# gillet-thomas/NeuroViT

Measured on AMD Instinct MI355X. Metric: fMRI volumes/sec (fwd+bwd) ViT3D 128^3 p16 d768 L12 [timed step = fwd+bwd+AdamW update], higher is better.
Workload: dtype bf16; 1 GPU; ViT3D-base 128^3 patch 16, train step (fwd+bwd+AdamW), batch 4/GPU, dropout 0; global_batch=4, parallelism=dp1, grad_buckets=7, grad_allreduce=none (1 GPU)

## Files before the change

include/neurovit_hip.h:

```cpp
#ifndef NEUROVIT_HIP_H
#define NEUROVIT_HIP_H

#ifdef __cplusplus
extern "C" {
#endif

#define NV_OK 0
#define NV_ERR_ARG (-1)
#define NV_ERR_HIP (-2)
#define NV_ERR_ARCH (-3)

int nv_version(void);
int nv_arch_ok(void);
const char* nv_last_error(void);

#define NV_OPERAND_BF16 0
#define NV_OPERAND_FP16 1
int nv_set_operand_format(int fmt);
int nv_operand_format(void);

int nv_prof_enable(int on);
int nv_prof_summary(int kind, double* ms, double* work, long* count);
int nv_prof_summary_bytes(int kind, double* bytes);

int nv_gemm_bf16(int layout, int epi, int M, int N, int K, const void* A, long lda, const void* B, long ldb, void* C,
                 long ldc, const float* bias, const void* aux_in, long ld_aux_in, void* aux_out, long ld_aux_out,
                 int accumulate, float alpha, unsigned long drop_seed, float drop_p, void* stream);

int nv_gemm_tile_rows(int layout, int M, int N, int K, long lda, long ldb);

int nv_quant_rows_f8(const float* W, long ldw, int rows, int cols, void* out8, long ld8, float act_scale, float* colscale, void* stream);
int nv_ln_fwd_f8(const float* x, long ldx, int M, int d, const float* gamma, const float* beta, float eps, float out_scale, void* y8,
                 long ldy, void* stream);
int nv_gemm_f8(int epi, int M, int N, int K, const void* A8, long lda, const void* B8, long ldb, void* C, long ldc,
               const float* colscale, const float* bias, const void* aux_in, long ld_aux_in, float out_scale, void* stream);
int nv_ln_fwd_f8_train(const float* x, long ldx, int M, int d, const float* gamma, const float* beta, float eps, float out_scale, void* y8, long ldy8,
                       void* y16, long ldy16, float* mean, float* rstd, void* stream);
int nv_gemm_f8_gelu_train(int M, int N, int K, const void* A8, long lda, const void* B8, long ldb, const float* colscale, const float* bias,
                          float out_scale, void* h8, long ldh8, void* h16, long ldh16, void* u16, long ldu16, unsigned long drop_seed,
                          float drop_p, void* stream);
int nv_gemm_f8_resid_drop(int M, int N, int K, const void* A8, long lda, const void* B8, long ldb, void* C, long ldc, const float* colscale,
                          const float* bias, const void* aux_in, long ld_aux_in, unsigned long drop_seed, float drop_p, void* stream);

int nv_gemm_f32(int epi, int M, int N, int K, const float* A, long lda, const float* B, long ldb, float* C, long ldc,
                const float* bias, const float* resid, long ldr, void* stream);
int nv_gemm_f32_set_tile(int wm, int wn);
int nv_attn_fwd_f32(const float* qkv, long ld_qkv, int B, int n, int heads, int dim_head, float scale, float* out, long ld_out,
                    void* stream);
int nv_ln_fwd_f32(const float* x, long ldx, int M, int d, const float* gamma, const float* beta, float eps, float* y, long ldy,
                  float* mean, float* rstd, void* stream);

typedef struct nv_gemm_problem {
  int M, N, K;
  const void* A; long lda;
  const void* B; long ldb;
  void* C; long ldc;
  int accumulate;
  void* C16; long ldc16;
} nv_gemm_problem;
int nv_gemm_bf16_grouped(int layout, int epi, int count, const nv_gemm_problem* problems, void* stream);

typedef struct nv_adamw_arena {
  int struct_size;
  int step;
  double lr, beta1, beta2, eps, weight_decay;
  float grad_scale;
  int keep_grads;
  float* params; float* grads; float* adam_m; float* adam_v; void* params16;
} nv_adamw_arena;
int nv_gemm_bf16_grouped_adamw(int count, const nv_gemm_problem* problems, const nv_adamw_arena* opt, void* stream);
int nv_adamw_ranges(const nv_adamw_arena* opt, const long* begins, const long* lens, int count, void* stream);

int nv_gemm_set_tile(int bm, int bn);

int nv_gemm_lnfold_supported(int M, int N, int K);
long nv_ln_fold_stats_floats(int M, int d);
int nv_ln_fold_weight(const float* W, long ldw, int N, int K, const float* gamma, const float* beta, const float* bias, void* Wg16, long ldg,
                      float* colsum, float* fbias, void* stream);
int nv_gemm_resid_ln(int M, int N, int K, const void* A, long lda, const void* W, long ldw, const float* bias, const float* resid, long ldr, float* out,
                     long ldo, void* out16, long ldo16, float* stats, void* stream);
int nv_gemm_lnfold(int gelu, int M, int N, int K, const void* X16, long ldx, const void* Wg16, long ldw, const float* stats, const float* colsum,
                   const float* fbias, float eps, void* out16, long ldo, void* stream);

int nv_skinny_nt(int epi, int R, int N, int K, const void* A, long lda, const void* W, long ldw, const float* bias, const float* resid,
                 long ldr, void* out, long ldo, void* u_out, long ldu, unsigned long drop_seed, float drop_p, void* stream);
int nv_skinny_nn(int epi, int R, int N, int K, const void* A, long lda, const void* W, long ldw, const void* u, long ldu, void* out, long ldo,
                 float* dcol, int accumulate, unsigned long drop_seed, float drop_p, void* stream);
int nv_skinny_nn_sparse(int R, int N, int K, const void* A, long lda, const void* W, long ldw, void* out, long total_rows, int keep_every,
                        void* stream);

int nv_ln_fwd(const float* x, long ldx, int M, int d, const float* gamma, const float* beta, float eps, void* y, long ldy,
              float* mean, float* rstd, void* stream);
long nv_ln_bwd_workspace_bytes(int M, int d);
int nv_ln_bwd(const float* dy, long lddy, const float* x, long ldx, const float* mean, const float* rstd, const float* gamma,
              int M, int d, const float* g_in, float* g_out, long ldg, void* g16, long ldg16, float* dgamma, float* dbeta,
              float* dcolsum, int accumulate, void* workspace, long ws_bytes, unsigned long drop_seed, float drop_p,
              void* stream, void* reduce_stream);
#define NV_LN_NO_REDUCE ((void*)(-1L))
int nv_ln_bwd_reduce(const void* workspace, int M, int d, float* dgamma, float* dbeta, float* dcolsum, int accumulate, void* stream);

typedef struct nv_reduce_job {
  const float* partials;
  int rows, width, nseg;
  float* out[3];
  int accumulate;
} nv_reduce_job;
int nv_reduce_multi(const nv_reduce_job* jobs, int count, void* stream);
int nv_ln_bwd_partial_rows(int M);

long nv_zscore_crop_workspace_bytes(int B);
int nv_volume_sigma(const void* raw, int dtype, const long* strides5, int B, const int* crop8, float eps, float* sigma, float* mean,
                    void* workspace, long ws_bytes, void* stream);
int nv_zscore_crop(const void* raw, int dtype, const long* strides5, int B, const int* crop8, float eps, float* out,
                   float* stats, void* workspace, long ws_bytes, void* stream);

int nv_patch_ln_fwd(const float* video, const long* strides5, int B, int C, int F, int H, int W, int p1, int p2, int pf,
                    const float* gamma, const float* beta, float eps, void* out, long ldo, float* mean, float* rstd,
                    const float* vol_sigma, void* stream);
int nv_patch_set_mode(int mode);
int nv_patch_ln_fwd_4d(const float* x, int Bo, int H, int W, int D, int T, int p1, int p2, int pf, const float* gamma,
                       const float* beta, float eps, void* out, long ldo, float* mean, float* rstd, const float* vol_sigma,
                       void* stream);
int nv_patch_ln_fwd_f32(const float* video, const long* strides5, int B, int C, int F, int H, int W, int p1, int p2, int pf,
                        const float* gamma, const float* beta, float eps, float* out, long ldo, float* mean, float* rstd,
                        const float* vol_sigma, void* stream);
int nv_patch_ln_fwd_4d_f32(const float* x, int Bo, int H, int W, int D, int T, int p1, int p2, int pf, const float* gamma,
                           const float* beta, float eps, float* out, long ldo, float* mean, float* rstd, const float* vol_sigma,
                           void* stream);
long nv_patch_ln_bwd_workspace_bytes(int tokens, int P);
int nv_patch_ln_bwd(const float* video, const long* strides5, int B, int C, int F, int H, int W, int p1, int p2, int pf,
                    const float* dxp, long ldd, const float* mean, const float* rstd, float* dgamma, float* dbeta,
                    int accumulate, void* workspace, long ws_bytes, void* stream);
int nv_patch_ln_dx(const float* video, const long* strides5, int B, int C, int F, int H, int W, int p1, int p2, int pf,
                   const float* dxp, long ldd, const float* mean, const float* rstd, const float* gamma,
                   float* dvideo, const long* dstrides5, void* stream);

int nv_embed_finish_fwd(const float* t, long ldt, int B, int N, int d, const float* gamma, const float* beta, float eps,
                        const float* pos, const float* cls, float* x, long ldx, float* mean, float* rstd,
                        unsigned long drop_seed, float drop_p, void* stream);
long nv_embed_finish_bwd_workspace_bytes(int B, int N, int d);
int nv_embed_finish_bwd(const float* g, long ldg, const float* t, long ldt, const float* mean, const float* rstd,
                        const float* gamma, int B, int N, int d, float* dt, long lddt, void* dt16, long lddt16, float* dgamma,
                        float* dbeta, float* dbias_pe, float* dpos, float* dcls, int accumulate, void* workspace, long ws_bytes,
                        unsigned long drop_seed, float drop_p, void* stream);

int nv_attn_set_mode(int mode);
int nv_attn_fwd(const void* qkv, long ld_qkv, int B, int n, int heads, int dim_head, float scale, void* out, long ld_out,
                float* lse, unsigned long drop_seed, float drop_p, void* stream);
int nv_attn_fwd_o8(const void* qkv, long ld_qkv, int B, int n, int heads, int dim_head, float scale, void* out, long ld_out,
                   float out_scale, void* stream);
int nv_attn_bwd(const void* qkv, long ld_qkv, const void* out, const void* dout, long ld_out, const float* lse, int B, int n,
                int heads, int dim_head, float scale, float* delta, void* dqkv, long ld_dqkv, unsigned long drop_seed,
                float drop_p, void* stream);
#define NV_ATTN_PER_HEAD 0
#define NV_ATTN_FUSE_MEAN 1
#define NV_ATTN_FUSE_MAX 2
#define NV_ATTN_FUSE_MIN 3
#define NV_ATTN_ROWS_ALL 0
#define NV_ATTN_ROWS_CLS 1
int nv_attn_probs(int qkv_f32, const void* qkv, long ld_qkv, int B, int n, int heads, int dim_head, float scale, int fusion, int rows,
                  float* out, void* stream);
long nv_attn_rollout_workspace_bytes(int B, int n);
int nv_attn_rollout(const float* const* maps, int L, int B, int n, int start_mean, float* out, void* workspace, long ws_bytes, void* stream);
#define NV_ATTN_GRAD_PER_HEAD 0
#define NV_ATTN_GRAD_RELEVANCE 1
int nv_attn_grad(const void* qkv, long ld_qkv, const void* dout, long ld_dout, int B, int n, int heads, int dim_head, float scale, int form,
                 float* out, void* stream);
long nv_attn_relevance_workspace_bytes(int B, int n);
int nv_attn_relevance(const float* const* maps, int L, int B, int n, int start_mean, float* out, void* workspace, long ws_bytes, void* stream);
int nv_stream_sync(void* from, void* to);
int nv_spin_us(int microseconds, void* stream);

int nv_head_fwd(const float* x, long row_stride, int B, int d, const float* gamma, const float* beta, float eps,
                const float* W, const float* bias, int C, float* xh, float* stats, float* logits, void* stream);
long nv_head_bwd_workspace_bytes(int B, int d);
int nv_head_bwd(const float* dlogits, int B, int C, const float* W, const float* x, long row_stride, const float* stats,
                const float* xh, const float* gamma, int d, int n, float* g, long ldg, void* g16, long ldg16, float* dgamma,
                float* dbeta, float* dW, float* dbias, float* dcolsum, int accumulate, void* workspace, long ws_bytes,
                unsigned long drop_seed, float drop_p, int pool_mean, void* stream);
long nv_head_step_workspace_bytes(int B, int d);
int nv_head_step(const float* x, long row_stride, int B, int d, const float* gamma, const float* beta, float eps, const float* W,
                 const float* bias, int C, const long* labels, float grad_scale, float* xh, float* stats, float* logits, float* loss,
                 float* dlogits, int n, float* g, long ldg, void* g16, long ldg16, float* dgamma, float* dbeta, float* dW, float* dbias,
                 float* dcolsum, int accumulate, void* workspace, long ws_bytes, unsigned long drop_seed, float drop_p, void* stream);
int nv_token_mean(const float* x, int B, int n, int d, float* out, void* stream);

long nv_colsum_workspace_bytes(int M, int N);
int nv_colsum_bf16(const void* X, long ld, int M, int N, float* out, int accumulate, void* workspace, long ws_bytes,
                   void* stream);

int nv_ce_loss(const float* logits, const long* target, int B, int C, float grad_scale, float* loss, float* dlogits,
               void* stream);
int nv_adamw_step(float* p, const void* grad, int grad_bf16, float* m, float* v, void* p16, long count, int step, double lr,
                  double beta1, double beta2, double eps, double weight_decay, float grad_scale, int max_blocks, void* stream);
#define NV_LOSS_SCALE_FLOATS 16
int nv_loss_scale_init(float* state, float init_scale, float growth_factor, float backoff_factor, int growth_interval, int start_step, void* stream);
int nv_loss_scale_check(const float* grads, long count, float* state, void* stream);
int nv_loss_scale_update(float* state, double lr, double beta1, double beta2, void* stream);
int nv_ce_loss_scaled(const float* logits, const long* target, int B, int C, float grad_scale, const float* scale_state, float* loss,
                      float* dlogits, void* stream);
int nv_adamw_step_scaled(float* p, const void* grad, int grad_bf16, float* m, float* v, void* p16, long count, int step, double lr,
                         double beta1, double beta2, double eps, double weight_decay, float grad_scale, int max_blocks,
                         const float* scale_state, void* stream);
int nv_head_step_scaled(const float* x, long row_stride, int B, int d, const float* gamma, const float* beta, float eps, const float* W,
                        const float* bias, int C, const long* labels, float grad_scale, const float* scale_state, float* xh, float* stats,
                        float* logits, float* loss, float* dlogits, int n, float* g, long ldg, void* g16, long ldg16, float* dgamma,
                        float* dbeta, float* dW, float* dbias, float* dcolsum, int accumulate, void* workspace, long ws_bytes,
                        unsigned long drop_seed, float drop_p, void* stream);
#define NV_GRAD_CLIP_MAX_BLOCKS 2048
#define NV_GRAD_CLIP_BYTES (64 + 8 * NV_GRAD_CLIP_MAX_BLOCKS)
int nv_grad_sumsq(const void* grad, int grad_16bit, long count, float* clip_state, float* scale_state, int max_blocks, void* stream);
int nv_grad_clip_finish(float* clip_state, float max_norm, float grad_scale, const float* scale_state, void* stream);
int nv_adamw_step_clipped(float* p, const void* grad, int grad_bf16, float* m, float* v, void* p16, long count, int step, double lr,
                          double beta1, double beta2, double eps, double weight_decay, float grad_scale, int max_blocks,
                          const float* scale_state, const float* clip_state, void* stream);
#define NV_ADAMW_MAX_GROUPS 64
#define NV_ADAMW_MAX_SEGMENTS 1024
typedef struct nv_adamw_groups {
  int struct_size;
  int n_groups;
  const void* segments;
  double lr[NV_ADAMW_MAX_GROUPS];
  double weight_decay[NV_ADAMW_MAX_GROUPS];
} nv_adamw_groups;
long nv_adamw_segments_bytes(int segments);
int nv_adamw_segments_build(void* table, long table_bytes, const long* ends, const int* groups, int segments, int n_groups, long count, void* stream);
int nv_adamw_segments_release(void* table);
int nv_adamw_step_grouped(float* p, const void* grad, int grad_bf16, float* m, float* v, void* p16, long count, int step,
                          const nv_adamw_groups* groups, double beta1, double beta2, double eps, float grad_scale, int max_blocks,
                          const float* scale_state, const float* clip_state, void* stream);
int nv_ema_update(float* ema, const float* p, long count, float weight, int max_blocks, void* stream);
int nv_cast_bf16_2d(const float* src, long ld_src, int rows, int cols, void* dst, long ld_dst, void* stream);
int nv_dropout_apply(const float* x, long ldx, int M, int N, unsigned long drop_seed, float drop_p, void* out16, long ld16,
                     float* out32, long ld32, void* stream);
int nv_copy_2d_f32(const float* src, long ld_src, int rows, int cols, float* dst, long ld_dst, int accumulate, void* stream);

long nv_gradcam_workspace_bytes(int B, int n);
int nv_gradcam_reduce(const void* act, const float* grad, int B, int n, int d, float* cam, float* minmax, void* workspace,
                      long ws_bytes, void* stream);
long nv_gradcam_per_volume_workspace_bytes(int B, int n);
int nv_gradcam_reduce_per_volume(const void* act, const float* grad, int B, int n, int d, float* cam, float* minmax, void* workspace,
                                 long ws_bytes, void* stream);
long nv_token_map_to_volume_workspace_bytes(int B, const int* grid3);
int nv_token_map_to_volume(const float* maps, int B, const int* grid3, const int* out3, int normalize, double keep_percent, float* out,
                           void* workspace, long ws_bytes, void* stream);

#define NV_SCORE_PROB 0
#define NV_SCORE_LOGIT 1
int nv_token_ranks(const float* maps, int B, int N, int* ranks, void* stream);
int nv_mask_patches(const float* x, int B, const int* size3, const int* patch3, const int* labels, const int* jobs, int J, float value,
                    const float* base, long base_stride, float* out, void* stream);
int nv_mask_patches_set_group(int group);
int nv_class_scores(const float* logits, int J, int C, const int* jobs, const long* cls, int B, int kind, float* scores, void* stream);
int nv_curve_auc(const float* scores, int B, int K, long ld, float* auc, void* stream);
int nv_occlusion_gather(const float* ref, const float* scores, const int* labels, int B, int N, int NB, float* maps, void* stream);

int nv_path_points(const float* x, int B, long V, const int* jobs, int J, const float* alphas, int K, float value, const float* base,
                   long base_stride, float* out, void* stream);
int nv_class_score_grads(const float* logits, int J, int C, const int* jobs, const long* cls, int B, int kind, float* dlogits, void* stream);
int nv_path_accumulate(const float* g, const int* jobs, int J, const float* weights, int K, float* acc, int B, long V, void* stream);
int nv_path_finish(const float* acc, const float* x, int B, long V, float value, const float* base, long base_stride, float* attr, void* stream);
int nv_attr_token_sums(const float* attr, int B, const int* size3, const int* patch3, float* sums, void* stream);

#define NV_SERIES_SCOPE_SERIES 0
#define NV_SERIES_SCOPE_VOLUME 1
#define NV_SERIES_LAYOUT_SERIES 0
#define NV_SERIES_LAYOUT_FRAMES 1
long nv_gradcam_grouped_workspace_bytes(int V, int n, int group);
int nv_gradcam_reduce_grouped(const void* act, const float* grad, int V, int n, int d, int group, float* cam, float* minmax, void* workspace,
                              long ws_bytes, void* stream);
long nv_series_map_to_volumes_workspace_bytes(int B, int T, const int* grid3, int scope);
int nv_series_map_to_volumes(const float* maps, int B, int T, const int* grid3, const int* out3, int normalize, int scope, double keep_percent,
                             int layout, float* out, void* workspace, long ws_bytes, void* stream);
int nv_series_leave_one_out(const float* z, const float* z_base, int B, int T, float* out, void* stream);
int nv_temporal_grad_x_input(const float* dx, const float* z, int B, int T, float* out, void* stream);

long nv_temporal_head_param_count(int ff);
int nv_temporal_head_fwd(const float* x, int B, int T, int ff, const float* params, float eps, unsigned long drop_seed, float drop_p,
                         float* out, void* stream);
int nv_temporal_head_bwd(const float* x, int B, int T, int ff, const float* params, float eps, unsigned long drop_seed, float drop_p,
                         const float* dout, float* grads, int accumulate, float* dx, void* stream);

typedef struct nv_vit_config {
  int image_size, image_patch_size, frames, frame_patch_size;
  int channels, num_classes, dim, depth, heads, dim_head, mlp_dim;
  float ln_eps;
  int pool_mean;
  int image_width, patch_width;
  int no_proj_dropout;
} nv_vit_config;

long nv_vit_param_count(const nv_vit_config* cfg);
int nv_vit_param_table(const nv_vit_config* cfg, long* offsets, long* numels, int max_entries);
long nv_vit_workspace_bytes(const nv_vit_config* cfg, int B, int training);
long nv_vit_workspace_offset(const nv_vit_config* cfg, int B, int training, const char* name, int layer);
typedef struct nv_vit_attn_export {
  int struct_size;
  float** maps;
  int fusion;
  int rows;
} nv_vit_attn_export;
typedef struct nv_vit_input {
  const float* vol_sigma;
  int time_points;
  int rows_form;
  const nv_vit_attn_export* attn_export;
} nv_vit_input;
int nv_vit_forward_in(const nv_vit_config* cfg, int B, const float* video, const long* shape5, const long* strides5,
                      const nv_vit_input* in, const float* params, const void* params16, void* workspace, long ws_bytes,
                      int training, float drop_p, float emb_drop_p, unsigned long drop_seed, float* logits, void* stream);
int nv_vit_forward(const nv_vit_config* cfg, int B, const float* video, const long* shape5, const long* strides5,
                   const float* params, const void* params16, void* workspace, long ws_bytes, int training, float drop_p, float emb_drop_p,
                   unsigned long drop_seed, float* logits, void* stream);
long nv_vit_lnfold_floats(const nv_vit_config* cfg);
int nv_vit_lnfold_prepare(const nv_vit_config* cfg, const float* params, void* fold16, float* fold32, void* stream);
int nv_vit_forward_lnfold(const nv_vit_config* cfg, int B, const float* video, const long* shape5, const long* strides5, const nv_vit_input* in,
                          const float* params, const void* params16, const void* fold16, const float* fold32, void* workspace, long ws_bytes,
                          float* logits, void* stream);
int nv_vit_forward_f32(const nv_vit_config* cfg, int B, const float* video, const long* shape5, const long* strides5,
                       const nv_vit_input* in, const float* params, void* workspace, long ws_bytes, float* logits, void* stream);
long nv_vit_fp8_scale_count(const nv_vit_config* cfg);
int nv_vit_quantize_fp8(const nv_vit_config* cfg, const float* params, const float* act_scales, void* params8, float* colscales, void* stream);
int nv_vit_forward_fp8(const nv_vit_config* cfg, int B, const float* video, const long* shape5, const long* strides5,
                       const nv_vit_input* in, const float* params, const void* params16, const void* params8, const float* colscales,
                       const float* act_scales, void* workspace, long ws_bytes, float* logits, void* stream);
int nv_vit_forward_fp8_train(const nv_vit_config* cfg, int B, const float* video, const long* shape5, const long* strides5,
                             const nv_vit_input* in, const float* params, const void* params16, const void* params8, const float* colscales,
                             const float* act_scales, void* workspace, long ws_bytes, float drop_p, float emb_drop_p, unsigned long drop_seed,
                             float* logits, void* stream);
int nv_vit_backward(const nv_vit_config* cfg, int B, const float* video, const long* strides5, const float* params,
                    const void* params16, void* workspace, long ws_bytes, const float* dlogits, float* grads,
                    int accumulate, float drop_p, float emb_drop_p, unsigned long drop_seed, void* stream, void* aux_stream);

int nv_vit_backward_stages(const nv_vit_config* cfg, int B, const float* video, const long* strides5, const float* params,
                           const void* params16, void* workspace, long ws_bytes, const float* dlogits, float* grads,
                           int accumulate, int first_stage, int last_stage, float drop_p, float emb_drop_p,
                           unsigned long drop_seed, void* stream, void* aux_stream, int join_aux);
int nv_vit_backward_stages16(const nv_vit_config* cfg, int B, const float* video, const long* strides5, const float* params,
                             const void* params16, void* workspace, long ws_bytes, const float* dlogits, float* grads, void* grads16,
                             int accumulate, int first_stage, int last_stage, float drop_p, float emb_drop_p,
                             unsigned long drop_seed, void* stream, void* aux_stream, int join_aux, int rows_form);
typedef struct nv_vit_backward_opts {
  int struct_size;
  float* dvideo;
  const long* dvideo_strides5;
  int weight_grads;
} nv_vit_backward_opts;
int nv_vit_backward_ex(const nv_vit_config* cfg, int B, const float* video, const long* strides5, const float* params,
                       const void* params16, void* workspace, long ws_bytes, const float* dlogits, float* grads, void* grads16,
                       int accumulate, int first_stage, int last_stage, float drop_p, float emb_drop_p,
                       unsigned long drop_seed, void* stream, void* aux_stream, int join_aux, int rows_form, const nv_vit_backward_opts* opts);
typedef struct nv_vit_attn_grad_export {
  int struct_size;
  float** maps;
  int form;
} nv_vit_attn_grad_export;
int nv_vit_backward_attn(const nv_vit_config* cfg, int B, const float* video, const long* strides5, const float* params,
                         const void* params16, void* workspace, long ws_bytes, const float* dlogits, float* grads, void* grads16,
                         int accumulate, int first_stage, int last_stage, float drop_p, float emb_drop_p,
                         unsigned long drop_seed, void* stream, void* aux_stream, int join_aux, int rows_form, const nv_vit_backward_opts* opts,
                         const nv_vit_attn_grad_export* attn_grad);
int nv_vit_backward_tokens(const nv_vit_config* cfg, int B, const float* video, const long* strides5, const float* params,
                           const void* params16, void* workspace, long ws_bytes, const float* dtokens, float* grads, void* grads16,
                           int accumulate, int first_stage, int last_stage, float drop_p, float emb_drop_p,
                           unsigned long drop_seed, void* stream, void* aux_stream, int join_aux, int rows_form, const nv_vit_backward_opts* opts);
int nv_vit_stage_param_range(const nv_vit_config* cfg, int stage, long* begin, long* end);
int nv_vit_set_cls_tail(int on);
int nv_vit_set_head_step(int on);

typedef struct nv_dp_plan {
  int struct_size;
  int world;
  void* comm;
  void* comm_stream;
  int n_buckets;
  int update_per_bucket;
  void* grads16;
// ... 143 lines not shown
```

neurovit_amd/_cabi.py:

```python
from __future__ import annotations

import ctypes
import os
import re
from typing import Dict, List, Tuple

_HERE = os.path.dirname(os.path.abspath(__file__))
HEADER = os.path.join(os.path.dirname(_HERE), "include", "neurovit_hip.h")
LIB_PATH = os.environ.get("NEUROVIT_HIP_LIB") or os.path.join(_HERE, "lib", "libneurovit_hip.so")

_SCALARS = {"int": ctypes.c_int, "long": ctypes.c_long, "float": ctypes.c_float, "double": ctypes.c_double}


class VitConfig(ctypes.Structure):
    _fields_ = [("image_size", ctypes.c_int), ("image_patch_size", ctypes.c_int), ("frames", ctypes.c_int),
                ("frame_patch_size", ctypes.c_int), ("channels", ctypes.c_int), ("num_classes", ctypes.c_int),
                ("dim", ctypes.c_int), ("depth", ctypes.c_int), ("heads", ctypes.c_int), ("dim_head", ctypes.c_int),
                ("mlp_dim", ctypes.c_int), ("ln_eps", ctypes.c_float), ("pool_mean", ctypes.c_int),
                ("image_width", ctypes.c_int), ("patch_width", ctypes.c_int),
                ("no_proj_dropout", ctypes.c_int)]


class VitInput(ctypes.Structure):
    _fields_ = [("vol_sigma", ctypes.c_void_p), ("time_points", ctypes.c_int), ("rows_form", ctypes.c_int), ("attn_export", ctypes.c_void_p)]
# ... 28 lines not shown

class AdamwArena(ctypes.Structure):
    _fields_ = [("struct_size", ctypes.c_int), ("step", ctypes.c_int), ("lr", ctypes.c_double), ("beta1", ctypes.c_double),
                ("beta2", ctypes.c_double), ("eps", ctypes.c_double), ("weight_decay", ctypes.c_double), ("grad_scale", ctypes.c_float),
                ("keep_grads", ctypes.c_int), ("params", ctypes.c_void_p), ("grads", ctypes.c_void_p), ("adam_m", ctypes.c_void_p),
                ("adam_v", ctypes.c_void_p), ("params16", ctypes.c_void_p)]


class BackwardOpts(ctypes.Structure):
    _fields_ = [("struct_size", ctypes.c_int), ("dvideo", ctypes.c_void_p), ("dvideo_strides5", ctypes.c_void_p), ("weight_grads", ctypes.c_int)]


class LossOpts(ctypes.Structure):
    _fields_ = [("struct_size", ctypes.c_int), ("label_smoothing", ctypes.c_float), ("class_weight", ctypes.c_void_p), ("mix", ctypes.c_void_p)]


class DropPath(ctypes.Structure):
    _fields_ = [("struct_size", ctypes.c_int), ("factors", ctypes.c_void_p)]


DROP_PATH_SCHEDULES = {"linear": 0, "constant": 1}


ADAMW_MAX_GROUPS, ADAMW_MAX_SEGMENTS = 64, 1024


class AdamwGroups(ctypes.Structure):
    _fields_ = [("struct_size", ctypes.c_int), ("n_groups", ctypes.c_int), ("segments", ctypes.c_void_p),
                ("lr", ctypes.c_double * ADAMW_MAX_GROUPS), ("weight_decay", ctypes.c_double * ADAMW_MAX_GROUPS)]


MIX_COLS = 12


ABI_VERSION = 8


def parse_header(path: str = HEADER) -> Dict[str, Tuple[object, List[object]]]:
    src = open(path).read()
    src = re.sub(r"/\*.*?\*/", " ", src, flags=re.S)
    protos = {}
    for m in re.finditer(r"\b(int|long|const char\s*\*)\s+(nv_\w+)\s*\(([^;{]*?)\)\s*;", src, flags=re.S):
        ret, name, args = m.group(1), m.group(2), " ".join(m.group(3).split())
        restype = ctypes.c_char_p if "char" in ret else _SCALARS[ret]
        argtypes = []
        if args and args != "void":
            for a in args.split(","):
                a = a.strip()
                if "*" in a:
                    argtypes.append(ctypes.c_char_p if re.match(r"const char\s*\*", a) else ctypes.c_void_p)
                elif a.startswith("unsigned long"):
                    argtypes.append(ctypes.c_ulong)
                else:
                    argtypes.append(_SCALARS[a.split()[0]])
        protos[name] = (restype, argtypes)
    return protos


class _Lib:
    def __init__(self):
        self._dll = None
        self.protos = parse_header()

    def load(self):
        if self._dll is None:
            if not os.path.exists(LIB_PATH):
                raise RuntimeError(
                    f"neurovit_amd: {LIB_PATH} not found - build it with `python -c 'import __graft_entry__ as g; g.build()'` "
                    "(or `make -C neurovit_amd/csrc`). There is no CPU / PyTorch fallback for this path.")
            dll = ctypes.CDLL(LIB_PATH)
            for name, (restype, argtypes) in self.protos.items():
                fn = getattr(dll, name)
                fn.restype, fn.argtypes = restype, argtypes
            got = dll.nv_abi_version()
            if got != ABI_VERSION:
                raise RuntimeError(f"neurovit_amd: {LIB_PATH} has ABI revision {got}, this binding expects {ABI_VERSION} - rebuild the library "
                                   "(make -C neurovit_amd/csrc); see INTEGRATION.md 'ABI revisions'")
            if os.environ.get("NEUROVIT_ATTN_MODE"):
                dll.nv_attn_set_mode(int(os.environ["NEUROVIT_ATTN_MODE"]))
            if os.environ.get("NEUROVIT_ADAMW_WGS"):
                dll.nv_gemm_set_tile(12, int(os.environ["NEUROVIT_ADAMW_WGS"]))
            if os.environ.get("NEUROVIT_HEAD_STEP"):
                dll.nv_vit_set_head_step(int(os.environ["NEUROVIT_HEAD_STEP"]))
            if os.environ.get("NEUROVIT_WGRAD_WGS"):
                dll.nv_gemm_set_tile(14, int(os.environ["NEUROVIT_WGRAD_WGS"]))
            if os.environ.get("NEUROVIT_PATCH_MODE"):
                dll.nv_patch_set_mode(int(os.environ["NEUROVIT_PATCH_MODE"]))
            if os.environ.get("NEUROVIT_ADAMW_CAP"):
                dll.nv_gemm_set_tile(13, int(os.environ["NEUROVIT_ADAMW_CAP"]))
            self._dll = dll
        return self._dll

    def __getattr__(self, name):
        return getattr(self.load(), name)


lib = _Lib()


OPERAND_FORMATS = {"bf16": 0, "fp16": 1}
_operand_format = "bf16"


def set_operand_format(fmt: str) -> None:
    global _operand_format
    if fmt != _operand_format:
        if fmt not in OPERAND_FORMATS:
            raise ValueError(f"neurovit_amd: operand format must be 'bf16' or 'fp16', got {fmt!r}")
        check(lib.nv_set_operand_format(OPERAND_FORMATS[fmt]), "nv_set_operand_format")
        _operand_format = fmt


def operand_format() -> str:
    return _operand_format


def last_error() -> str:
    return (lib.nv_last_error() or b"").decode()


def check(rc: int, what: str = "") -> None:
    if rc != 0:
        raise RuntimeError(f"neurovit_amd C-ABI call failed ({what}, rc={rc}): {last_error()}")


def require_gpu() -> None:
    import torch
    if not torch.cuda.is_available():
        raise RuntimeError("neurovit_amd: no HIP device available - this path only runs on MI355X (gfx950); "
                           "there is no CPU fallback.")
    if lib.nv_arch_ok() != 1:
        raise RuntimeError(f"neurovit_amd: current device is not gfx950: {last_error()}")
```

neurovit_amd/csrc/attention.hip:

```cpp
#include "common.h"

bool attn_generic_supported(int dim_head);
int launch_attn_generic_fwd(const void* qkv, long ld, int B, int n, int heads, int dh, float scale, void* out, long ldo, float* lse, DropCfg drop,
                            hipStream_t s);
int launch_attn_generic_bwd(const void* qkv, long ld, const void* out, const void* dout, long ldo, const float* lse, int B, int n, int heads, int dh,
                            float scale, float* delta, void* dqkv, long ldd, DropCfg drop, hipStream_t s);

constexpr int DH = 64;
constexpr int TQ = 64;
constexpr int TK = 64;
constexpr int IMG = TK * DH * 2;

__device__ __forceinline__ void tile_gload(const r16* X, long ld, int row0, int nrows, int tid, uint4 (&reg)[2]) {
#pragma unroll
  for (int i = 0; i < 2; ++i) {
    const int c = tid + 256 * i, row = row0 + (c >> 3);
    const bool ok = row < nrows;
    const uint4 v = *reinterpret_cast<const uint4*>(X + (ok ? (long)row * ld + ((c & 7) << 3) : 0));
    reg[i] = ok ? v : make_uint4(0, 0, 0, 0);
  }
}
__device__ __forceinline__ void tile_swrite(char* img, int tid, const uint4 (&reg)[2]) {
#pragma unroll
  for (int i = 0; i < 2; ++i) {
// ... 742 lines not shown
  for (int qt = 0; qt < nqt; ++qt) {
    __syncthreads();
    tile_swrite(sQ, tid, rq);
    tile_swrite(sD, tid, rd);
    if (tid < TQ) { sL[tid] = rl; sDl[tid] = rdl; }
    __syncthreads();
    if (qt + 1 < nqt) {
      tile_gload(Q, ld, (qt + 1) * TQ, n, tid, rq);
      tile_gload(dO, ldo, (qt + 1) * TQ, n, tid, rd);
      stats_load(qt + 1);
    }
    dkv_tile<DROP, T>(sQ, sD, sL, sDl, qt, n, kf, vf, dk, dv, scale_log2e, drop, gb.by, key0 + r, r, g);
  }
  const int key = key0 + r;
  if (key < n) {
    r16* drow = dqkv + ((long)b * n + key) * ldd + h * DH;
#pragma unroll
    for (int t = 0; t < 4; ++t) {
      *reinterpret_cast<r16x4*>(drow + inner + 16 * t + 4 * g) = cvt4<T>(dk[t][0] * scale, dk[t][1] * scale, dk[t][2] * scale, dk[t][3] * scale);
      *reinterpret_cast<r16x4*>(drow + 2 * inner + 16 * t + 4 * g) = cvt4<T>(dv[t][0], dv[t][1], dv[t][2], dv[t][3]);
    }
  }
}

template <typename T>
__device__ __forceinline__ float row_delta(const r16* __restrict__ dout, const r16* __restrict__ out, long off, int g, r16x8 (&dof)[2]) {
  float dl = 0.f;
#pragma unroll
  for (int ks = 0; ks < 2; ++ks) {
    dof[ks] = *reinterpret_cast<const r16x8*>(dout + off + 32 * ks + 8 * g);
    const r16x8 of = *reinterpret_cast<const r16x8*>(out + off + 32 * ks + 8 * g);
#pragma unroll
    for (int j = 0; j < 8; ++j) dl += dec1<T>(dof[ks][j]) * dec1<T>(of[j]);
  }
  return group_sum(dl);
}

template <bool DROP, typename T>
__device__ __forceinline__ void attn_bwd_dq_res_body(char* rsmem, int by, int bx, int nblk, const r16* __restrict__ qkv, long ld,
                                                     const r16* __restrict__ out, const r16* __restrict__ dout, long ldo,
                                                     const float* __restrict__ lse, int n, int heads, float scale, float* __restrict__ delta,
                                                     r16* __restrict__ dqkv, long ldd, const DropCfg& drop) {
  const int tid = threadIdx.x, lane = tid & 63, r = lane & 15, g = lane >> 4;
  const int wid = __builtin_amdgcn_readfirstlane(tid >> 6);
  const int b = by / heads, h = by - b * heads, inner = heads * DH;
  const r16* Q = qkv + (long)b * n * ld + h * DH;
  const int nkt = (n + TK - 1) / TK;
  char* sK = rsmem;
  char* sV = rsmem + nkt * IMG;
  res_dma(Q + inner, ld, n, nkt, sK, wid, lane);
  res_dma(Q + 2 * inner, ld, n, nkt, sV, wid, lane);
  const int grp = res_group(n, wid, bx, nblk);
  const int q0 = (grp < 0 ? 0 : grp) * 16;
  const int qrow = min(q0 + r, n - 1);
  const float scale_log2e = scale * 1.44269504088896340736f;

  r16x8 qf[2], dof[2];
#pragma unroll
  for (int ks = 0; ks < 2; ++ks) qf[ks] = *reinterpret_cast<const r16x8*>(Q + (long)qrow * ld + 32 * ks + 8 * g);
  const float dl = row_delta<T>(dout, out, ((long)b * n + qrow) * ldo + h * DH, g, dof);
  const float lse2 = lse[((long)b * heads + h) * n + qrow] * 1.44269504088896340736f;
  __syncthreads();
  if (grp < 0) return;
  if (g == 0 && q0 + r < n) delta[((long)b * heads + h) * n + q0 + r] = dl;

  f32x4 dq[4];
#pragma unroll
  for (int t = 0; t < 4; ++t) dq[t] = f32x4{0.f, 0.f, 0.f, 0.f};
  for (int kt = 0; kt < nkt; ++kt)
    dq_tile<DROP, T>(sK + kt * IMG, sV + kt * IMG, kt, n, qf, dof, dq, dl, lse2, scale_log2e, drop, by, q0 + r, r, g);
  const int q = q0 + r;
  if (q < n) {
    r16* drow = dqkv + ((long)b * n + q) * ldd + h * DH;
#pragma unroll
    for (int t = 0; t < 4; ++t)
      *reinterpret_cast<r16x4*>(drow + 16 * t + 4 * g) = cvt4<T>(dq[t][0] * scale, dq[t][1] * scale, dq[t][2] * scale, dq[t][3] * scale);
  }
}

template <bool DROP, bool OWN_DELTA, typename T>
__device__ __forceinline__ void attn_bwd_dkv_res_body(char* rsmem, int by, int bx, int nblk, const r16* __restrict__ qkv, long ld,
                                                      const r16* __restrict__ out, const r16* __restrict__ dout, long ldo,
                                                      const float* __restrict__ lse, const float* __restrict__ delta, int n, int heads,
                                                      float scale, r16* __restrict__ dqkv, long ldd, const DropCfg& drop) {
  const int tid = threadIdx.x, lane = tid & 63, r = lane & 15, g = lane >> 4;
  const int wid = __builtin_amdgcn_readfirstlane(tid >> 6);
  const int b = by / heads, h = by - b * heads, inner = heads * DH;
  const r16* Q = qkv + (long)b * n * ld + h * DH;
  const r16* K = Q + inner;
  const r16* V = Q + 2 * inner;
  const r16* dO = dout + (long)b * n * ldo + h * DH;
  const float* L = lse + ((long)b * heads + h) * n;
  const int nqt = (n + TQ - 1) / TQ;
  char* sQ = rsmem;
  char* sD = rsmem + nqt * IMG;
  float* sL = reinterpret_cast<float*>(rsmem + 2 * nqt * IMG);
  float* sDl = sL + nqt * TQ;
  res_dma(Q, ld, n, nqt, sQ, wid, lane);
  res_dma(dO, ldo, n, nqt, sD, wid, lane);
  if constexpr (OWN_DELTA) {
    for (int q = tid; q < nqt * TQ; q += RES_THREADS) sL[q] = (q < n) ? L[q] * 1.44269504088896340736f : INFINITY;
    const r16* O = out + (long)b * n * ldo + h * DH;
    for (int q0 = 16 * wid; q0 < nqt * TQ; q0 += 16 * (RES_THREADS / 64)) {
      r16x8 scratch[2];
      const int q = q0 + r;
      const float dl = row_delta<T>(dO, O, (long)min(q, n - 1) * ldo, g, scratch);
      if (g == 0) sDl[q] = (q < n) ? dl : 0.f;
    }
  } else {
    const float* Dl = delta + ((long)b * heads + h) * n;
    for (int q = tid; q < nqt * TQ; q += RES_THREADS) {
      sL[q] = (q < n) ? L[q] * 1.44269504088896340736f : INFINITY;
      sDl[q] = (q < n) ? Dl[q] : 0.f;
    }
  }
  const int grp = res_group(n, wid, bx, nblk);
  const int key0 = (grp < 0 ? 0 : grp) * 16;
  const int krow = min(key0 + r, n - 1);
  const float scale_log2e = scale * 1.44269504088896340736f;
  r16x8 kf[2], vf[2];
#pragma unroll
  for (int ks = 0; ks < 2; ++ks) {
    kf[ks] = *reinterpret_cast<const r16x8*>(K + (long)krow * ld + 32 * ks + 8 * g);
    vf[ks] = *reinterpret_cast<const r16x8*>(V + (long)krow * ld + 32 * ks + 8 * g);
  }
  __syncthreads();
  if (grp < 0) return;

  f32x4 dk[4], dv[4];
#pragma unroll
  for (int t = 0; t < 4; ++t) dk[t] = dv[t] = f32x4{0.f, 0.f, 0.f, 0.f};
  for (int qt = 0; qt < nqt; ++qt)
    dkv_tile<DROP, T>(sQ + qt * IMG, sD + qt * IMG, sL + qt * TQ, sDl + qt * TQ, qt, n, kf, vf, dk, dv, scale_log2e, drop, by, key0 + r, r, g);
  const int key = key0 + r;
  if (key < n) {
    r16* drow = dqkv + ((long)b * n + key) * ldd + h * DH;
#pragma unroll
    for (int t = 0; t < 4; ++t) {
      *reinterpret_cast<r16x4*>(drow + inner + 16 * t + 4 * g) = cvt4<T>(dk[t][0] * scale, dk[t][1] * scale, dk[t][2] * scale, dk[t][3] * scale);
      *reinterpret_cast<r16x4*>(drow + 2 * inner + 16 * t + 4 * g) = cvt4<T>(dv[t][0], dv[t][1], dv[t][2], dv[t][3]);
    }
  }
}

template <bool DROP, typename T>
__global__ __launch_bounds__(RES_THREADS) void attn_bwd_dq_res_kernel(const r16* __restrict__ qkv, long ld, const r16* __restrict__ out,
                                                                      const r16* __restrict__ dout, long ldo, const float* __restrict__ lse,
                                                                      int n, int heads, float scale, float* __restrict__ delta,
                                                                      r16* __restrict__ dqkv, long ldd, DropCfg drop) {
  extern __shared__ __attribute__((aligned(16))) char rsmem[];
  const ResBlock rb = res_block(n);
  attn_bwd_dq_res_body<DROP, T>(rsmem, rb.by, rb.bx, rb.nblk, qkv, ld, out, dout, ldo, lse, n, heads, scale, delta, dqkv, ldd, drop);
}

template <bool DROP, typename T>
__global__ __launch_bounds__(RES_THREADS) void attn_bwd_dkv_res_kernel(const r16* __restrict__ qkv, long ld, const r16* __restrict__ dout,
                                                                       long ldo, const float* __restrict__ lse, const float* __restrict__ delta,
                                                                       int n, int heads, float scale, r16* __restrict__ dqkv, long ldd,
                                                                       DropCfg drop) {
  extern __shared__ __attribute__((aligned(16))) char rsmem[];
  const ResBlock rb = res_block(n);
  attn_bwd_dkv_res_body<DROP, false, T>(rsmem, rb.by, rb.bx, rb.nblk, qkv, ld, nullptr, dout, ldo, lse, delta, n, heads, scale, dqkv, ldd, drop);
}

template <bool DROP, typename T>
__global__ __launch_bounds__(RES_THREADS) void attn_bwd_res_kernel(const r16* __restrict__ qkv, long ld, const r16* __restrict__ out,
                                                                   const r16* __restrict__ dout, long ldo, const float* __restrict__ lse,
                                                                   int n, int heads, float scale, float* __restrict__ delta,
                                                                   r16* __restrict__ dqkv, long ldd, DropCfg drop) {
  extern __shared__ __attribute__((aligned(16))) char rsmem[];
  const int nblk = attn_res_blocks(n);
  const int lid = xcd_remap(blockIdx.x, gridDim.x);
  const int by = lid / (2 * nblk), rem = lid - by * 2 * nblk;
  if (rem < nblk) attn_bwd_dkv_res_body<DROP, true, T>(rsmem, by, rem, nblk, qkv, ld, out, dout, ldo, lse, nullptr, n, heads, scale, dqkv, ldd, drop);
  else attn_bwd_dq_res_body<DROP, T>(rsmem, by, rem - nblk, nblk, qkv, ld, out, dout, ldo, lse, n, heads, scale, delta, dqkv, ldd, drop);
}

template <bool DROP, typename T>
__global__ __launch_bounds__(256, 2) void attn_bwd_dq_wide_kernel(const r16* __restrict__ qkv, long ld, const r16* __restrict__ out,
                                                                  const r16* __restrict__ dout, long ldo, const float* __restrict__ lse, int n,
                                                                  int heads, float scale, float* __restrict__ delta, r16* __restrict__ dqkv,
                                                                  long ldd, DropCfg drop) {
  __shared__ __attribute__((aligned(16))) char wsmem[2 * 2 * IMG];
  const int tid = threadIdx.x, lane = tid & 63, r = lane & 15, g = lane >> 4;
  const int wid = __builtin_amdgcn_readfirstlane(tid >> 6);
  const Grid2 gb = grid2d_xcd((n + WIDE_ROWS - 1) / WIDE_ROWS);
  const int b = gb.by / heads, h = gb.by - b * heads, inner = heads * DH;
  const r16* Q = qkv + (long)b * n * ld + h * DH;
  const int q0 = gb.bx * WIDE_ROWS + 32 * wid;
  const float scale_log2e = scale * 1.44269504088896340736f;

  r16x8 qf[2][2], dof[2][2];
  float dl[2], lse2[2];
#pragma unroll
  for (int u = 0; u < 2; ++u) {
    const int qrow = min(q0 + 16 * u + r, n - 1);
    float d = 0.f;
#pragma unroll
    for (int ks = 0; ks < 2; ++ks) {
      qf[u][ks] = *reinterpret_cast<const r16x8*>(Q + (long)qrow * ld + 32 * ks + 8 * g);
      const long off = ((long)b * n + qrow) * ldo + h * DH + 32 * ks + 8 * g;
      dof[u][ks] = *reinterpret_cast<const r16x8*>(dout + off);
      const r16x8 of = *reinterpret_cast<const r16x8*>(out + off);
#pragma unroll
      for (int j = 0; j < 8; ++j) d += dec1<T>(dof[u][ks][j]) * dec1<T>(of[j]);
    }
    dl[u] = group_sum(d);
    lse2[u] = lse[((long)b * heads + h) * n + qrow] * 1.44269504088896340736f;
    if (g == 0 && q0 + 16 * u + r < n) delta[((long)b * heads + h) * n + q0 + 16 * u + r] = dl[u];
  }

  const unsigned bytes = (unsigned)((((long)n - 1) * ld + DH) * 2);
  const dma_desc rsK = uniform_rsrc((Q + inner), bytes);
  const dma_desc rsV = uniform_rsrc((Q + 2 * inner), bytes);
  int voff[2];
#pragma unroll
  for (int i = 0; i < 2; ++i) {
    const int row = (wid + 4 * i) * 8 + (lane >> 3);
    voff[i] = (int)(((long)row * ld + (((lane & 7) ^ (row & 7)) << 3)) * 2);
  }
  const int step = (int)(64 * ld * 2);
  auto issue = [&](int t, char* stage) {
#pragma unroll
    for (int i = 0; i < 2; ++i) {
      lds_dma<16>(rsK, stage + (wid + 4 * i) * 1024, voff[i], t * step);
      lds_dma<16>(rsV, stage + IMG + (wid + 4 * i) * 1024, voff[i], t * step);
    }
  };

  f32x4 dq[2][4];
#pragma unroll
  for (int u = 0; u < 2; ++u)
#pragma unroll
    for (int t = 0; t < 4; ++t) dq[u][t] = f32x4{0.f, 0.f, 0.f, 0.f};
  const int nkt = (n + TK - 1) / TK;
  issue(0, wsmem);
  for (int kt = 0; kt < nkt; ++kt) {
    const char* cur = wsmem + (kt & 1) * 2 * IMG;
    asm volatile("s_waitcnt vmcnt(0)" ::: "memory");
    __builtin_amdgcn_s_barrier();
    if (kt + 1 < nkt) issue(kt + 1, wsmem + ((kt + 1) & 1) * 2 * IMG);
    RowFrags F;
    f32x4 sc[2][4], dp[2][4], ds[2][4];
    load_row_frags(cur, r, g, F);
    mfma_rows<T>(F, qf[0], sc[0], true);
// ... 92 lines not shown
      lds_dma<4>(rsL, stage + 2 * IMG, ln * 4, t * TQ * 4);
      lds_dma<4>(rsDl, stage + 2 * IMG + TQ * 4, ln * 4, t * TQ * 4);
    }
  };

  f32x4 dk[2][4], dv[2][4];
#pragma unroll
  for (int u = 0; u < 2; ++u)
#pragma unroll
    for (int t = 0; t < 4; ++t) dk[u][t] = dv[u][t] = f32x4{0.f, 0.f, 0.f, 0.f};
  const int nqt = (n + TQ - 1) / TQ;
  issue(0, wsmem);
  for (int qt = 0; qt < nqt; ++qt) {
    const char* cur = wsmem + (qt & 1) * STG;
    asm volatile("s_waitcnt vmcnt(0)" ::: "memory");
    __builtin_amdgcn_s_barrier();
    if (qt + 1 < nqt) issue(qt + 1, wsmem + ((qt + 1) & 1) * STG);
    const float* sL = reinterpret_cast<const float*>(cur + 2 * IMG);
    const float* sDl = sL + TQ;
    RowFrags F;
    if constexpr (DROP) {
#pragma unroll
      for (int u = 0; u < 2; ++u) {
        f32x4 sc1[4], dp1[4];
        load_row_frags(cur, r, g, F);
        mfma_rows<T>(F, kf[u], sc1, true);
        __builtin_amdgcn_sched_barrier(0);
        load_row_frags(cur + IMG, r, g, F);
        mfma_rows<T>(F, vf[u], dp1, true);
        __builtin_amdgcn_sched_barrier(0);
        dkv_softmax_grad_inplace<DROP>(sc1, dp1, sL, sDl, qt, n, scale_log2e, drop, gb.by, key0 + 16 * u + r, g);
        r16x8 pf1[2], dsf1[2];
        pf1[0] = cvt8<T>(sc1[0], sc1[1]); pf1[1] = cvt8<T>(sc1[2], sc1[3]);
        dsf1[0] = cvt8<T>(dp1[0], dp1[1]); dsf1[1] = cvt8<T>(dp1[2], dp1[3]);
        __builtin_amdgcn_sched_barrier(0);
        load_tr_frags(cur + IMG, r, g, F);
        mfma_rows<T>(F, pf1, dv[u], false);
        __builtin_amdgcn_sched_barrier(0);
        load_tr_frags(cur, r, g, F);
        mfma_rows<T>(F, dsf1, dk[u], false);
        __builtin_amdgcn_sched_barrier(0);
      }
      continue;
    }
    f32x4 sc[2][4], dp[2][4];
    load_row_frags(cur, r, g, F);
    mfma_rows<T>(F, kf[0], sc[0], true);
    mfma_rows<T>(F, kf[1], sc[1], true);
    __builtin_amdgcn_sched_barrier(0);
    load_row_frags(cur + IMG, r, g, F);
    mfma_rows<T>(F, vf[0], dp[0], true);
    mfma_rows<T>(F, vf[1], dp[1], true);
    __builtin_amdgcn_sched_barrier(0);
    r16x8 pf[2][2], dsf[2][2];
    dkv_softmax_grad_inplace<DROP>(sc[0], dp[0], sL, sDl, qt, n, scale_log2e, drop, gb.by, key0 + r, g);
    pf[0][0] = cvt8<T>(sc[0][0], sc[0][1]); pf[0][1] = cvt8<T>(sc[0][2], sc[0][3]);
    dsf[0][0] = cvt8<T>(dp[0][0], dp[0][1]); dsf[0][1] = cvt8<T>(dp[0][2], dp[0][3]);
    dkv_softmax_grad_inplace<DROP>(sc[1], dp[1], sL, sDl, qt, n, scale_log2e, drop, gb.by, key0 + 16 + r, g);
    pf[1][0] = cvt8<T>(sc[1][0], sc[1][1]); pf[1][1] = cvt8<T>(sc[1][2], sc[1][3]);
    dsf[1][0] = cvt8<T>(dp[1][0], dp[1][1]); dsf[1][1] = cvt8<T>(dp[1][2], dp[1][3]);
    __builtin_amdgcn_sched_barrier(0);
    load_tr_frags(cur + IMG, r, g, F);
    mfma_rows<T>(F, pf[0], dv[0], false);
    mfma_rows<T>(F, pf[1], dv[1], false);
    __builtin_amdgcn_sched_barrier(0);
    load_tr_frags(cur, r, g, F);
    mfma_rows<T>(F, dsf[0], dk[0], false);
    mfma_rows<T>(F, dsf[1], dk[1], false);
  }
#pragma unroll
  for (int u = 0; u < 2; ++u) {
    const int key = key0 + 16 * u + r;
    if (key < n) {
      r16* drow = dqkv + ((long)b * n + key) * ldd + h * DH;
#pragma unroll
      for (int t = 0; t < 4; ++t) {
        *reinterpret_cast<r16x4*>(drow + inner + 16 * t + 4 * g) = cvt4<T>(dk[u][t][0] * scale, dk[u][t][1] * scale, dk[u][t][2] * scale, dk[u][t][3] * scale);
        *reinterpret_cast<r16x4*>(drow + 2 * inner + 16 * t + 4 * g) = cvt4<T>(dv[u][t][0], dv[u][t][1], dv[u][t][2], dv[u][t][3]);
      }
    }
  }
}

extern "C" int nv_attn_bwd(const void* qkv, long ld_qkv, const void* out, const void* dout, long ld_out, const float* lse, int B, int n,
                           int heads, int dim_head, float scale, float* delta, void* dqkv, long ld_dqkv, unsigned long drop_seed, float drop_p,
                           void* stream) {
  NV_CHECK_ARG(attn_generic_supported(dim_head), "nv_attn_bwd: dim_head=%d unsupported (multiples of 8 up to 128)", dim_head);
  NV_CHECK_ARG(B > 0 && n > 0 && heads > 0 && ld_qkv >= 3 * heads * dim_head && ld_dqkv >= 3 * heads * dim_head && ld_out >= heads * dim_head &&
                   (ld_qkv % 8) == 0 && (ld_out % 8) == 0 && (ld_dqkv % 4) == 0,
               "nv_attn_bwd: bad dims");
  NV_CHECK_ARG(nv_aligned16(qkv) && nv_aligned16(out) && nv_aligned16(dout) && nv_aligned16(dqkv), "nv_attn_bwd: alignment");
  hipStream_t s = (hipStream_t)stream;
  const DropCfg drop = make_drop(drop_seed, drop_p);
  if (dim_head != DH)
    return launch_attn_generic_bwd(qkv, ld_qkv, out, dout, ld_out, lse, B, n, heads, dim_head, scale, delta, dqkv, ld_dqkv, drop, s);
  const dim3 grid(((n + TQ - 1) / TQ) * B * heads);
  const bool dropping = drop.thresh != 0, fp16 = nv_operand_format() == NV_OPERAND_FP16;
  const r16* q16 = (const r16*)qkv; const r16* o16 = (const r16*)out; const r16* do16 = (const r16*)dout; r16* dq16 = (r16*)dqkv;
  const int slot = nv_prof_begin(4, 10.0 * B * heads * (double)n * n * DH, stream);
  if (attn_resident(n) && g_attn_mode != 3) {
    NV_CHECK_ARG((long)n * ld_qkv < (1L << 30) && (long)n * ld_out < (1L << 30), "nv_attn_bwd: operand too large for 32-bit buffer offsets");
    const int nt = (n + TK - 1) / TK;
    static bool attr = false;
    if (!attr) {
      ATTN_ATTR(K_DQ_RES, 2 * RES_MAX_TILES * IMG);
      ATTN_ATTR(K_DKV_RES, 2 * RES_MAX_TILES * IMG + 2 * RES_MAX_TILES * TQ * 4);
      ATTN_ATTR(K_BWD_RES, 2 * RES_MAX_TILES * IMG + 2 * RES_MAX_TILES * TQ * 4);
      attr = true;
    }
    const dim3 rgrid(attn_res_blocks(n) * B * heads);
    if (g_attn_bwd_merged) {
      ATTN_LAUNCH(K_BWD_RES, dim3(2 * rgrid.x), dim3(RES_THREADS), 2 * nt * IMG + 2 * nt * TQ * 4, s, q16, ld_qkv, o16, do16, ld_out, lse, n, heads, scale, delta, dq16, ld_dqkv, drop);
      nv_prof_end(slot, stream);
      NV_CHECK_LAUNCH("nv_attn_bwd(resident, one launch)");
      return NV_OK;
    }
    ATTN_LAUNCH(K_DQ_RES, rgrid, dim3(RES_THREADS), 2 * nt * IMG, s, q16, ld_qkv, o16, do16, ld_out, lse, n, heads, scale, delta, dq16, ld_dqkv, drop);
    NV_CHECK_LAUNCH("nv_attn_bwd/dq(resident)");
    ATTN_LAUNCH(K_DKV_RES, rgrid, dim3(RES_THREADS), 2 * nt * IMG + 2 * nt * TQ * 4, s, q16, ld_qkv, do16, ld_out, lse, delta, n, heads, scale, dq16, ld_dqkv, drop);
    nv_prof_end(slot, stream);
    NV_CHECK_LAUNCH("nv_attn_bwd/dkv(resident)");
    return NV_OK;
  }
  const bool wide = g_attn_mode != 1 && (long)n * ld_qkv < (1L << 30) && (long)n * ld_out < (1L << 30) &&
                    (g_attn_mode >= 3 || (long)B * heads * ((n + WIDE_ROWS - 1) / WIDE_ROWS) >= 512);
  const dim3 wgrid(((n + WIDE_ROWS - 1) / WIDE_ROWS) * B * heads);
  if (wide) ATTN_LAUNCH(K_DQ_WIDE, wgrid, dim3(256), 0, s, q16, ld_qkv, o16, do16, ld_out, lse, n, heads, scale, delta, dq16, ld_dqkv, drop);
  else ATTN_LAUNCH(K_DQ, grid, dim3(256), 0, s, q16, ld_qkv, o16, do16, ld_out, lse, n, heads, scale, delta, dq16, ld_dqkv, drop);
  NV_CHECK_LAUNCH("nv_attn_bwd/dq");
  if (wide) ATTN_LAUNCH(K_DKV_WIDE, wgrid, dim3(256), 0, s, q16, ld_qkv, do16, ld_out, lse, delta, n, heads, scale, dq16, ld_dqkv, drop);
  else ATTN_LAUNCH(K_DKV, grid, dim3(256), 0, s, q16, ld_qkv, do16, ld_out, lse, delta, n, heads, scale, dq16, ld_dqkv, drop);
  nv_prof_end(slot, stream);
  NV_CHECK_LAUNCH("nv_attn_bwd/dkv");
  return NV_OK;
}
```

neurovit_amd/csrc/engine.hip:

```cpp
#include <stdlib.h>
#include <string.h>

#include <unordered_map>
#include <utility>
#include <vector>

#include "../../include/neurovit_hip.h"

#include "common.h"

namespace {

inline long align_up(long v, long a) { return (v + a - 1) / a * a; }

struct Dims {
  int B, N, n, P, Ppad, d, inner, m, L, C, heads, dh, M, T;
  int gf, gh, gw;
  int pool_mean;
};

static int g_cls_tail = 1;
extern "C" int nv_vit_set_cls_tail(int on) { g_cls_tail = on ? 1 : 0; return 0; }
static int g_head_step = 1;
extern "C" int nv_vit_set_head_step(int on) { g_head_step = on ? 1 : 0; return 0; }
static bool cls_tail_wanted(const Dims& D, int training, float drop_p, int rows_form) {
  const bool want = rows_form == 1 ? false : (rows_form == 2 ? true : g_cls_tail != 0);
  (void)drop_p;
  return want && !D.pool_mean && (!training || D.B <= 4);
}

static inline float proj_drop_p(const nv_vit_config* c, float drop_p) { return c->no_proj_dropout ? 0.f : drop_p; }

static inline int img_w(const nv_vit_config* c) { return c->image_width > 0 ? c->image_width : c->image_size; }
static inline int pat_w(const nv_vit_config* c) { return c->patch_width > 0 ? c->patch_width : c->image_patch_size; }

int make_dims(const nv_vit_config* c, int B, Dims& D) {
  NV_CHECK_ARG(c && B > 0, "nv_vit: null config or B <= 0");
  NV_CHECK_ARG(c->image_size > 0 && c->image_patch_size > 0 && c->frames > 0 && c->frame_patch_size > 0 &&
                   c->image_size % c->image_patch_size == 0 && c->image_width >= 0 && c->patch_width >= 0 && img_w(c) % pat_w(c) == 0,
               "Image dimensions must be divisible by the patch size.");
  NV_CHECK_ARG(c->frames % c->frame_patch_size == 0, "Frames must be divisible by frame patch size");
  NV_CHECK_ARG(c->dim_head >= 8 && c->dim_head <= 128 && c->dim_head % 8 == 0,
               "nv_vit: dim_head=%d unsupported (multiples of 8 up to 128; 64 runs the MFMA attention kernels, the others scalar ones)", c->dim_head);
  NV_CHECK_ARG(c->dim % 8 == 0 && c->dim <= 2048 && c->mlp_dim % 8 == 0, "nv_vit: dim must be a multiple of 8 and <= 2048, mlp_dim a multiple of 8");
  NV_CHECK_ARG(c->depth >= 1 && c->num_classes >= 1 && c->channels >= 1, "nv_vit: bad depth/classes/channels");
  D.B = B;
  D.gf = c->frames / c->frame_patch_size;
  D.gh = c->image_size / c->image_patch_size;
  D.gw = img_w(c) / pat_w(c);
  D.N = D.gf * D.gh * D.gw;
  D.n = D.N + 1;
  D.P = c->channels * c->image_patch_size * pat_w(c) * c->frame_patch_size;
  D.Ppad = (int)align_up(D.P, 8);
  D.d = c->dim; D.heads = c->heads; D.dh = c->dim_head; D.inner = c->heads * c->dim_head; D.m = c->mlp_dim;
  D.L = c->depth; D.C = c->num_classes;
  D.M = B * D.n; D.T = B * D.N;
  D.pool_mean = c->pool_mean != 0;
  return NV_OK;
}

struct LayerP { long n1g, n1b, wqkv, wo, bo, n2g, n2b, w1, b1, w2, b2; };
struct ParamTab {
  long pos, cls, pe_g, pe_b, pe_w, pe_bias, pe_g2, pe_b2, hg, hb, hw, hbias, total;
  std::vector<LayerP> layer;
  std::vector<long> offsets, numels;
};

void make_params(const Dims& D, ParamTab& T) {
  long cur = 0;
  auto add = [&](long numel) { const long o = cur; T.offsets.push_back(o); T.numels.push_back(numel); cur = align_up(cur + numel, 8); return o; };
  T.pos = add((long)D.n * D.d); T.cls = add(D.d);
  T.pe_g = add(D.P); T.pe_b = add(D.P); T.pe_w = add((long)D.d * D.P); T.pe_bias = add(D.d); T.pe_g2 = add(D.d); T.pe_b2 = add(D.d);
  T.layer.resize(D.L);
  for (int l = 0; l < D.L; ++l) {
    LayerP& p = T.layer[l];
    p.n1g = add(D.d); p.n1b = add(D.d); p.wqkv = add(3L * D.inner * D.d); p.wo = add((long)D.d * D.inner); p.bo = add(D.d);
    p.n2g = add(D.d); p.n2b = add(D.d); p.w1 = add((long)D.m * D.d); p.b1 = add(D.m); p.w2 = add((long)D.d * D.m); p.b2 = add(D.d);
  }
  T.hg = add(D.d); T.hb = add(D.d); T.hw = add((long)D.C * D.d); T.hbias = add(D.C);
  T.total = cur;
}

struct LayerW { long xn1, st1, qkv, lse, ao, x1, xn2, st2, u, h, x2; };
struct LayerScratch { long g16, g16b, du, dqkv, red, red2, red3, cs1; };
struct WS {
  long xp, pst, t, est, x0, xh, hst, wpe16, xm;
  long fst1, fst2;
  long f8x, f8h;
  std::vector<LayerW> layer;
  long g, dxn, hookg, dao, delta, dt, dt16, dxp, dwpe;
  LayerScratch sc[2];
  const LayerScratch& scratch(int l) const { return sc[l & 1]; }
  long red_bytes, red2_bytes, total;
};

void make_ws(const Dims& D, int training, WS& W) {
  long cur = 0;
  auto add = [&](long bytes) { const long o = cur; cur = align_up(cur + bytes, 256); return o; };
  const long M = D.M, T = D.T, d = D.d;
  W.xp = add(T * D.Ppad * 2); W.pst = add(T * 2 * 4); W.t = add(T * d * 4); W.est = add(T * 2 * 4); W.x0 = add(M * d * 4);
  W.xh = add((long)D.B * d * 4); W.hst = add((long)D.B * 2 * 4);
  W.xm = D.pool_mean ? add((long)D.B * d * 4) : -1;
  W.wpe16 = (D.P != D.Ppad) ? add(d * D.Ppad * 2) : -1;
  W.fst1 = add(nv_ln_fold_stats_floats((int)M, (int)d) * 4); W.fst2 = add(nv_ln_fold_stats_floats((int)M, (int)d) * 4);
  const int nl = training ? D.L : 1;
  W.layer.resize(D.L);
  for (int l = 0; l < nl; ++l) {
    LayerW& w = W.layer[l];
    w.xn1 = add(M * d * 2); w.st1 = add(M * 2 * 4); w.qkv = add(M * 3 * D.inner * 2); w.lse = add((long)D.B * D.heads * D.n * 4);
    w.ao = add(M * D.inner * 2); w.x1 = add(M * d * 4); w.xn2 = add(M * d * 2); w.st2 = add(M * 2 * 4);
    w.u = add(M * D.m * 2); w.h = add(M * D.m * 2); w.x2 = add(M * d * 4);
  }
  for (int l = nl; l < D.L; ++l) W.layer[l] = W.layer[0];
  W.f8x = W.f8h = -1;
  if (training) {
    LayerScratch& e = W.sc[0]; LayerScratch& o = W.sc[1];
    W.g = add(M * d * 4); e.g16 = add(M * d * 2); W.dxn = add(M * d * 4); W.hookg = add(M * d * 4); e.du = add(M * D.m * 2);
    W.dao = add(M * D.inner * 2); e.dqkv = add(M * 3 * D.inner * 2); W.delta = add((long)D.B * D.heads * D.n * 4);
    W.dt = add(T * d * 4); W.dt16 = add(T * d * 2); W.dxp = add(T * D.Ppad * 4);
    W.dwpe = (D.P != D.Ppad) ? add(d * D.Ppad * 4) : -1;
    long r = nv_ln_bwd_workspace_bytes(D.M, D.d);
    const long r2 = nv_patch_ln_bwd_workspace_bytes(D.T, D.P), r3 = nv_head_step_workspace_bytes(D.B, D.d),
               r4 = nv_colsum_workspace_bytes(D.M, D.m);
    r = r > r2 ? r : r2; r = r > r3 ? r : r3; r = r > r4 ? r : r4;
    W.red_bytes = r; e.red = add(r);
    e.g16b = add(M * d * 2);
    W.red2_bytes = r4 > r2 ? r4 : r2; e.red2 = add(W.red2_bytes);
    e.red3 = add(nv_ln_bwd_workspace_bytes(D.M, D.d));
    o.g16 = add(M * d * 2); o.g16b = add(M * d * 2); o.du = add(M * D.m * 2); o.dqkv = add(M * 3 * D.inner * 2);
    o.red = add(W.red_bytes); o.red2 = add(W.red2_bytes); o.red3 = add(nv_ln_bwd_workspace_bytes(D.M, D.d));
    const long cs1_bytes = (long)((M + 63) / 64) * D.m * 4;
    e.cs1 = add(cs1_bytes); o.cs1 = add(cs1_bytes);
    W.f8x = add(M * d); W.f8h = add(M * (long)D.m);
  } else {
    W.g = W.dxn = W.hookg = W.dao = W.delta = W.dt = W.dt16 = W.dxp = W.dwpe = -1;
    W.sc[0] = W.sc[1] = {-1, -1, -1, -1, -1, -1, -1, -1};
    W.red_bytes = W.red2_bytes = 0;
  }
  W.total = cur;
}

struct WSF { long xp, pst, t, est, x0, xh, hst, xm, xn1, qkv, ao, x1, xn2, h, x2, total; };
void make_wsf(const Dims& D, WSF& W) {
  long cur = 0;
  auto add = [&](long bytes) { const long o = cur; cur = align_up(cur + bytes, 256); return o; };
  const long M = D.M, T = D.T, d = D.d;
  W.xp = add(T * D.P * 4); W.pst = add(T * 2 * 4); W.t = add(T * d * 4); W.est = add(T * 2 * 4); W.x0 = add(M * d * 4);
  W.xh = add((long)D.B * d * 4); W.hst = add((long)D.B * 2 * 4);
  W.xm = D.pool_mean ? add((long)D.B * d * 4) : -1;
  W.xn1 = add(M * d * 4); W.qkv = add(M * 3 * D.inner * 4); W.ao = add(M * D.inner * 4); W.x1 = add(M * d * 4);
  W.xn2 = add(M * d * 4); W.h = add(M * D.m * 4); W.x2 = add(M * d * 4);
  W.total = cur;
}

inline unsigned long site_seed(unsigned long seed, int site) { return seed ^ (0x9E3779B97F4A7C15ul * (unsigned long)(site + 1)); }

inline const float* path_of(const float* sd, int l, int c, int B) { return sd ? sd + ((long)l * 2 + c) * B : nullptr; }
int check_drop_path(const nv_vit_drop_path* sd, const char* who) {
  if (!sd) return NV_OK;
  NV_CHECK_ARG(sd->struct_size == (int)sizeof(nv_vit_drop_path), "%s: nv_vit_drop_path.struct_size=%d, expected %d (ABI revision %d)", who, sd->struct_size,
               (int)sizeof(nv_vit_drop_path), NV_ABI_VERSION);
  NV_CHECK_ARG(sd->factors && nv_aligned(sd->factors, 4), "%s: nv_vit_drop_path.factors is NULL or not 4-byte aligned", who);
  return NV_OK;
}

inline int stream_sync(hipStream_t from, hipStream_t to) { return nv_stream_sync((void*)from, (void*)to); }
inline int event_failed(const char* what) { nv_set_error("nv_vit_backward: event %s failed", what); return NV_ERR_HIP; }
inline int wait_event(hipStream_t s, hipEvent_t e) { return hipStreamWaitEvent(s, e, 0) == hipSuccess ? NV_OK : event_failed("wait"); }
inline int record_event(hipEvent_t e, hipStream_t s) { return (e && hipEventRecord(e, s) == hipSuccess) ? NV_OK : event_failed("record"); }
inline hipEvent_t deferred_event() {
  static std::vector<hipEvent_t> pool;
  static size_t next = 0;
  if (pool.size() < 32) {
    hipEvent_t e;
    if (hipEventCreateWithFlags(&e, nv_sync_event_flags()) != hipSuccess) return nullptr;
    pool.push_back(e);
    return e;
  }
  return pool[next++ % pool.size()];
}

struct Carry { hipEvent_t ev = nullptr; bool pending = false; };
std::unordered_map<void*, Carry>& carry_map() { static std::unordered_map<void*, Carry> m; return m; }
hipEvent_t carry_take(void* workspace) {
  auto it = carry_map().find(workspace);
  if (it == carry_map().end() || !it->second.pending) return nullptr;
  it->second.pending = false;
  return it->second.ev;
}
int carry_record(void* workspace, hipStream_t on) {
  Carry& c = carry_map()[workspace];
  if (!c.ev && hipEventCreateWithFlags(&c.ev, nv_sync_event_flags()) != hipSuccess) return event_failed("create");
  if (const int rc = record_event(c.ev, on)) return rc;
  c.pending = true;
  return NV_OK;
}

#define RUN(call)            \
  do {                       \
    const int rc__ = (call); \
    if (rc__) return rc__;   \
  } while (0)

struct LinearW { long off[4], numel[4]; };
inline LinearW linear_weights(const Dims& D, const LayerP& q) {
  return {{q.wqkv, q.wo, q.w1, q.w2}, {3L * D.inner * D.d, (long)D.d * D.inner, (long)D.m * D.d, (long)D.d * D.m}};
}

struct Layout { Dims D; ParamTab T; WS W; };
int make_layout(const nv_vit_config* c, int B, int training, Layout& Y) {
  RUN(make_dims(c, B, Y.D));
  make_params(Y.D, Y.T);
  make_ws(Y.D, training, Y.W);
  return NV_OK;
}

}

extern "C" long nv_vit_param_count(const nv_vit_config* cfg) {
  Dims D; if (make_dims(cfg, 1, D)) return -1;
// ... 4 lines not shown
extern "C" int nv_vit_param_table(const nv_vit_config* cfg, long* offsets, long* numels, int max_entries) {
  Dims D; if (make_dims(cfg, 1, D)) return NV_ERR_ARG;
  ParamTab T; make_params(D, T);
  const int cnt = (int)T.offsets.size();
  for (int i = 0; i < cnt && i < max_entries; ++i) { offsets[i] = T.offsets[i]; numels[i] = T.numels[i]; }
  return cnt;
}

extern "C" long nv_vit_workspace_bytes(const nv_vit_config* cfg, int B, int training) {
  Dims D; if (make_dims(cfg, B, D)) return -1;
  if (training == 2) { WSF F; make_wsf(D, F); return F.total; }
  WS W; make_ws(D, training, W);
  return W.total;
}

extern "C" long nv_vit_workspace_offset(const nv_vit_config* cfg, int B, int training, const char* name, int layer) {
  Dims D; if (make_dims(cfg, B, D)) return -1;
  if (training == 2) {
    WSF F; make_wsf(D, F);
    if (layer >= D.L) return -1;
    if (!strcmp(name, "xn1")) return F.xn1; if (!strcmp(name, "qkv")) return F.qkv; if (!strcmp(name, "ao")) return F.ao;
    if (!strcmp(name, "x1")) return F.x1; if (!strcmp(name, "xn2")) return F.xn2; if (!strcmp(name, "h")) return F.h;
    if (!strcmp(name, "x2")) return (layer >= 0 && (layer & 1)) ? F.x0 : F.x2;
    if (!strcmp(name, "xp")) return F.xp; if (!strcmp(name, "t")) return F.t; if (!strcmp(name, "x0")) return F.x0; if (!strcmp(name, "xh")) return F.xh;
    return -1;
  }
  WS W; make_ws(D, training, W);
  if (layer >= 0) {
    if (layer >= D.L) return -1;
    const LayerW& w = W.layer[layer];
    if (!strcmp(name, "xn1")) return w.xn1; if (!strcmp(name, "st1")) return w.st1; if (!strcmp(name, "qkv")) return w.qkv;
    if (!strcmp(name, "lse")) return w.lse; if (!strcmp(name, "ao")) return w.ao; if (!strcmp(name, "x1")) return w.x1;
    if (!strcmp(name, "xn2")) return w.xn2; if (!strcmp(name, "st2")) return w.st2; if (!strcmp(name, "u")) return w.u;
    if (!strcmp(name, "h")) return w.h; if (!strcmp(name, "x2")) return w.x2;
    return -1;
  }
  if (!strcmp(name, "xp")) return W.xp; if (!strcmp(name, "pst")) return W.pst; if (!strcmp(name, "t")) return W.t;
  if (!strcmp(name, "est")) return W.est; if (!strcmp(name, "x0")) return W.x0; if (!strcmp(name, "xh")) return W.xh;
  if (!strcmp(name, "g")) return W.g; if (!strcmp(name, "hookg")) return W.hookg; if (!strcmp(name, "dqkv")) return W.sc[0].dqkv;
  if (!strcmp(name, "dt")) return W.dt; if (!strcmp(name, "dxp")) return W.dxp;
  return -1;
}

static int check_video(const char* who, const nv_vit_config* cfg, int B, const long* shape5, const nv_vit_input* in, bool allow_4d) {
  if (in && in->time_points > 0) {
    NV_CHECK_ARG(allow_4d, "%s: the fused 4D input form is forward-only", who);
    NV_CHECK_ARG(shape5[0] * shape5[4] == B && shape5[4] == in->time_points && shape5[1] == cfg->image_size && shape5[2] == img_w(cfg) && shape5[3] == cfg->frames &&
                     B % in->time_points == 0 && cfg->channels == 1,
                 "%s: 4D input is [%ld,%ld,%ld,%ld,%ld], expected [B/T, %d, %d, %d, T=%d] with B = %d", who, shape5[0], shape5[1], shape5[2], shape5[3],
                 shape5[4], cfg->image_size, img_w(cfg), cfg->frames, in->time_points, B);
    return NV_OK;
  }
  NV_CHECK_ARG(shape5[0] == B && shape5[1] == cfg->channels && shape5[2] == cfg->frames && shape5[3] == cfg->image_size && shape5[4] == img_w(cfg),
               "%s: video is [%ld,%ld,%ld,%ld,%ld], the model was built for [%d,%d,%d,%d,%d] (B, channels, frames, height, width)", who,
               shape5[0], shape5[1], shape5[2], shape5[3], shape5[4], B, cfg->channels, cfg->frames, cfg->image_size, img_w(cfg));
  return NV_OK;
}

static int embed_front16(const nv_vit_config* cfg, const Layout& Y, int B, const float* video, const long* strides5, const nv_vit_input* in, const float* p,
                         const r16* p16, char* ws, unsigned long emb_seed, float emb_drop_p, void* stream) {
  const Dims& D = Y.D; const ParamTab& T = Y.T; const WS& W = Y.W;
  const float eps = cfg->ln_eps;
  const int d = D.d;
  float* pst = (float*)(ws + W.pst);
  const float* sigma = in ? in->vol_sigma : nullptr;
  if (in && in->time_points > 0)
    RUN(nv_patch_ln_fwd_4d(video, B / in->time_points, cfg->image_size, img_w(cfg), cfg->frames, in->time_points, cfg->image_patch_size,
                           pat_w(cfg), cfg->frame_patch_size, p + T.pe_g, p + T.pe_b, eps, ws + W.xp, D.Ppad, pst, pst + D.T, sigma, stream));
  else
    RUN(nv_patch_ln_fwd(video, strides5, B, cfg->channels, cfg->frames, cfg->image_size, img_w(cfg), cfg->image_patch_size,
                        pat_w(cfg), cfg->frame_patch_size, p + T.pe_g, p + T.pe_b, eps, ws + W.xp, D.Ppad, pst, pst + D.T, sigma, stream));
  const void* wpe = p16 + T.pe_w;
  if (D.P != D.Ppad) {
    RUN(nv_cast_bf16_2d(p + T.pe_w, D.P, d, D.P, ws + W.wpe16, D.Ppad, stream));
    wpe = ws + W.wpe16;
  }
  RUN(nv_gemm_bf16(0, 2, D.T, d, D.Ppad, ws + W.xp, D.Ppad, wpe, D.Ppad, ws + W.t, d, p + T.pe_bias, nullptr, 0, nullptr, 0, 0, 1.f, 0, 0.f, stream));
  float* est = (float*)(ws + W.est);
  return nv_embed_finish_fwd((float*)(ws + W.t), d, B, D.N, d, p + T.pe_g2, p + T.pe_b2, eps, p + T.pos, p + T.cls, (float*)(ws + W.x0), d, est,
                             est + D.T, emb_seed, emb_drop_p, stream);
}

static int cls_rows_block16(const Dims& D, const LayerP& q, const LayerW& w, int l, const float* p, const r16* p16, char* ws, float eps, const float* xin,
                            float* x1, float* x2, float* st2, void* u, unsigned long drop_seed, float drop_p, float proj_p, void* stream, const float* sd = nullptr) {
  const int B = D.B, d = D.d;
  const long rs = D.n;
  RUN(nv_skinny_nt_path(0, B, d, D.inner, ws + w.ao, D.inner * rs, p16 + q.wo, D.inner, p + q.bo, xin, d * rs, x1, d * rs, nullptr, 0, site_seed(drop_seed, 4 * l + 1), proj_p, stream,
                        path_of(sd, l, 0, B), D.n));
  RUN(nv_ln_fwd(x1, d * rs, B, d, p + q.n2g, p + q.n2b, eps, ws + w.xn2, d * rs, st2, st2 + D.M, stream));
  RUN(nv_skinny_nt(1, B, D.m, d, ws + w.xn2, d * rs, p16 + q.w1, d, p + q.b1, nullptr, 0, ws + w.h, D.m * rs, u, D.m * rs, site_seed(drop_seed, 4 * l + 2), drop_p, stream));
  return nv_skinny_nt_path(0, B, d, D.m, ws + w.h, D.m * rs, p16 + q.w2, D.m, p + q.b2, x1, d * rs, x2, d * rs, nullptr, 0, site_seed(drop_seed, 4 * l + 3), drop_p, stream,
                           path_of(sd, l, 1, B), D.n);
}

static int pool_head(const Dims& D, const ParamTab& T, const float* p, float eps, const float* xin, char* ws, long xm, long xh, long hst, float* logits,
                     void* stream) {
  const float* pooled = xin;
  long pooled_stride = (long)D.n * D.d;
  if (D.pool_mean) {
    RUN(nv_token_mean(xin, D.B, D.n, D.d, (float*)(ws + xm), stream));
    pooled = (float*)(ws + xm); pooled_stride = D.d;
  }
  return nv_head_fwd(pooled, pooled_stride, D.B, D.d, p + T.hg, p + T.hb, eps, p + T.hw, p + T.hbias, D.C, (float*)(ws + xh), (float*)(ws + hst), logits, stream);
}

extern "C" int nv_vit_forward(const nv_vit_config* cfg, int B, const float* video, const long* shape5, const long* strides5,
                              const float* params, const void* params16, void* workspace, long ws_bytes, int training, float drop_p, float emb_drop_p,
                              unsigned long drop_seed, float* logits, void* stream) {
  return nv_vit_forward_in(cfg, B, video, shape5, strides5, nullptr, params, params16, workspace, ws_bytes, training, drop_p, emb_drop_p, drop_seed, logits, stream);
}

static const nv_vit_attn_export* attn_export_of(const nv_vit_input* in) { return in ? in->attn_export : nullptr; }
static int check_attn_export(const nv_vit_input* in, const char* who) {
  const nv_vit_attn_export* ex = attn_export_of(in);
  if (!ex) return NV_OK;
  NV_CHECK_ARG(ex->struct_size == (int)sizeof(nv_vit_attn_export), "%s: nv_vit_attn_export.struct_size=%d, expected %d (ABI revision %d)", who,
               ex->struct_size, (int)sizeof(nv_vit_attn_export), NV_ABI_VERSION);
  NV_CHECK_ARG(ex->maps, "%s: nv_vit_attn_export.maps is NULL", who);
  NV_CHECK_ARG(ex->fusion >= NV_ATTN_PER_HEAD && ex->fusion <= NV_ATTN_FUSE_MIN && (ex->rows == NV_ATTN_ROWS_ALL || ex->rows == NV_ATTN_ROWS_CLS),
               "%s: nv_vit_attn_export fusion=%d / rows=%d out of range", who, ex->fusion, ex->rows);
  return NV_OK;
}
static int export_layer(const nv_vit_input* in, int l, int qkv_f32, const void* qkv, const Dims& D, int B, float scale, void* stream) {
  const nv_vit_attn_export* ex = attn_export_of(in);
  if (!ex || !ex->maps[l]) return NV_OK;
  return nv_attn_probs(qkv_f32, qkv, 3L * D.inner, B, D.n, D.heads, D.dh, scale, ex->fusion, ex->rows, ex->maps[l], stream);
}

static int forward_in_impl(const Layout& Y, const nv_vit_config* cfg, int B, const float* video, const long* shape5, const long* strides5, const nv_vit_input* in,
                           const float* params, const void* params16, void* workspace, long ws_bytes, int training, float drop_p, float emb_drop_p,
                           unsigned long drop_seed, float* logits, void* stream, bool skip_head, const void* fold16 = nullptr, const float* fold32 = nullptr,
                           const float* sd = nullptr);

extern "C" long nv_vit_lnfold_floats(const nv_vit_config* cfg) {
  Dims D; if (make_dims(cfg, 1, D)) return -1;
  return (long)D.L * (6L * D.inner + 2L * D.m);
}
extern "C" int nv_vit_lnfold_prepare(const nv_vit_config* cfg, const float* params, void* fold16, float* fold32, void* stream) {
  Dims D; RUN(make_dims(cfg, 1, D));
  ParamTab T; make_params(D, T);
  NV_CHECK_ARG(params && fold16 && fold32 && nv_aligned16(params) && nv_aligned16(fold16) && nv_aligned16(fold32), "nv_vit_lnfold_prepare: null / unaligned arena");
  r16* f16 = (r16*)fold16;
  const long per = 6L * D.inner + 2L * D.m;
  for (int l = 0; l < D.L; ++l) {
    const LayerP& q = T.layer[l];
    float* f = fold32 + l * per;
    RUN(nv_ln_fold_weight(params + q.wqkv, D.d, 3 * D.inner, D.d, params + q.n1g, params + q.n1b, nullptr, f16 + q.wqkv, D.d, f, f + 3L * D.inner, stream));
    RUN(nv_ln_fold_weight(params + q.w1, D.d, D.m, D.d, params + q.n2g, params + q.n2b, params + q.b1, f16 + q.w1, D.d, f + 6L * D.inner, f + 6L * D.inner + D.m, stream));
  }
  return NV_OK;
}
extern "C" int nv_vit_forward_lnfold(const nv_vit_config* cfg, int B, const float* video, const long* shape5, const long* strides5, const nv_vit_input* in,
                                     const float* params, const void* params16, const void* fold16, const float* fold32, void* workspace, long ws_bytes,
                                     float* logits, void* stream) {
  NV_CHECK_ARG(fold16 && fold32 && nv_aligned16(fold16) && nv_aligned16(fold32), "nv_vit_forward_lnfold: null / unaligned fold arenas (nv_vit_lnfold_prepare)");
  Layout Y; RUN(make_layout(cfg, B, 0, Y));
  return forward_in_impl(Y, cfg, B, video, shape5, strides5, in, params, params16, workspace, ws_bytes, 0, 0.f, 0.f, 0, logits, stream, false, fold16, fold32);
}

extern "C" int nv_vit_forward_in(const nv_vit_config* cfg, int B, const float* video, const long* shape5, const long* strides5, const nv_vit_input* in,
                                 const float* params, const void* params16, void* workspace, long ws_bytes, int training, float drop_p, float emb_drop_p,
                                 unsigned long drop_seed, float* logits, void* stream) {
  Layout Y; RUN(make_layout(cfg, B, training, Y));
  return forward_in_impl(Y, cfg, B, video, shape5, strides5, in, params, params16, workspace, ws_bytes, training, drop_p, emb_drop_p, drop_seed, logits, stream, false);
}

extern "C" int nv_vit_forward_sd(const nv_vit_config* cfg, int B, const float* video, const long* shape5, const long* strides5, const nv_vit_input* in,
                                 const float* params, const void* params16, void* workspace, long ws_bytes, int training, float drop_p, float emb_drop_p,
                                 unsigned long drop_seed, float* logits, void* stream, const nv_vit_drop_path* sd) {
  if (!sd) return nv_vit_forward_in(cfg, B, video, shape5, strides5, in, params, params16, workspace, ws_bytes, training, drop_p, emb_drop_p, drop_seed, logits, stream);
  RUN(check_drop_path(sd, "nv_vit_forward_sd"));
  NV_CHECK_ARG(training == 1, "nv_vit_forward_sd: stochastic depth belongs to training forwards (training = %d)", training);
  NV_CHECK_ARG(!(in && in->time_points > 0), "nv_vit_forward_sd: not with the fused 4D input form (time_points > 0)");
  Layout Y; RUN(make_layout(cfg, B, 1, Y));
  return forward_in_impl(Y, cfg, B, video, shape5, strides5, in, params, params16, workspace, ws_bytes, 1, drop_p, emb_drop_p, drop_seed, logits, stream, false, nullptr, nullptr,
                         sd->factors);
}

static int forward_in_impl(const Layout& Y, const nv_vit_config* cfg, int B, const float* video, const long* shape5, const long* strides5, const nv_vit_input* in,
                           const float* params, const void* params16, void* workspace, long ws_bytes, int training, float drop_p, float emb_drop_p,
                           unsigned long drop_seed, float* logits, void* stream, bool skip_head, const void* fold16, const float* fold32, const float* sd) {
  const Dims& D = Y.D; const ParamTab& T = Y.T; const WS& W = Y.W;
  NV_CHECK_ARG(video && shape5 && strides5 && params && params16 && workspace && logits, "nv_vit_forward: null pointer");
  RUN(check_video("nv_vit_forward", cfg, B, shape5, in, true));
  NV_CHECK_ARG(ws_bytes >= W.total, "nv_vit_forward: workspace too small (%ld < %ld)", ws_bytes, W.total);
  NV_CHECK_ARG(((uintptr_t)workspace & 255) == 0 && nv_aligned16(params) && nv_aligned16(params16), "nv_vit_forward: alignment");
  RUN(check_attn_export(in, "nv_vit_forward"));
  char* ws = (char*)workspace;
  const float* p = params;
  const r16* p16 = (const r16*)params16;
  const float eps = cfg->ln_eps;
  const int M = D.M, d = D.d;

  RUN(embed_front16(cfg, Y, B, video, strides5, in, p, p16, ws, site_seed(drop_seed, 4 * D.L), emb_drop_p, stream));
  const float scale = 1.0f / sqrtf((float)D.dh);
  const float* xin = (float*)(ws + W.x0);
  const bool tail = cls_tail_wanted(D, training, drop_p, in ? in->rows_form : 0);
  const bool fold = fold16 && fold32 && !training && drop_p == 0.f && M <= 12288 && nv_gemm_lnfold_supported(M, 3 * D.inner, d) && nv_gemm_lnfold_supported(M, D.m, d) &&
                    nv_gemm_lnfold_supported(M, d, D.inner) && nv_gemm_lnfold_supported(M, d, D.m);
  const r16* f16 = (const r16*)fold16;
  const long fper = 6L * D.inner + 2L * D.m;
  float* fst1 = (float*)(ws + W.fst1);
  float* fst2 = (float*)(ws + W.fst2);
  bool have_in16 = false;
  for (int l = 0; l < D.L; ++l) {
    const LayerP& q = T.layer[l];
    const LayerW& w = W.layer[l];
    const float* ff = fold ? fold32 + l * fper : nullptr;
    float* x1 = (float*)(ws + w.x1);
    float* x2 = (float*)(ws + ((!training && (l & 1)) ? W.x0 : w.x2));
    float* st1 = (float*)(ws + w.st1);
    float* st2 = (float*)(ws + w.st2);
    if (have_in16) {
      RUN(nv_gemm_lnfold(0, M, 3 * D.inner, d, ws + w.xn1, d, f16 + q.wqkv, d, fst1, ff, ff + 3L * D.inner, eps, ws + w.qkv, 3 * D.inner, stream));
    } else {
      RUN(nv_ln_fwd(xin, d, M, d, p + q.n1g, p + q.n1b, eps, ws + w.xn1, d, st1, st1 + M, stream));
      RUN(nv_gemm_bf16(0, 0, M, 3 * D.inner, d, ws + w.xn1, d, p16 + q.wqkv, d, ws + w.qkv, 3 * D.inner, nullptr, nullptr, 0, nullptr, 0, 0, 1.f, 0, 0.f, stream));
    }
    have_in16 = false;
    RUN(nv_attn_fwd(ws + w.qkv, 3 * D.inner, B, D.n, D.heads, D.dh, scale, ws + w.ao, D.inner, (float*)(ws + w.lse), site_seed(drop_seed, 4 * l + 0), drop_p, stream));
    RUN(export_layer(in, l, 0, ws + w.qkv, D, B, scale, stream));
    if (tail && l == D.L - 1) {
      RUN(cls_rows_block16(D, q, w, l, p, p16, ws, eps, xin, x1, x2, st2, training ? ws + w.u : nullptr, drop_seed, drop_p, proj_drop_p(cfg, drop_p), stream, sd));
      xin = x2;
      continue;
    }
    if (fold) {
      RUN(nv_gemm_resid_ln(M, d, D.inner, ws + w.ao, D.inner, p16 + q.wo, D.inner, p + q.bo, xin, d, x1, d, ws + w.xn2, d, fst2, stream));
      RUN(nv_gemm_lnfold(1, M, D.m, d, ws + w.xn2, d, f16 + q.w1, d, fst2, ff + 6L * D.inner, ff + 6L * D.inner + D.m, eps, ws + w.h, D.m, stream));
      const bool next_folds = l + 1 <= D.L - 2;
      if (next_folds) {
        RUN(nv_gemm_resid_ln(M, d, D.m, ws + w.h, D.m, p16 + q.w2, D.m, p + q.b2, x1, d, x2, d, ws + W.layer[l + 1].xn1, d, fst1, stream));
        have_in16 = true;
      } else {
        RUN(nv_gemm_bf16(0, 4, M, d, D.m, ws + w.h, D.m, p16 + q.w2, D.m, x2, d, p + q.b2, x1, d, nullptr, 0, 0, 1.f, 0, 0.f, stream));
      }
      xin = x2;
      continue;
    }
    RUN(nv_gemm_bf16_path(0, 4, M, d, D.inner, ws + w.ao, D.inner, p16 + q.wo, D.inner, x1, d, p + q.bo, xin, d, nullptr, 0, 0, 1.f, site_seed(drop_seed, 4 * l + 1), proj_drop_p(cfg, drop_p), stream,
                          path_of(sd, l, 0, B), D.n));
    RUN(nv_ln_fwd(x1, d, M, d, p + q.n2g, p + q.n2b, eps, ws + w.xn2, d, st2, st2 + M, stream));
    RUN(nv_gemm_bf16(0, 3, M, D.m, d, ws + w.xn2, d, p16 + q.w1, d, ws + w.h, D.m, p + q.b1, nullptr, 0, training ? ws + w.u : nullptr, D.m, 0, 1.f, site_seed(drop_seed, 4 * l + 2), drop_p, stream));
    RUN(nv_gemm_bf16_path(0, 4, M, d, D.m, ws + w.h, D.m, p16 + q.w2, D.m, x2, d, p + q.b2, x1, d, nullptr, 0, 0, 1.f, site_seed(drop_seed, 4 * l + 3), drop_p, stream,
                          path_of(sd, l, 1, B), D.n));
    xin = x2;
  }
  if (skip_head) return NV_OK;
  return pool_head(D, T, p, eps, xin, ws, W.xm, W.xh, W.hst, logits, stream);
}

extern "C" int nv_vit_forward_f32(const nv_vit_config* cfg, int B, const float* video, const long* shape5, const long* strides5, const nv_vit_input* in,
                                  const float* params, void* workspace, long ws_bytes, float* logits, void* stream) {
  Dims D; RUN(make_dims(cfg, B, D));
  ParamTab T; make_params(D, T);
  WSF W; make_wsf(D, W);
  NV_CHECK_ARG(video && shape5 && strides5 && params && workspace && logits, "nv_vit_forward_f32: null pointer");
  RUN(check_video("nv_vit_forward_f32", cfg, B, shape5, in, true));
  NV_CHECK_ARG(ws_bytes >= W.total, "nv_vit_forward_f32: workspace too small (%ld < %ld)", ws_bytes, W.total);
  NV_CHECK_ARG(((uintptr_t)workspace & 255) == 0 && nv_aligned16(params), "nv_vit_forward_f32: alignment");
  RUN(check_attn_export(in, "nv_vit_forward_f32"));
  char* ws = (char*)workspace;
  const float* p = params;
  const float eps = cfg->ln_eps;
  const int M = D.M, d = D.d;
  auto F32 = [&](long off) -> float* { return (float*)(ws + off); };

  float* pst = F32(W.pst);
  const float* sigma = in ? in->vol_sigma : nullptr;
  if (in && in->time_points > 0)
    RUN(nv_patch_ln_fwd_4d_f32(video, B / in->time_points, cfg->image_size, img_w(cfg), cfg->frames, in->time_points, cfg->image_patch_size,
                               pat_w(cfg), cfg->frame_patch_size, p + T.pe_g, p + T.pe_b, eps, F32(W.xp), D.P, pst, pst + D.T, sigma, stream));
  else
    RUN(nv_patch_ln_fwd_f32(video, strides5, B, cfg->channels, cfg->frames, cfg->image_size, img_w(cfg), cfg->image_patch_size,
                            pat_w(cfg), cfg->frame_patch_size, p + T.pe_g, p + T.pe_b, eps, F32(W.xp), D.P, pst, pst + D.T, sigma, stream));
  RUN(nv_gemm_f32(2, D.T, d, D.P, F32(W.xp), D.P, p + T.pe_w, D.P, F32(W.t), d, p + T.pe_bias, nullptr, 0, stream));
  float* est = F32(W.est);
  RUN(nv_embed_finish_fwd(F32(W.t), d, B, D.N, d, p + T.pe_g2, p + T.pe_b2, eps, p + T.pos, p + T.cls, F32(W.x0), d, est, est + D.T, 0, 0.f, stream));
  const float scale = 1.0f / sqrtf((float)D.dh);
  const float* xin = F32(W.x0);
  const bool tail = cls_tail_wanted(D, 0, 0.f, in ? in->rows_form : 0);
  for (int l = 0; l < D.L; ++l) {
    const LayerP& q = T.layer[l];
    float* x1 = F32(W.x1);
    float* x2 = F32((l & 1) ? W.x0 : W.x2);
    RUN(nv_ln_fwd_f32(xin, d, M, d, p + q.n1g, p + q.n1b, eps, F32(W.xn1), d, nullptr, nullptr, stream));
    RUN(nv_gemm_f32(0, M, 3 * D.inner, d, F32(W.xn1), d, p + q.wqkv, d, F32(W.qkv), 3 * D.inner, nullptr, nullptr, 0, stream));
    RUN(nv_attn_fwd_f32(F32(W.qkv), 3 * D.inner, B, D.n, D.heads, D.dh, scale, F32(W.ao), D.inner, stream));
    RUN(export_layer(in, l, 1, F32(W.qkv), D, B, scale, stream));
    const bool cls_rows = tail && l == D.L - 1;
    const int Mr = cls_rows ? B : M;
    const long rs = cls_rows ? (long)D.n : 1;
    RUN(nv_gemm_f32(4, Mr, d, D.inner, F32(W.ao), D.inner * rs, p + q.wo, D.inner, x1, d * rs, p + q.bo, xin, d * rs, stream));
    RUN(nv_ln_fwd_f32(x1, d * rs, Mr, d, p + q.n2g, p + q.n2b, eps, F32(W.xn2), d * rs, nullptr, nullptr, stream));
    RUN(nv_gemm_f32(3, Mr, D.m, d, F32(W.xn2), d * rs, p + q.w1, d, F32(W.h), D.m * rs, p + q.b1, nullptr, 0, stream));
    RUN(nv_gemm_f32(4, Mr, d, D.m, F32(W.h), D.m * rs, p + q.w2, D.m, x2, d * rs, p + q.b2, x1, d * rs, stream));
    xin = x2;
  }
  return pool_head(D, T, p, eps, xin, ws, W.xm, W.xh, W.hst, logits, stream);
}

extern "C" long nv_vit_fp8_scale_count(const nv_vit_config* cfg) {
  Dims D; if (make_dims(cfg, 1, D)) return -1;
  return (long)D.L * (3L * D.inner + D.m + 2L * D.d);
}

// ... 30 lines not shown
  NV_CHECK_ARG(ws_bytes >= W.total, "nv_vit_forward_fp8: workspace too small (%ld < %ld)", ws_bytes, W.total);
  NV_CHECK_ARG(D.d % 128 == 0 && D.m % 128 == 0, "nv_vit_forward_fp8: dim and mlp_dim must be multiples of 128");
  NV_CHECK_ARG(((uintptr_t)workspace & 255) == 0 && nv_aligned16(params) && nv_aligned16(params16) && nv_aligned16(params8), "nv_vit_forward_fp8: alignment");
  NV_CHECK_ARG(!attn_export_of(in), "nv_vit_forward_fp8: no attention-probability export on the fp8 path");
  char* ws = (char*)workspace;
  const float* p = params;
  const r16* p16 = (const r16*)params16;
  const char* p8 = (const char*)params8;
  const float eps = cfg->ln_eps;
  const int M = D.M, d = D.d;
  const long per = 3L * D.inner + D.m + 2L * D.d;

  RUN(embed_front16(cfg, Y, B, video, strides5, in, p, p16, ws, 0, 0.f, stream));
  const float scale = 1.0f / sqrtf((float)D.dh);
  const float* xin = (float*)(ws + W.x0);
  const bool tail8 = cls_tail_wanted(D, 0, 0.f, in ? in->rows_form : 0);
  for (int l = 0; l < D.L; ++l) {
    const LayerP& q = T.layer[l];
    const LayerW& w = W.layer[l];
    const float* cs = colscales + l * per;
    const float s_xn1 = act_scales[4 * l], s_xn2 = act_scales[4 * l + 1], s_h = act_scales[4 * l + 2], s_ao = act_scales[4 * l + 3];
    const bool tail_here = tail8 && l == D.L - 1;
    const bool ao8 = !tail_here && D.dh == 64 && s_ao > 0.f && D.inner % 128 == 0;
    float* x1 = (float*)(ws + w.x1);
    float* x2 = (float*)(ws + ((l & 1) ? W.x0 : w.x2));
    RUN(nv_ln_fwd_f8(xin, d, M, d, p + q.n1g, p + q.n1b, eps, s_xn1, ws + w.xn1, d, stream));
    RUN(nv_gemm_f8(0, M, 3 * D.inner, d, ws + w.xn1, d, p8 + q.wqkv, d, ws + w.qkv, 3 * D.inner, cs, nullptr, nullptr, 0, 1.f, stream));
    if (ao8) RUN(nv_attn_fwd_o8(ws + w.qkv, 3 * D.inner, B, D.n, D.heads, D.dh, scale, ws + w.ao, D.inner, s_ao, stream));
    else RUN(nv_attn_fwd(ws + w.qkv, 3 * D.inner, B, D.n, D.heads, D.dh, scale, ws + w.ao, D.inner, (float*)(ws + w.lse), 0, 0.f, stream));
    if (tail_here) {
      RUN(cls_rows_block16(D, q, w, l, p, p16, ws, eps, xin, x1, x2, (float*)(ws + w.st2), nullptr, 0, 0.f, 0.f, stream));
      xin = x2;
      continue;
    }
    if (ao8) RUN(nv_gemm_f8(4, M, d, D.inner, ws + w.ao, D.inner, p8 + q.wo, D.inner, x1, d, cs + 3L * D.inner + D.m + D.d, p + q.bo, xin, d, 1.f, stream));
    else RUN(nv_gemm_bf16(0, 4, M, d, D.inner, ws + w.ao, D.inner, p16 + q.wo, D.inner, x1, d, p + q.bo, xin, d, nullptr, 0, 0, 1.f, 0, 0.f, stream));
    RUN(nv_ln_fwd_f8(x1, d, M, d, p + q.n2g, p + q.n2b, eps, s_xn2, ws + w.xn2, d, stream));
    RUN(nv_gemm_f8(7, M, D.m, d, ws + w.xn2, d, p8 + q.w1, d, ws + w.h, D.m, cs + 3L * D.inner, p + q.b1, nullptr, 0, s_h, stream));
    RUN(nv_gemm_f8(4, M, d, D.m, ws + w.h, D.m, p8 + q.w2, D.m, x2, d, cs + 3L * D.inner + D.m, p + q.b2, x1, d, 1.f, stream));
    xin = x2;
  }
  return pool_head(D, T, p, eps, xin, ws, W.xm, W.xh, W.hst, logits, stream);
}

extern "C" int nv_vit_forward_fp8_train(const nv_vit_config* cfg, int B, const float* video, const long* shape5, const long* strides5, const nv_vit_input* in,
                                        const float* params, const void* params16, const void* params8, const float* colscales, const float* act_scales,
                                        void* workspace, long ws_bytes, float drop_p, float emb_drop_p, unsigned long drop_seed, float* logits, void* stream) {
  Layout Y; RUN(make_layout(cfg, B, 1, Y));
  const Dims& D = Y.D; const ParamTab& T = Y.T; const WS& W = Y.W;
  NV_CHECK_ARG(video && shape5 && strides5 && params && params16 && params8 && colscales && act_scales && workspace && logits, "nv_vit_forward_fp8_train: null pointer");
  RUN(check_video("nv_vit_forward_fp8_train", cfg, B, shape5, in, false));
  NV_CHECK_ARG(ws_bytes >= W.total, "nv_vit_forward_fp8_train: workspace too small (%ld < %ld): the training layout is needed", ws_bytes, W.total);
  NV_CHECK_ARG(D.d % 128 == 0 && D.m % 128 == 0, "nv_vit_forward_fp8_train: dim and mlp_dim must be multiples of 128 (got %d, %d)", D.d, D.m);
  NV_CHECK_ARG(((uintptr_t)workspace & 255) == 0 && nv_aligned16(params) && nv_aligned16(params16) && nv_aligned16(params8), "nv_vit_forward_fp8_train: alignment");
  NV_CHECK_ARG(!attn_export_of(in), "nv_vit_forward_fp8_train: no attention-probability export on the fp8 path");
  char* ws = (char*)workspace;
  const float* p = params;
  const r16* p16 = (const r16*)params16;
  const char* p8 = (const char*)params8;
  const float eps = cfg->ln_eps;
  const int M = D.M, d = D.d;
  const long per = 3L * D.inner + D.m + 2L * D.d;

  RUN(embed_front16(cfg, Y, B, video, strides5, in, p, p16, ws, site_seed(drop_seed, 4 * D.L), emb_drop_p, stream));
  const float scale = 1.0f / sqrtf((float)D.dh);
  const float* xin = (float*)(ws + W.x0);
  const bool tail = cls_tail_wanted(D, 1, drop_p, in ? in->rows_form : 0);
  void* x8 = ws + W.f8x;
  void* h8 = ws + W.f8h;
  for (int l = 0; l < D.L; ++l) {
    const LayerP& q = T.layer[l];
    const LayerW& w = W.layer[l];
    const float* cs = colscales + l * per;
    const float s_xn1 = act_scales[4 * l], s_xn2 = act_scales[4 * l + 1], s_h = act_scales[4 * l + 2];
    NV_CHECK_ARG(s_xn1 > 0.f && s_xn2 > 0.f && s_h > 0.f, "nv_vit_forward_fp8_train: activation scales of layer %d must be positive", l);
    float* x1 = (float*)(ws + w.x1);
    float* x2 = (float*)(ws + w.x2);
    float* st1 = (float*)(ws + w.st1);
    float* st2 = (float*)(ws + w.st2);
    RUN(nv_ln_fwd_f8_train(xin, d, M, d, p + q.n1g, p + q.n1b, eps, s_xn1, x8, d, ws + w.xn1, d, st1, st1 + M, stream));
    RUN(nv_gemm_f8(0, M, 3 * D.inner, d, x8, d, p8 + q.wqkv, d, ws + w.qkv, 3 * D.inner, cs, nullptr, nullptr, 0, 1.f, stream));
    RUN(nv_attn_fwd(ws + w.qkv, 3 * D.inner, B, D.n, D.heads, D.dh, scale, ws + w.ao, D.inner, (float*)(ws + w.lse), site_seed(drop_seed, 4 * l + 0), drop_p, stream));
    if (tail && l == D.L - 1) {
      RUN(cls_rows_block16(D, q, w, l, p, p16, ws, eps, xin, x1, x2, st2, ws + w.u, drop_seed, drop_p, proj_drop_p(cfg, drop_p), stream));
      xin = x2;
      continue;
    }
    RUN(nv_gemm_bf16(0, 4, M, d, D.inner, ws + w.ao, D.inner, p16 + q.wo, D.inner, x1, d, p + q.bo, xin, d, nullptr, 0, 0, 1.f, site_seed(drop_seed, 4 * l + 1), proj_drop_p(cfg, drop_p), stream));
    RUN(nv_ln_fwd_f8_train(x1, d, M, d, p + q.n2g, p + q.n2b, eps, s_xn2, x8, d, ws + w.xn2, d, st2, st2 + M, stream));
    RUN(nv_gemm_f8_gelu_train(M, D.m, d, x8, d, p8 + q.w1, d, cs + 3L * D.inner, p + q.b1, s_h, h8, D.m, ws + w.h, D.m, ws + w.u, D.m,
                              site_seed(drop_seed, 4 * l + 2), drop_p, stream));
    RUN(nv_gemm_f8_resid_drop(M, d, D.m, h8, D.m, p8 + q.w2, D.m, x2, d, cs + 3L * D.inner + D.m, p + q.b2, x1, d, site_seed(drop_seed, 4 * l + 3), drop_p, stream));
    xin = x2;
  }
  return pool_head(D, T, p, eps, xin, ws, W.xm, W.xh, W.hst, logits, stream);
}

namespace {

struct BwdCall {
  const float* video; const long* strides5; const float* params; const void* params16; void* workspace; long ws_bytes; const float* dlogits;
  float* grads; void* grads16;
  int accumulate, first_stage, last_stage; float drop_p, emb_drop_p; unsigned long drop_seed; void* stream; void* aux_stream; int join_aux, rows_form;
  const nv_adamw_arena* fuse; int fuse_mode;
  const nv_vit_backward_opts* opts;
  const nv_vit_attn_grad_export* attn_grad;
  const float* dtokens;
  const float* sd;
};

struct BwdLayer { int l; bool tail; int Mr; long rs; };

struct Bwd {
  const nv_vit_config* cfg; const BwdCall& c; const Dims& D; const ParamTab& T; const WS& W;
  char* ws; const float* p; const r16* p16; float* g;
  bool wg, tail_fwd;
  int M, d, acc, du_tile_rows;
  float scale;
  hipStream_t S, A;
  float* GR(long off) const { return c.grads ? c.grads + off : nullptr; }
  void* M16(long off) const { return c.grads16 ? (void*)((r16*)c.grads16 + off) : nullptr; }
  float* dxn1(int l) const { return (float*)(ws + (l == D.L - 1 ? W.hookg : W.dxn)); }

  int bwd_head() const {
    const float* xlast = (float*)(ws + W.layer[D.L - 1].x2);
    return nv_head_bwd_path(c.dlogits, D.B, D.C, p + T.hw, D.pool_mean ? (const float*)(ws + W.xm) : xlast, D.pool_mean ? (long)d : (long)D.n * d,
                       (float*)(ws + W.hst), (float*)(ws + W.xh), p + T.hg, d, D.n, g, d, ws + W.scratch(D.L - 1).g16, d,
                       GR(T.hg), GR(T.hb), GR(T.hw), GR(T.hbias), GR(T.layer[D.L - 1].b2), acc, ws + W.sc[0].red, W.red_bytes,
                       site_seed(c.drop_seed, 4 * (D.L - 1) + 3), c.drop_p, D.pool_mean, S, path_of(c.sd, D.L - 1, 1, D.B), D.n);
  }

  int bwd_ffn(const BwdLayer& R) const {
    const int l = R.l; const long rs = R.rs;
    const LayerP& q = T.layer[l]; const LayerW& w = W.layer[l]; const LayerScratch& sc = W.scratch(l);
    float* dxn = (float*)(ws + W.dxn); float* st2 = (float*)(ws + w.st2);
    void* g16 = ws + sc.g16; void* du = ws + sc.du;
    if (R.tail) {
      RUN(nv_skinny_nn(0, D.B, D.m, d, g16, d * rs, p16 + q.w2, D.m, ws + w.u, D.m * rs, du, D.m * rs, GR(q.b1), acc, site_seed(c.drop_seed, 4 * l + 2), c.drop_p, S));
      RUN(nv_skinny_nn(1, D.B, d, D.m, du, D.m * rs, p16 + q.w1, d, nullptr, 0, dxn, d * rs, nullptr, 0, 0, 0.f, S));
    } else {
      RUN(nv_gemm_bf16(1, du_tile_rows ? 6 : 5, M, D.m, d, g16, d, p16 + q.w2, D.m, du, D.m, nullptr, ws + w.u, D.m, du_tile_rows ? (float*)(ws + sc.cs1) : nullptr, D.m, 0, 1.f,
                       site_seed(c.drop_seed, 4 * l + 2), c.drop_p, S));
      RUN(nv_gemm_bf16(1, 1, M, d, D.m, du, D.m, p16 + q.w1, d, dxn, d, nullptr, nullptr, 0, nullptr, 0, 0, 1.f, 0, 0.f, S));
    }
    return nv_ln_bwd_path(dxn, d * rs, (float*)(ws + w.x1), d * rs, st2, st2 + M, p + q.n2g, R.Mr, d, g, g, d * rs, ws + sc.g16b, d * rs, GR(q.n2g), GR(q.n2b), GR(q.bo), acc, ws + sc.red,
                          W.red_bytes, site_seed(c.drop_seed, 4 * l + 1), proj_drop_p(cfg, c.drop_p), S, NV_LN_NO_REDUCE, path_of(c.sd, l, 0, D.B), D.n);
  }

  int bwd_attn(const BwdLayer& R) const {
    const int l = R.l;
    const LayerP& q = T.layer[l]; const LayerW& w = W.layer[l]; const LayerScratch& sc = W.scratch(l);
    if (R.tail)
      RUN(nv_skinny_nn_sparse(D.B, D.inner, d, ws + sc.g16b, d * R.rs, p16 + q.wo, D.inner, ws + W.dao, M, D.n, S));
    else
      RUN(nv_gemm_bf16(1, 0, M, D.inner, d, ws + sc.g16b, d, p16 + q.wo, D.inner, ws + W.dao, D.inner, nullptr, nullptr, 0, nullptr, 0, 0, 1.f, 0, 0.f, S));
    RUN(nv_attn_bwd(ws + w.qkv, 3 * D.inner, ws + w.ao, ws + W.dao, D.inner, (float*)(ws + w.lse), D.B, D.n, D.heads, D.dh, scale,
                    (float*)(ws + W.delta), ws + sc.dqkv, 3 * D.inner, site_seed(c.drop_seed, 4 * l + 0), c.drop_p, S));
    if (c.attn_grad && c.attn_grad->maps[l])
      RUN(nv_attn_grad(ws + w.qkv, 3 * D.inner, ws + W.dao, D.inner, D.B, D.n, D.heads, D.dh, scale, c.attn_grad->form, c.attn_grad->maps[l], S));
    return NV_OK;
  }

  int bwd_dxn1(int l) const {
    return nv_gemm_bf16(1, 1, M, d, 3 * D.inner, ws + W.scratch(l).dqkv, 3 * D.inner, p16 + T.layer[l].wqkv, d, dxn1(l), d, nullptr, nullptr, 0, nullptr, 0, 0, 1.f, 0, 0.f, S);
  }

  int bwd_ln1(int l) const {
    const LayerP& q = T.layer[l];
    const float* xin = (l == 0) ? (float*)(ws + W.x0) : (float*)(ws + W.layer[l - 1].x2);
    float* st1 = (float*)(ws + W.layer[l].st1);
    return nv_ln_bwd_path(dxn1(l), d, xin, d, st1, st1 + M, p + q.n1g, M, d, g, g, d, ws + W.scratch(l - 1).g16, d, GR(q.n1g), GR(q.n1b), (l > 0) ? GR(T.layer[l - 1].b2) : nullptr,
                          acc, ws + W.scratch(l).red3, nv_ln_bwd_workspace_bytes(M, d), site_seed(c.drop_seed, 4 * (l - 1) + 3), (l > 0) ? c.drop_p : 0.f, S, NV_LN_NO_REDUCE,
                          (l > 0) ? path_of(c.sd, l - 1, 1, D.B) : nullptr, D.n);
  }

  int bwd_reduce_ln1(int lp) const {
    const LayerP& qp = T.layer[lp];
    return nv_ln_bwd_reduce(ws + W.scratch(lp).red3, M, d, GR(qp.n1g), GR(qp.n1b), (lp > 0) ? GR(T.layer[lp - 1].b2) : nullptr, acc, A);
  }

  int bwd_layer_update(int lu) const {
    const LinearW lw = linear_weights(D, T.layer[lu]);
    const long b[3] = {lw.off[0], lw.off[2], lw.off[3]};
    const long n[3] = {align_up(lw.numel[0], 8) + lw.numel[1], lw.numel[2], lw.numel[3]};
    return nv_adamw_ranges(c.fuse, b, n, 3, A);
  }

  int bwd_layer_params(const BwdLayer& R, int ln1_of) const {
    const int l = R.l, Mr = R.Mr; const long rs = R.rs;
    const LayerP& q = T.layer[l]; const LayerW& w = W.layer[l]; const LayerScratch& sc = W.scratch(l);
    void* g16 = ws + sc.g16; void* g16b = ws + sc.g16b; void* du = ws + sc.du; void* dqkv = ws + sc.dqkv;
    nv_reduce_job jobs[3];
    int nj = 0;
    if (R.tail) {}
    else if (du_tile_rows) jobs[nj++] = {(float*)(ws + sc.cs1), (M + du_tile_rows - 1) / du_tile_rows, D.m, 1, {GR(q.b1), nullptr, nullptr}, acc};
    else RUN(nv_colsum_bf16(du, D.m, M, D.m, GR(q.b1), acc, ws + sc.red2, W.red2_bytes, A));
    jobs[nj++] = {(const float*)(ws + sc.red), nv_ln_bwd_partial_rows(Mr), d, 3, {GR(q.n2g), GR(q.n2b), GR(q.bo)}, acc};
    if (ln1_of >= 0) {
      const LayerP& qp = T.layer[ln1_of];
      jobs[nj++] = {(const float*)(ws + W.scratch(ln1_of).red3), nv_ln_bwd_partial_rows(M), d, 3, {GR(qp.n1g), GR(qp.n1b), (ln1_of > 0) ? GR(T.layer[ln1_of - 1].b2) : nullptr}, acc};
    }
    RUN(nv_reduce_multi(jobs, nj, A));
    nv_gemm_problem pr[4];
    pr[0] = {d, D.m, Mr, g16, d * rs, ws + w.h, D.m * rs, GR(q.w2), D.m, acc, M16(q.w2), D.m};
    pr[1] = {D.m, d, Mr, du, D.m * rs, ws + w.xn2, d * rs, GR(q.w1), d, acc, M16(q.w1), d};
    pr[2] = {d, D.inner, Mr, g16b, d * rs, ws + w.ao, D.inner * rs, GR(q.wo), D.inner, acc, M16(q.wo), D.inner};
    pr[3] = {3 * D.inner, d, M, dqkv, 3 * D.inner, ws + w.xn1, d, GR(q.wqkv), d, acc, M16(q.wqkv), d};
    if (c.fuse && c.fuse_mode != 3) return nv_gemm_bf16_grouped_adamw(4, pr, c.fuse, A);
    return nv_gemm_bf16_grouped(2, 1, 4, pr, A);
  }

  int bwd_embed_tokens() const {
    float* est = (float*)(ws + W.est);
    return nv_embed_finish_bwd(g, d, (float*)(ws + W.t), d, est, est + D.T, p + T.pe_g2, D.B, D.N, d, (float*)(ws + W.dt), d, ws + W.dt16, d, GR(T.pe_g2),
                               GR(T.pe_b2), GR(T.pe_bias), GR(T.pos), GR(T.cls), acc, ws + W.sc[1].red, W.red_bytes, site_seed(c.drop_seed, 4 * D.L), c.emb_drop_p, S);
  }

  int bwd_embed() const {
    float* pst = (float*)(ws + W.pst);
    float* const dvideo = c.opts ? c.opts->dvideo : nullptr;
    const void* wpe = (D.P != D.Ppad) ? (const void*)(ws + W.wpe16) : (const void*)(p16 + T.pe_w);
    void* redA = ws + (A != S ? W.sc[0].red2 : W.sc[0].red);
    const long redA_bytes = A != S ? W.red2_bytes : W.red_bytes;
    RUN(nv_gemm_bf16(1, 1, D.T, D.Ppad, d, ws + W.dt16, d, wpe, D.Ppad, ws + W.dxp, D.Ppad, nullptr, nullptr, 0, nullptr, 0, 0, 1.f, 0, 0.f, A));
    if (dvideo)
      RUN(nv_patch_ln_dx(c.video, c.strides5, D.B, cfg->channels, cfg->frames, cfg->image_size, img_w(cfg), cfg->image_patch_size, pat_w(cfg), cfg->frame_patch_size,
                         (const float*)(ws + W.dxp), D.Ppad, pst, pst + D.T, p + T.pe_g, dvideo, c.opts->dvideo_strides5, A));
    if (!wg) return NV_OK;
    RUN(nv_patch_ln_bwd(c.video, c.strides5, D.B, cfg->channels, cfg->frames, cfg->image_size, img_w(cfg), cfg->image_patch_size,
                        pat_w(cfg), cfg->frame_patch_size, (float*)(ws + W.dxp), D.Ppad, pst, pst + D.T, GR(T.pe_g), GR(T.pe_b), acc, redA, redA_bytes, A));
    if (D.P != D.Ppad) {
      RUN(nv_gemm_bf16(2, 1, d, D.Ppad, D.T, ws + W.dt16, d, ws + W.xp, D.Ppad, ws + W.dwpe, D.Ppad, nullptr, nullptr, 0, nullptr, 0, 0, 1.f, 0, 0.f, S));
      return nv_copy_2d_f32((float*)(ws + W.dwpe), D.Ppad, d, D.P, GR(T.pe_w), D.P, acc, S);
    }
    return nv_gemm_bf16(2, 1, d, D.P, D.T, ws + W.dt16, d, ws + W.xp, D.Ppad, GR(T.pe_w), D.P, nullptr, nullptr, 0, M16(T.pe_w), D.P, acc, 1.f, 0, 0.f, S);
  }
};


int seed_tokens(const Bwd& X) {
// ... 367 lines not shown
```

neurovit_amd/csrc/norm.hip:

```cpp
#include "common.h"

#define WAVES_PER_BLOCK 4

#include <type_traits>
template <typename OT>
__device__ __forceinline__ void store4(OT* p, const f32x4& o) {
  if constexpr (std::is_same<OT, float>::value) *reinterpret_cast<f32x4*>(p) = o;
  else *reinterpret_cast<r16x4*>(p) = cvt4<OT>(o[0], o[1], o[2], o[3]);
}
__device__ __forceinline__ r16 cvt1_rt(float v, int fp16) { return fp16 ? cvt1<fp16_t>(v) : cvt1<bf16_t>(v); }

template <int NV>
__device__ __forceinline__ void row_load(const float* row, int d, int lane, f32x4 (&x)[NV]) {
#pragma unroll
  for (int v = 0; v < NV; ++v) {
    const int c = (lane + 64 * v) * 4;
    x[v] = (c < d) ? *reinterpret_cast<const f32x4*>(row + c) : f32x4{0.f, 0.f, 0.f, 0.f};
  }
}
template <int NV>
__device__ __forceinline__ void row_stats(const f32x4 (&x)[NV], int d, int lane, float eps, float& mean, float& rstd) {
  float s = 0.f;
#pragma unroll
  for (int v = 0; v < NV; ++v) s += (x[v][0] + x[v][1]) + (x[v][2] + x[v][3]);
  mean = wave_sum(s) / (float)d;
  float q = 0.f;
#pragma unroll
  for (int v = 0; v < NV; ++v) {
    const int c = (lane + 64 * v) * 4;
    if (c < d) {
      const f32x4 t = x[v] - mean;
      q += (t[0] * t[0] + t[1] * t[1]) + (t[2] * t[2] + t[3] * t[3]);
    }
  }
  rstd = 1.0f / sqrtf(wave_sum(q) / (float)d + eps);
}

template <int NV, typename OT>
__global__ __launch_bounds__(256) void ln_fwd_kernel(const float* __restrict__ x, long ldx, int M, int d, const float* __restrict__ gamma,
                                                     const float* __restrict__ beta, float eps, OT* __restrict__ y, long ldy,
                                                     float* __restrict__ mean_out, float* __restrict__ rstd_out) {
  const int lane = threadIdx.x & 63, row = blockIdx.x * WAVES_PER_BLOCK + (threadIdx.x >> 6);
  if (row >= M) return;
  f32x4 xv[NV];
  row_load<NV>(x + (long)row * ldx, d, lane, xv);
  float mean, rstd;
  row_stats<NV>(xv, d, lane, eps, mean, rstd);
#pragma unroll
  for (int v = 0; v < NV; ++v) {
    const int c = (lane + 64 * v) * 4;
    if (c < d) {
      const f32x4 gm = *reinterpret_cast<const f32x4*>(gamma + c), bt = *reinterpret_cast<const f32x4*>(beta + c);
      const f32x4 o = (xv[v] - mean) * rstd * gm + bt;
      store4<OT>(y + (long)row * ldy + c, o);
    }
  }
  if (lane == 0 && mean_out) {
    mean_out[row] = mean;
    rstd_out[row] = rstd;
  }
}

extern "C" int nv_ln_fwd(const float* x, long ldx, int M, int d, const float* gamma, const float* beta, float eps, void* y,
                         long ldy, float* mean, float* rstd, void* stream) {
  NV_CHECK_ARG(M > 0 && d > 0 && (d % 4) == 0 && d <= 2048, "nv_ln_fwd: d=%d must be a multiple of 4 and <= 2048", d);
  NV_CHECK_ARG((ldx % 4) == 0 && (ldy % 4) == 0 && nv_aligned16(x) && nv_aligned16(y) && nv_aligned16(gamma) && nv_aligned16(beta),
               "nv_ln_fwd: alignment");
  const dim3 grid((M + WAVES_PER_BLOCK - 1) / WAVES_PER_BLOCK), block(256);
  hipStream_t s = (hipStream_t)stream;
  NV_DISPATCH_OPERAND(T,
    if (d <= 1024) hipLaunchKernelGGL((ln_fwd_kernel<4, T>), grid, block, 0, s, x, ldx, M, d, gamma, beta, eps, (T*)y, ldy, mean, rstd);
    else hipLaunchKernelGGL((ln_fwd_kernel<8, T>), grid, block, 0, s, x, ldx, M, d, gamma, beta, eps, (T*)y, ldy, mean, rstd));
  NV_CHECK_LAUNCH("nv_ln_fwd");
  return NV_OK;
}

extern "C" int nv_ln_fwd_f32(const float* x, long ldx, int M, int d, const float* gamma, const float* beta, float eps, float* y,
                             long ldy, float* mean, float* rstd, void* stream) {
  NV_CHECK_ARG(M > 0 && d > 0 && (d % 4) == 0 && d <= 2048, "nv_ln_fwd_f32: d=%d must be a multiple of 4 and <= 2048", d);
  NV_CHECK_ARG((ldx % 4) == 0 && (ldy % 4) == 0 && nv_aligned16(x) && nv_aligned16(y) && nv_aligned16(gamma) && nv_aligned16(beta) && (!mean == !rstd),
               "nv_ln_fwd_f32: alignment");
  const dim3 grid((M + WAVES_PER_BLOCK - 1) / WAVES_PER_BLOCK), block(256);
  hipStream_t s = (hipStream_t)stream;
  if (d <= 1024) hipLaunchKernelGGL((ln_fwd_kernel<4, float>), grid, block, 0, s, x, ldx, M, d, gamma, beta, eps, y, ldy, mean, rstd);
  else hipLaunchKernelGGL((ln_fwd_kernel<8, float>), grid, block, 0, s, x, ldx, M, d, gamma, beta, eps, y, ldy, mean, rstd);
  NV_CHECK_LAUNCH("nv_ln_fwd_f32");
  return NV_OK;
}

template <bool PATH> using HeadPath = std::conditional_t<PATH, const float*, NoPath>;
template <int NV, int ROWS, typename T, bool PATH>
__global__ __launch_bounds__(256) void ln_bwd_kernel(const float* __restrict__ dy, long lddy, const float* __restrict__ x, long ldx,
                                                     const float* __restrict__ mean_in, const float* __restrict__ rstd_in,
                                                     const float* __restrict__ gamma, int M, int d, const float* g_in, float* g_out,
                                                     long ldg, r16* __restrict__ g16, long ldg16, float* __restrict__ partials,
                                                     DropCfg drop, int seg_rows, int seg_skip, PathArg<PATH> path) {
  extern __shared__ __attribute__((aligned(16))) float red[];
  const int lane = threadIdx.x & 63, wid = threadIdx.x >> 6;
  const int nw = gridDim.x * WAVES_PER_BLOCK;
  f32x4 gm[NV], a_g[NV], a_b[NV], a_c[NV];
#pragma unroll
  for (int v = 0; v < NV; ++v) {
    const int c = (lane + 64 * v) * 4;
    gm[v] = (c < d) ? *reinterpret_cast<const f32x4*>(gamma + c) : f32x4{0.f, 0.f, 0.f, 0.f};
    a_g[v] = a_b[v] = a_c[v] = f32x4{0.f, 0.f, 0.f, 0.f};
  }
  for (int base = blockIdx.x * WAVES_PER_BLOCK + wid; base < M; base += ROWS * nw) {
    f32x4 xv[ROWS][NV], dv[ROWS][NV], gi[ROWS][NV];
    float mean[ROWS], rstd[ROWS];
#pragma unroll
    for (int r = 0; r < ROWS; ++r) {
      const int row = base + r * nw;
      const int rr = row < M ? row : base;
      row_load<NV>(x + (long)rr * ldx, d, lane, xv[r]);
      const long dyr = seg_rows ? (long)rr + (long)(rr / seg_rows) * seg_skip : (long)rr;
      row_load<NV>(dy + dyr * lddy, d, lane, dv[r]);
      if (g_in) row_load<NV>(g_in + (long)rr * ldg, d, lane, gi[r]);
      mean[r] = mean_in[rr]; rstd[r] = rstd_in[rr];
    }
#pragma unroll
    for (int r = 0; r < ROWS; ++r) {
      const int row = base + r * nw;
      if (row < M) {
        [[maybe_unused]] float pf = 1.f;
        if constexpr (PATH) pf = path_factor(path, row);
        float s1 = 0.f, s2 = 0.f;
#pragma unroll
        for (int v = 0; v < NV; ++v) {
          xv[r][v] = (xv[r][v] - mean[r]) * rstd[r];
          const f32x4 dyh = dv[r][v] * gm[v];
          s1 += (dyh[0] + dyh[1]) + (dyh[2] + dyh[3]);
          const f32x4 t = dyh * xv[r][v];
          s2 += (t[0] + t[1]) + (t[2] + t[3]);
          a_g[v] += dv[r][v] * xv[r][v];
          a_b[v] += dv[r][v];
        }
        const float c1 = wave_sum(s1) / (float)d, c2 = wave_sum(s2) / (float)d;
#pragma unroll
        for (int v = 0; v < NV; ++v) {
// ... 1282 lines not shown
```

neurovit_amd/csrc/skinny.hip:

```cpp
#include "common.h"

namespace {

constexpr int SK_R = 4;

enum { SK_NT_RESID = 0, SK_NT_GELU = 1 };
enum { SK_NN_DGELU = 0, SK_NN_F32 = 1, SK_NN_BF16 = 2 };

template <int EPI, typename T, bool PATH>
__global__ __launch_bounds__(256) void skinny_nt_kernel(const r16* __restrict__ A, long lda, int R, const r16* __restrict__ W, long ldw, int N, int K,
                                                        const float* __restrict__ bias, const float* __restrict__ resid, long ldr,
                                                        void* __restrict__ out, long ldo, r16* __restrict__ u_out, long ldu, DropCfg drop, PathArg<PATH> path) {
  const int lane = threadIdx.x & 63, n = blockIdx.x * 4 + (threadIdx.x >> 6);
  const int r0 = blockIdx.y * SK_R, rows = (R - r0 < SK_R) ? R - r0 : SK_R;
  if (n >= N) return;
  float acc[SK_R];
#pragma unroll
  for (int r = 0; r < SK_R; ++r) acc[r] = 0.f;
  const r16* w = W + (long)n * ldw;
  for (int k = lane * 8; k < K; k += 4 * 512) {
    r16x8 wq[4], aq[4][SK_R];
#pragma unroll
    for (int q = 0; q < 4; ++q) {
      const int kq = k + 512 * q;
      if (kq < K) {
        wq[q] = *reinterpret_cast<const r16x8*>(w + kq);
#pragma unroll
        for (int r = 0; r < SK_R; ++r)
          if (r < rows) aq[q][r] = *reinterpret_cast<const r16x8*>(A + (long)(r0 + r) * lda + kq);
      }
    }
#pragma unroll
    for (int q = 0; q < 4; ++q) {
      if (k + 512 * q < K) {
#pragma unroll
        for (int r = 0; r < SK_R; ++r) {
          if (r < rows) {
#pragma unroll
            for (int e = 0; e < 8; ++e) acc[r] = __builtin_fmaf(dec1<T>(aq[q][r][e]), dec1<T>(wq[q][e]), acc[r]);
          }
        }
      }
    }
  }
  float mine = 0.f;
#pragma unroll
  for (int r = 0; r < SK_R; ++r) {
    if (r < rows) {
      const float t = wave_sum(acc[r]);
      if (lane == r) mine = t;
    }
  }
  if (lane < rows) {
    const long row = r0 + lane;
    const float v = mine + bias[n];
    float keep = drop.thresh ? drop_factor(drop, (unsigned long long)(row * ldo + n)) : 1.f;
    if constexpr (PATH) keep *= path_factor(path, (int)row);
    if constexpr (EPI == SK_NT_RESID) {
      ((float*)out)[row * ldo + n] = v * keep + resid[row * ldr + n];
    } else {
      if (u_out) u_out[row * ldu + n] = cvt1<T>(v);
      ((r16*)out)[row * ldo + n] = cvt1<T>(gelu_f(v) * keep);
    }
  }
}

constexpr int NN_COLS = 16;
constexpr int NN_KK = 64 / (NN_COLS / 8);

template <int EPI, typename T>
__global__ __launch_bounds__(1024) void skinny_nn_kernel(const r16* __restrict__ A, long lda, int R, const r16* __restrict__ W, long ldw, int N, int K,
                                                         const r16* __restrict__ u, long ldu, void* __restrict__ out, long ldo,
                                                         float* __restrict__ dcol, int accumulate, long fill_rows, int keep_every, DropCfg drop) {
  extern __shared__ __attribute__((aligned(16))) float sk_lds[];
  if (blockIdx.z == 1) {
    zero_rows_except(reinterpret_cast<char*>(out), fill_rows, (long)N * 2, keep_every, blockIdx.y * gridDim.x + blockIdx.x, gridDim.x * gridDim.y);
    return;
  }
  float (*part)[NN_KK][SK_R][NN_COLS] = reinterpret_cast<float (*)[NN_KK][SK_R][NN_COLS]>(sk_lds);
  float (*red)[SK_R][NN_COLS] = reinterpret_cast<float (*)[SK_R][NN_COLS]>(sk_lds + 16 * NN_KK * SK_R * NN_COLS);
  const int tid = threadIdx.x, lane = tid & 63, wv = tid >> 6, ng = lane & (NN_COLS / 8 - 1), kk = lane / (NN_COLS / 8);
  const int n0 = blockIdx.x * NN_COLS, nc = n0 + ng * 8;
  const int r0 = blockIdx.y * SK_R, rows = (R - r0 < SK_R) ? R - r0 : SK_R;
  float acc[SK_R][8];
#pragma unroll
  for (int r = 0; r < SK_R; ++r)
#pragma unroll
    for (int e = 0; e < 8; ++e) acc[r][e] = 0.f;
  if (nc < N) {
    constexpr int STEP = 16 * NN_KK;
    for (int k = wv * NN_KK + kk; k < K; k += 4 * STEP) {
      r16x8 wq[4];
      float aq[4][SK_R];
#pragma unroll
      for (int q = 0; q < 4; ++q) {
        const int kq = k + STEP * q;
        if (kq < K) {
          wq[q] = *reinterpret_cast<const r16x8*>(W + (long)kq * ldw + nc);
#pragma unroll
          for (int r = 0; r < SK_R; ++r)
            if (r < rows) aq[q][r] = dec1<T>(A[(long)(r0 + r) * lda + kq]);
        }
      }
#pragma unroll
      for (int q = 0; q < 4; ++q) {
        if (k + STEP * q < K) {
#pragma unroll
          for (int r = 0; r < SK_R; ++r) {
            if (r < rows) {
#pragma unroll
              for (int e = 0; e < 8; ++e) acc[r][e] = __builtin_fmaf(aq[q][r], dec1<T>(wq[q][e]), acc[r][e]);
            }
          }
        }
      }
    }
  }
#pragma unroll
  for (int r = 0; r < SK_R; ++r) {
    *reinterpret_cast<f32x4*>(&part[wv][kk][r][ng * 8]) = f32x4{acc[r][0], acc[r][1], acc[r][2], acc[r][3]};
    *reinterpret_cast<f32x4*>(&part[wv][kk][r][ng * 8 + 4]) = f32x4{acc[r][4], acc[r][5], acc[r][6], acc[r][7]};
  }
  __syncthreads();
  {
    const int w = tid / (SK_R * NN_COLS), rc = tid % (SK_R * NN_COLS);
    float v = 0.f;
#pragma unroll
    for (int q = 0; q < NN_KK; ++q) v += part[w][q][rc / NN_COLS][rc % NN_COLS];
    red[w][rc / NN_COLS][rc % NN_COLS] = v;
  }
  __syncthreads();
  const int c = tid % NN_COLS, r = tid / NN_COLS;
  float stored = 0.f;
  const bool live = r < rows && n0 + c < N;
  if (live) {
    float v = 0.f;
#pragma unroll
    for (int w = 0; w < 16; ++w) v += red[w][r][c];
    const long row = r0 + r;
    const int n = n0 + c;
    if constexpr (EPI == SK_NN_DGELU) {
      const float keep = drop.thresh ? drop_factor(drop, (unsigned long long)(row * ldo + n)) : 1.f;
      const r16 o = cvt1<T>(v * keep * gelu_grad_f(dec1<T>(u[row * ldu + n])));
      ((r16*)out)[row * ldo + n] = o;
      stored = dec1<T>(o);
    } else if constexpr (EPI == SK_NN_F32) {
      ((float*)out)[row * ldo + n] = v;
    } else {
      ((r16*)out)[row * ldo + n] = cvt1<T>(v);
    }
  }
  if constexpr (EPI == SK_NN_DGELU) {
    if (dcol) {
      __syncthreads();
      if (r < SK_R) red[0][r][c] = live ? stored : 0.f;
      __syncthreads();
      if (r == 0 && n0 + c < N) {
        float s = 0.f;
#pragma unroll
        for (int q = 0; q < SK_R; ++q) s += red[0][q][c];
        dcol[n0 + c] = (accumulate ? dcol[n0 + c] : 0.f) + s;
      }
    }
  }
}

constexpr int NN_LDS = (16 * NN_KK * SK_R * NN_COLS + 16 * SK_R * NN_COLS) * (int)sizeof(float);
template <typename T>
void nn_attrs_fmt() {
  (void)hipFuncSetAttribute(reinterpret_cast<const void*>(skinny_nn_kernel<SK_NN_DGELU, T>), hipFuncAttributeMaxDynamicSharedMemorySize, NN_LDS);
  (void)hipFuncSetAttribute(reinterpret_cast<const void*>(skinny_nn_kernel<SK_NN_F32, T>), hipFuncAttributeMaxDynamicSharedMemorySize, NN_LDS);
  (void)hipFuncSetAttribute(reinterpret_cast<const void*>(skinny_nn_kernel<SK_NN_BF16, T>), hipFuncAttributeMaxDynamicSharedMemorySize, NN_LDS);
}
void nn_attrs() {
  static bool attr = false;
  if (attr) return;
  nn_attrs_fmt<bf16_t>(); nn_attrs_fmt<fp16_t>();
  attr = true;
}

}

extern "C" int nv_skinny_nt(int epi, int R, int N, int K, const void* A, long lda, const void* W, long ldw, const float* bias, const float* resid,
                            long ldr, void* out, long ldo, void* u_out, long ldu, unsigned long drop_seed, float drop_p, void* stream) {
  NV_CHECK_ARG(drop_p == 0.f || (ldo % N) == 0, "nv_skinny_nt: with dropout `out` must be a row-strided view of a dense [M, N] tensor (ldo a multiple of N)");
  const DropCfg drop = make_drop(drop_seed, drop_p);
  NV_CHECK_ARG(R > 0 && N > 0 && K > 0 && (K % 8) == 0 && (lda % 8) == 0 && (ldw % 8) == 0 && A && W && bias && out && nv_aligned16(A) && nv_aligned16(W),
               "nv_skinny_nt: K, lda, ldw must be multiples of 8, operands 16-byte aligned");
  NV_CHECK_ARG(epi == SK_NT_GELU || (epi == SK_NT_RESID && resid), "nv_skinny_nt: epilogue 0 needs resid; epilogues are 0 (bias + residual, f32) and 1 (bias + GELU, bf16)");
  const dim3 grid((N + 3) / 4, (R + SK_R - 1) / SK_R), block(256);
  hipStream_t s = (hipStream_t)stream;
  NV_DISPATCH_OPERAND(T,
    if (epi == SK_NT_RESID)
      hipLaunchKernelGGL((skinny_nt_kernel<SK_NT_RESID, T, false>), grid, block, 0, s, (const r16*)A, lda, R, (const r16*)W, ldw, N, K, bias, resid, ldr, out, ldo, (r16*)nullptr, 0L, drop, NoPath{});
    else
      hipLaunchKernelGGL((skinny_nt_kernel<SK_NT_GELU, T, false>), grid, block, 0, s, (const r16*)A, lda, R, (const r16*)W, ldw, N, K, bias, resid, ldr, out, ldo, (r16*)u_out, ldu, drop, NoPath{}));
  NV_CHECK_LAUNCH("nv_skinny_nt");
  return NV_OK;
}

extern "C" int nv_skinny_nt_path(int epi, int R, int N, int K, const void* A, long lda, const void* W, long ldw, const float* bias, const float* resid,
                                 long ldr, void* out, long ldo, void* u_out, long ldu, unsigned long drop_seed, float drop_p, void* stream, const float* path,
                                 int path_rows) {
  if (!path) return nv_skinny_nt(epi, R, N, K, A, lda, W, ldw, bias, resid, ldr, out, ldo, u_out, ldu, drop_seed, drop_p, stream);
  NV_CHECK_ARG(epi == SK_NT_RESID && resid, "nv_skinny_nt_path: a factor table goes with epilogue 0 (bias + residual) only, got %d", epi);
  NV_CHECK_ARG(R > 0 && N > 0 && K > 0 && (K % 8) == 0 && (lda % 8) == 0 && (ldw % 8) == 0 && A && W && bias && out && nv_aligned16(A) && nv_aligned16(W),
               "nv_skinny_nt_path: K, lda, ldw must be multiples of 8, operands 16-byte aligned");
  NV_CHECK_ARG(path_rows > 0 && nv_aligned(path, 4) && ldo >= N && (ldo % N) == 0 && (long)R * (ldo / N) < (1L << 31),
               "nv_skinny_nt_path: path_rows = %d must be positive and `out` a row-strided view of a dense [M, N] tensor (ldo a multiple of N)", path_rows);
  const DropCfg drop = make_drop(drop_seed, drop_p);
  const PathCfg pc{path, path_rows, (int)(ldo / N)};
  const dim3 grid((N + 3) / 4, (R + SK_R - 1) / SK_R), block(256);
  NV_DISPATCH_OPERAND(T, hipLaunchKernelGGL((skinny_nt_kernel<SK_NT_RESID, T, true>), grid, block, 0, (hipStream_t)stream, (const r16*)A, lda, R, (const r16*)W, ldw, N, K, bias,
                                            resid, ldr, out, ldo, (r16*)nullptr, 0L, drop, pc));
  NV_CHECK_LAUNCH("nv_skinny_nt_path");
  return NV_OK;
}

extern "C" int nv_skinny_nn(int epi, int R, int N, int K, const void* A, long lda, const void* W, long ldw, const void* u, long ldu, void* out, long ldo,
                            float* dcol, int accumulate, unsigned long drop_seed, float drop_p, void* stream) {
  NV_CHECK_ARG(drop_p == 0.f || (epi == SK_NN_DGELU && (ldo % N) == 0), "nv_skinny_nn: dropout only with epilogue 0, `out` a row-strided view of a dense [M, N] tensor");
  const DropCfg drop = make_drop(drop_seed, drop_p);
  NV_CHECK_ARG(R > 0 && N > 0 && K > 0 && (N % 8) == 0 && (ldw % 8) == 0 && A && W && out && nv_aligned16(W), "nv_skinny_nn: N, ldw must be multiples of 8, W 16-byte aligned");
  NV_CHECK_ARG(epi >= 0 && epi <= 2 && (epi != SK_NN_DGELU || u) && (!dcol || (epi == SK_NN_DGELU && R <= SK_R)), "nv_skinny_nn: epilogue 0 needs u; column sums only with epilogue 0 and R <= 4");
  const dim3 grid((N + NN_COLS - 1) / NN_COLS, (R + SK_R - 1) / SK_R), block(1024);
  hipStream_t s = (hipStream_t)stream;
  nn_attrs();
#define SK_NN(E) hipLaunchKernelGGL((skinny_nn_kernel<E, T>), grid, block, NN_LDS, s, (const r16*)A, lda, R, (const r16*)W, ldw, N, K, (const r16*)u, ldu, out, ldo, dcol, accumulate, 0L, 0, drop)
  NV_DISPATCH_OPERAND(T, if (epi == SK_NN_DGELU) SK_NN(SK_NN_DGELU); else if (epi == SK_NN_F32) SK_NN(SK_NN_F32); else SK_NN(SK_NN_BF16));
#undef SK_NN
  NV_CHECK_LAUNCH("nv_skinny_nn");
  return NV_OK;
}

extern "C" int nv_skinny_nn_sparse(int R, int N, int K, const void* A, long lda, const void* W, long ldw, void* out, long total_rows, int keep_every,
                                   void* stream) {
  NV_CHECK_ARG(R > 0 && N > 0 && K > 0 && (N % 8) == 0 && (ldw % 8) == 0 && A && W && out && nv_aligned16(W) && nv_aligned16(out) && keep_every >= 1 &&
                   (long)(R - 1) * keep_every < total_rows && (long)R * keep_every >= total_rows,
               "nv_skinny_nn_sparse: N, ldw multiples of 8; W, out 16-byte aligned; R = ceil(total_rows / keep_every) (every kept row is computed: the fill skips them all)");
  const dim3 grid((N + NN_COLS - 1) / NN_COLS, (R + SK_R - 1) / SK_R, 2), block(1024);
  nn_attrs();
  NV_DISPATCH_OPERAND(T, hipLaunchKernelGGL((skinny_nn_kernel<SK_NN_BF16, T>), grid, block, NN_LDS, (hipStream_t)stream, (const r16*)A, lda, R, (const r16*)W, ldw, N, K,
                                            (const r16*)nullptr, 0L, out, (long)N * keep_every, (float*)nullptr, 0, total_rows, keep_every, make_drop(0, 0.f)));
  NV_CHECK_LAUNCH("nv_skinny_nn_sparse");
  return NV_OK;
}
```

neurovit_amd/ops.py:

```python
from __future__ import annotations

import ctypes
from typing import Optional, Tuple

import torch

from . import _cabi
from ._cabi import check, lib


def op16() -> torch.dtype:
    return torch.float16 if _cabi.operand_format() == "fp16" else torch.bfloat16


NT, NN, TN = 0, 1, 2
EPI_STORE_BF16, EPI_STORE_F32, EPI_BIAS_F32, EPI_BIAS_GELU, EPI_BIAS_RESID, EPI_DGELU, EPI_DGELU_COLSUM = 0, 1, 2, 3, 4, 5, 6


def _stream() -> int:
    return torch.cuda.current_stream().cuda_stream


def _p(t: Optional[torch.Tensor]):
    return None if t is None else t.data_ptr()


def _need_cuda(*ts):
    for t in ts:
        if t is not None and not t.is_cuda:
            raise RuntimeError("neurovit_amd ops run on MI355X only (got a CPU tensor); there is no CPU fallback")


def shape5(video: torch.Tensor):
    assert video.dim() == 5
    return (ctypes.c_long * 5)(*video.shape)


def cast_ranges_bf16(src: torch.Tensor, dst: torch.Tensor, ranges) -> None:
    _need_cuda(src, dst)
    assert src.dtype == torch.float32 and dst.dtype == op16() and src.dim() == 1 and dst.numel() >= src.numel()
    ranges = [(int(b), int(e)) for b, e in ranges if e > b]
    if not ranges:
        return
    begins = (ctypes.c_long * len(ranges))(*[b for b, _ in ranges])
    lens = (ctypes.c_long * len(ranges))(*[e - b for b, e in ranges])
    check(lib.nv_cast_ranges_bf16(_p(src), _p(dst), begins, lens, len(ranges), _stream()), "nv_cast_ranges_bf16")


NO_PATH = object()


def _path_call(name: str, path, path_rows: int):
    if path is NO_PATH:
        return getattr(lib, name), ()
    return getattr(lib, name + "_path"), (_p(path), int(path_rows))


def skinny_nt(epi: int, A: torch.Tensor, W: torch.Tensor, bias: torch.Tensor, out: torch.Tensor, resid: Optional[torch.Tensor] = None,
              u_out: Optional[torch.Tensor] = None, drop_seed: int = 0, drop_p: float = 0.0, path=NO_PATH, path_rows: int = 0) -> torch.Tensor:
    _need_cuda(A, W)
    R, K = A.shape
    N = W.shape[0]
    fn, tail = _path_call("nv_skinny_nt", path, path_rows)
    check(fn(epi, R, N, K, _p(A), A.stride(0), _p(W), W.stride(0), _p(bias), _p(resid), 0 if resid is None else resid.stride(0),
             _p(out), out.stride(0), _p(u_out), 0 if u_out is None else u_out.stride(0), int(drop_seed), float(drop_p), _stream(), *tail), "nv_skinny_nt")
    return out


def skinny_nn(epi: int, A: torch.Tensor, W: torch.Tensor, out: torch.Tensor, u: Optional[torch.Tensor] = None,
              dcol: Optional[torch.Tensor] = None, accumulate: bool = False, drop_seed: int = 0, drop_p: float = 0.0) -> torch.Tensor:
    _need_cuda(A, W)
    R, K = A.shape
    N = W.shape[1]
    check(lib.nv_skinny_nn(epi, R, N, K, _p(A), A.stride(0), _p(W), W.stride(0), _p(u), 0 if u is None else u.stride(0), _p(out), out.stride(0),
                           _p(dcol), int(accumulate), int(drop_seed), float(drop_p), _stream()), "nv_skinny_nn")
    return out


def strides5(video: torch.Tensor):
    assert video.dim() == 5
    return (ctypes.c_long * 5)(*video.stride())


def gemm(layout: int, epi: int, A: torch.Tensor, B: torch.Tensor, *, out: Optional[torch.Tensor] = None, bias=None,
         aux_in=None, aux_out=None, accumulate: bool = False, alpha: float = 1.0, drop_seed: int = 0, drop_p: float = 0.0,
         path=NO_PATH, path_rows: int = 0) -> torch.Tensor:
    _need_cuda(A, B)
    assert A.dtype == op16() and B.dtype == op16() and A.stride(1) == 1 and B.stride(1) == 1
    if layout == NT:
        M, K = A.shape; N = B.shape[0]; assert B.shape[1] == K
    elif layout == NN:
        M, K = A.shape; N = B.shape[1]; assert B.shape[0] == K
    else:
        K, M = A.shape; N = B.shape[1]; assert B.shape[0] == K
    odt = op16() if epi in (EPI_STORE_BF16, EPI_BIAS_GELU, EPI_DGELU, EPI_DGELU_COLSUM) else torch.float32
    if out is None:
        out = torch.empty((M, N), dtype=odt, device=A.device)
    assert out.dtype == odt and out.shape == (M, N) and out.stride(1) == 1
    fn, tail = _path_call("nv_gemm_bf16", path, path_rows)
    check(fn(layout, epi, M, N, K, _p(A), A.stride(0), _p(B), B.stride(0), _p(out), out.stride(0), _p(bias),
             _p(aux_in), 0 if aux_in is None else aux_in.stride(0), _p(aux_out),
             0 if aux_out is None else aux_out.stride(0), int(accumulate), float(alpha), drop_seed, drop_p, _stream(), *tail), "nv_gemm_bf16")
    return out


EPI_F32_STORE, EPI_F32_BIAS, EPI_F32_BIAS_GELU, EPI_F32_BIAS_RESID = 0, 2, 3, 4


def gemm_f32(epi: int, A: torch.Tensor, W: torch.Tensor, *, bias=None, resid=None, out: Optional[torch.Tensor] = None) -> torch.Tensor:
    _need_cuda(A, W)
    assert A.dtype == torch.float32 and W.dtype == torch.float32 and A.stride(1) == 1 and W.stride(1) == 1
    M, K = A.shape
    N = W.shape[0]
    assert W.shape[1] == K
    if out is None:
        out = torch.empty((M, N), dtype=torch.float32, device=A.device)
    assert out.dtype == torch.float32 and out.shape == (M, N) and out.stride(1) == 1
    check(lib.nv_gemm_f32(epi, M, N, K, _p(A), A.stride(0), _p(W), W.stride(0), _p(out), out.stride(0), _p(bias), _p(resid),
                          0 if resid is None else resid.stride(0), _stream()), "nv_gemm_f32")
    return out


def attn_fwd_f32(qkv: torch.Tensor, B: int, n: int, heads: int, dim_head: int = 64) -> torch.Tensor:
    _need_cuda(qkv)
    assert qkv.dtype == torch.float32 and qkv.stride(1) == 1
    inner = heads * dim_head
    out = torch.empty((B * n, inner), dtype=torch.float32, device=qkv.device)
    check(lib.nv_attn_fwd_f32(_p(qkv), qkv.stride(0), B, n, heads, dim_head, dim_head ** -0.5, _p(out), inner, _stream()), "nv_attn_fwd_f32")
    return out


def ln_fwd_f32(x: torch.Tensor, gamma, beta, eps: float = 1e-5) -> torch.Tensor:
    _need_cuda(x)
    M, d = x.shape
    y = torch.empty((M, d), dtype=torch.float32, device=x.device)
    check(lib.nv_ln_fwd_f32(_p(x), x.stride(0), M, d, _p(gamma), _p(beta), eps, _p(y), d, None, None, _stream()), "nv_ln_fwd_f32")
    return y


def patch_ln_fwd_f32(video: torch.Tensor, p1: int, p2: int, pf: int, gamma, beta, eps: float = 1e-5, vol_sigma=None):
    _need_cuda(video)
    B, C, F, H, W = video.shape
    P = C * p1 * p2 * pf
    N = (F // pf) * (H // p1) * (W // p2)
    out = torch.empty((B * N, P), dtype=torch.float32, device=video.device)
    st = torch.empty((2, B * N), dtype=torch.float32, device=video.device)
    check(lib.nv_patch_ln_fwd_f32(_p(video), strides5(video), B, C, F, H, W, p1, p2, pf, _p(gamma), _p(beta), eps, _p(out), P, _p(st[0]),
                                  _p(st[1]), _p(vol_sigma), _stream()), "nv_patch_ln_fwd_f32")
    return out, st


class GemmProblem(ctypes.Structure):
    _fields_ = [("M", ctypes.c_int), ("N", ctypes.c_int), ("K", ctypes.c_int), ("A", ctypes.c_void_p), ("lda", ctypes.c_long),
                ("B", ctypes.c_void_p), ("ldb", ctypes.c_long), ("C", ctypes.c_void_p), ("ldc", ctypes.c_long), ("accumulate", ctypes.c_int),
                ("C16", ctypes.c_void_p), ("ldc16", ctypes.c_long)]


def gemm_tn_grouped(problems) -> None:
# ... 106 lines not shown
    dgamma, dbeta, dbias = (torch.empty(d, device=dev) for _ in range(3))
    dpos = torch.empty((N + 1, d), device=dev); dcls = torch.empty(d, device=dev)
    nb = lib.nv_embed_finish_bwd_workspace_bytes(B, N, d)
    ws = torch.empty(nb, dtype=torch.uint8, device=dev)
    g2 = g.reshape(B * (N + 1), d)
    check(lib.nv_embed_finish_bwd(_p(g2), d, _p(t), t.stride(0), _p(st[0]), _p(st[1]), _p(gamma), B, N, d, _p(dt), d, _p(dt16), d, _p(dgamma),
                                  _p(dbeta), _p(dbias), _p(dpos), _p(dcls), 0, _p(ws), nb, drop_seed, drop_p, _stream()), "nv_embed_finish_bwd")
    return dt, dt16, dgamma, dbeta, dbias, dpos, dcls


def attn_fwd(qkv: torch.Tensor, B: int, n: int, heads: int, dim_head: int = 64, drop_seed=0, drop_p=0.0):
    _need_cuda(qkv)
    inner = heads * dim_head
    out = torch.empty((B * n, inner), dtype=op16(), device=qkv.device)
    lse = torch.empty((B, heads, n), dtype=torch.float32, device=qkv.device)
    check(lib.nv_attn_fwd(_p(qkv), qkv.stride(0), B, n, heads, dim_head, dim_head ** -0.5, _p(out), inner, _p(lse), drop_seed, drop_p, _stream()), "nv_attn_fwd")
    return out, lse


def attn_fwd_o8(qkv: torch.Tensor, B: int, n: int, heads: int, out_scale: float, dim_head: int = 64) -> torch.Tensor:
    _need_cuda(qkv)
    inner = heads * dim_head
    out = torch.empty((B * n, inner), dtype=torch.uint8, device=qkv.device)
    check(lib.nv_attn_fwd_o8(_p(qkv), qkv.stride(0), B, n, heads, dim_head, dim_head ** -0.5, _p(out), inner, float(out_scale), _stream()), "nv_attn_fwd_o8")
    return out


def attn_probs(qkv: torch.Tensor, B: int, n: int, heads: int, dim_head: int = 64, head_fusion: Optional[str] = None, rows: str = "all",
               out: Optional[torch.Tensor] = None) -> torch.Tensor:
    _need_cuda(qkv)
    assert qkv.stride(1) == 1 and qkv.dtype in (torch.float32, op16())
    fusion, form = _cabi.ATTN_FUSIONS[head_fusion], _cabi.ATTN_ROWS[rows]
    R = 1 if rows == "cls" else n
    shape = (B, heads, R, n) if head_fusion is None else (B, R, n)
    if out is None:
        out = torch.empty(shape, dtype=torch.float32, device=qkv.device)
    assert out.shape == shape and out.dtype == torch.float32 and out.is_contiguous()
    check(lib.nv_attn_probs(int(qkv.dtype == torch.float32), _p(qkv), qkv.stride(0), B, n, heads, dim_head, dim_head ** -0.5, fusion, form,
                            _p(out), _stream()), "nv_attn_probs")
    return out


def attn_rollout(maps, start_mean: bool = False) -> torch.Tensor:
    _need_cuda(*maps)
    B, n, _ = maps[0].shape
    for m in maps:
        assert m.shape == (B, n, n) and m.dtype == torch.float32 and m.is_contiguous()
    ptrs = (ctypes.c_void_p * len(maps))(*[m.data_ptr() for m in maps])
    nb = lib.nv_attn_rollout_workspace_bytes(B, n)
    ws = torch.empty(nb // 4, dtype=torch.float32, device=maps[0].device)
    out = torch.empty((B, n - 1), dtype=torch.float32, device=maps[0].device)
    check(lib.nv_attn_rollout(ctypes.cast(ptrs, ctypes.c_void_p), len(maps), B, n, int(bool(start_mean)), _p(out), _p(ws), nb, _stream()),
          "nv_attn_rollout")
    return out


def attn_grad(qkv: torch.Tensor, dout: torch.Tensor, B: int, n: int, heads: int, dim_head: int = 64, form: str = "per_head",
              out: Optional[torch.Tensor] = None) -> torch.Tensor:
    _need_cuda(qkv, dout)
    assert qkv.stride(1) == 1 and dout.stride(1) == 1 and qkv.dtype == op16() and dout.dtype == op16()
    shape = (B, heads, n, n) if form == "per_head" else (B, n, n)
    if out is None:
        out = torch.empty(shape, dtype=torch.float32, device=qkv.device)
    assert out.shape == shape and out.dtype == torch.float32 and out.is_contiguous()
    check(lib.nv_attn_grad(_p(qkv), qkv.stride(0), _p(dout), dout.stride(0), B, n, heads, dim_head, dim_head ** -0.5,
                           _cabi.ATTN_GRAD_FORMS[form], _p(out), _stream()), "nv_attn_grad")
    return out


def attn_relevance(maps, start_mean: bool = False) -> torch.Tensor:
    _need_cuda(*maps)
    B, n, _ = maps[0].shape
    for m in maps:
        assert m.shape == (B, n, n) and m.dtype == torch.float32 and m.is_contiguous()
    ptrs = (ctypes.c_void_p * len(maps))(*[m.data_ptr() for m in maps])
    nb = lib.nv_attn_relevance_workspace_bytes(B, n)
    ws = torch.empty(nb // 4, dtype=torch.float32, device=maps[0].device)
    out = torch.empty((B, n - 1), dtype=torch.float32, device=maps[0].device)
    check(lib.nv_attn_relevance(ctypes.cast(ptrs, ctypes.c_void_p), len(maps), B, n, int(bool(start_mean)), _p(out), _p(ws), nb, _stream()),
          "nv_attn_relevance")
    return out


def attn_bwd(qkv, out, dout, lse, B, n, heads, dim_head=64, drop_seed=0, drop_p=0.0):
    inner = heads * dim_head
    dqkv = torch.empty((B * n, 3 * inner), dtype=op16(), device=qkv.device)
    delta = torch.empty((B, heads, n), dtype=torch.float32, device=qkv.device)
    check(lib.nv_attn_bwd(_p(qkv), qkv.stride(0), _p(out), _p(dout), inner, _p(lse), B, n, heads, dim_head, dim_head ** -0.5, _p(delta),
                          _p(dqkv), 3 * inner, drop_seed, drop_p, _stream()), "nv_attn_bwd")
    return dqkv, delta


def head_fwd(x: torch.Tensor, gamma, beta, W, bias, eps=1e-5):
    B, n, d = x.shape
    C = W.shape[0]
    xh = torch.empty((B, d), device=x.device); st = torch.empty((B, 2), device=x.device)
    logits = torch.empty((B, C), device=x.device)
    check(lib.nv_head_fwd(_p(x), n * d, B, d, _p(gamma), _p(beta), eps, _p(W), _p(bias), C, _p(xh), _p(st), _p(logits), _stream()), "nv_head_fwd")
    return logits, xh, st


def head_bwd(dlogits, W, x, st, xh, gamma, drop_seed=0, drop_p=0.0, path=NO_PATH, path_rows: int = 0):
    B, n, d = x.shape
    C = W.shape[0]
    dev = x.device
    g = torch.empty((B, n, d), device=dev); g16 = torch.empty((B, n, d), dtype=op16(), device=dev)
    dgamma, dbeta, dcol = (torch.empty(d, device=dev) for _ in range(3))
    dW = torch.empty((C, d), device=dev); db = torch.empty(C, device=dev)
    nb = lib.nv_head_bwd_workspace_bytes(B, d)
    ws = torch.empty(nb, dtype=torch.uint8, device=dev)
    fn, tail = _path_call("nv_head_bwd", path, path_rows)
    check(fn(_p(dlogits), B, C, _p(W), _p(x), n * d, _p(st), _p(xh), _p(gamma), d, n, _p(g), d, _p(g16), d, _p(dgamma), _p(dbeta),
             _p(dW), _p(db), _p(dcol), 0, _p(ws), nb, drop_seed, drop_p, 0, _stream(), *tail), "nv_head_bwd")
    return g, g16, dgamma, dbeta, dW, db, dcol


def _head_step_outputs(B, n, d, C, dev):
    logits, xh, st = torch.empty((B, C), device=dev), torch.empty((B, d), device=dev), torch.empty((B, 2), device=dev)
    loss, dl = torch.empty(1, device=dev), torch.empty((B, C), device=dev)
    g = torch.full((B, n, d), float("nan"), device=dev)
    g16 = torch.full((B, n, d), float("nan"), dtype=op16(), device=dev)
    dgamma, dbeta, dcol = (torch.empty(d, device=dev) for _ in range(3))
    dW, db = torch.empty((C, d), device=dev), torch.empty(C, device=dev)
    ws = torch.empty(lib.nv_head_step_workspace_bytes(B, d), dtype=torch.uint8, device=dev)
    return (logits, xh, st, loss, dl, g, g16, dgamma, dbeta, dW, db, dcol), ws


def head_step(x, gamma, beta, W, bias, labels, eps=1e-5, drop_seed=0, drop_p=0.0, path=NO_PATH, path_rows: int = 0, scale_state=None, opts=None):
    B, n, d = x.shape
    C = W.shape[0]
    outs, ws = _head_step_outputs(B, n, d, C, x.device)
    logits, xh, st, loss, dl, g, g16, dgamma, dbeta, dW, db, dcol = outs
    if path is not NO_PATH:
        check(lib.nv_head_step_path(_p(x), n * d, B, d, _p(gamma), _p(beta), eps, _p(W), _p(bias), C, _p(labels), 1.0, _p(scale_state),
                                    None if opts is None else ctypes.byref(opts), _p(xh), _p(st), _p(logits), _p(loss), _p(dl), n, _p(g), d, _p(g16), d,
                                    _p(dgamma), _p(dbeta), _p(dW), _p(db), _p(dcol), 0, _p(ws), ws.numel(), drop_seed, drop_p, _stream(), _p(path), int(path_rows)),
              "nv_head_step_path")
        return outs
    check(lib.nv_head_step(_p(x), n * d, B, d, _p(gamma), _p(beta), eps, _p(W), _p(bias), C, _p(labels), 1.0, _p(xh), _p(st), _p(logits), _p(loss), _p(dl),
                           n, _p(g), d, _p(g16), d, _p(dgamma), _p(dbeta), _p(dW), _p(db), _p(dcol), 0, _p(ws), ws.numel(), drop_seed, drop_p, _stream()),
          "nv_head_step")
    return outs


def colsum_bf16(X: torch.Tensor, accumulate=False, out=None):
    M, N = X.shape
    out = torch.empty(N, device=X.device) if out is None else out
    nb = lib.nv_colsum_workspace_bytes(M, N)
    ws = torch.empty(nb, dtype=torch.uint8, device=X.device)
    check(lib.nv_colsum_bf16(_p(X), X.stride(0), M, N, _p(out), int(accumulate), _p(ws), nb, _stream()), "nv_colsum_bf16")
    return out


def ce_loss(logits: torch.Tensor, target: torch.Tensor, grad_scale: float = 1.0, want_grad=True, scale_state=None):
    B, C = logits.shape
    loss = torch.empty(1, device=logits.device)
    dl = torch.empty_like(logits) if want_grad else None
    check(lib.nv_ce_loss_scaled(_p(logits), _p(target), B, C, grad_scale, _p(scale_state), _p(loss), _p(dl), _stream()), "nv_ce_loss")
    return loss, dl


def loss_opts(label_smoothing: float = 0.0, class_weight: Optional[torch.Tensor] = None, mix: Optional[torch.Tensor] = None, B: Optional[int] = None,
              C: Optional[int] = None, device=None):
    from ._cabi import LossOpts, MIX_COLS
    if isinstance(label_smoothing, bool) or not isinstance(label_smoothing, (int, float)):
        raise TypeError(f"label_smoothing must be a number, got {label_smoothing!r}")
    if not (0.0 <= float(label_smoothing) < 1.0):
        raise ValueError(f"label_smoothing {label_smoothing} outside [0, 1)")
    if class_weight is not None:
        if not (torch.is_tensor(class_weight) and class_weight.dtype == torch.float32 and class_weight.dim() == 1 and class_weight.is_contiguous()):
            raise ValueError("class_weight must be a dense float32 vector [C]")
        if C is not None and class_weight.numel() != C:
# ... 679 lines not shown
```

Measured before the change: 1165 volumes/s.

## Specialize last-layer CLS tail: fused LN+skinny GEMM, split skinny NN, live-tile attention bwd

For the last layer, when only CLS rows matter (the tail path), the forward fuses LayerNorm with the skinny NT matmul into one kernel. The backward uses a split-K style skinny NN kernel that takes a workspace. The attention dK/dV backward now iterates only over the first query tile, since the gradient on the other query rows is zero in the tail. A new default-on flag (NEUROVIT_CLS_TURN) gates all of this. The aim is to cut launches and wasted work in the final block, at the cost of extra workspace and correctness that depends on the assumption that only CLS rows carry gradient.

```diff
diff --git a/include/neurovit_hip.h b/include/neurovit_hip.h
--- a/include/neurovit_hip.h
+++ b/include/neurovit_hip.h
@@ -88,6 +88,14 @@
                  float* dcol, int accumulate, unsigned long drop_seed, float drop_p, void* stream);
 int nv_skinny_nn_sparse(int R, int N, int K, const void* A, long lda, const void* W, long ldw, void* out, long total_rows, int keep_every,
                         void* stream);
+int nv_skinny_nn_ws(int epi, int R, int N, int K, const void* A, long lda, const void* W, long ldw, const void* u, long ldu, void* out, long ldo,
+                    float* dcol, int accumulate, unsigned long drop_seed, float drop_p, void* stream, void* ws, long ws_bytes);
+int nv_skinny_nt_ln(int R, int N, int K, const float* x, long ldx, const float* gamma, const float* beta, float eps, void* xn, long ldxn, float* mean,
+                    float* rstd, const void* W, long ldw, const float* bias, void* out, long ldo, void* u_out, long ldu, unsigned long drop_seed,
+                    float drop_p, void* stream, void* nn_ws);
+long nv_skinny_nn_workspace_bytes(int N);
+int nv_skinny_nt_ws(int epi, int R, int N, int K, const void* A, long lda, const void* W, long ldw, const float* bias, const float* resid,
+                    long ldr, void* out, long ldo, void* u_out, long ldu, unsigned long drop_seed, float drop_p, void* stream, void* nn_ws);
 
 int nv_ln_fwd(const float* x, long ldx, int M, int d, const float* gamma, const float* beta, float eps, void* y, long ldy,
               float* mean, float* rstd, void* stream);
@@ -152,6 +160,9 @@
 int nv_attn_bwd(const void* qkv, long ld_qkv, const void* out, const void* dout, long ld_out, const float* lse, int B, int n,
                 int heads, int dim_head, float scale, float* delta, void* dqkv, long ld_dqkv, unsigned long drop_seed,
                 float drop_p, void* stream);
+int nv_attn_bwd_live(const void* qkv, long ld_qkv, const void* out, const void* dout, long ld_out, const float* lse, int B, int n,
+                     int heads, int dim_head, float scale, float* delta, void* dqkv, long ld_dqkv, unsigned long drop_seed,
+                     float drop_p, void* stream, int live_q_tiles);
 #define NV_ATTN_PER_HEAD 0
 #define NV_ATTN_FUSE_MEAN 1
 #define NV_ATTN_FUSE_MAX 2
@@ -293,6 +304,7 @@
 long nv_vit_param_count(const nv_vit_config* cfg);
 int nv_vit_param_table(const nv_vit_config* cfg, long* offsets, long* numels, int max_entries);
 long nv_vit_workspace_bytes(const nv_vit_config* cfg, int B, int training);
+int nv_vit_set_cls_turn(int on);
 long nv_vit_workspace_offset(const nv_vit_config* cfg, int B, int training, const char* name, int layer);
 typedef struct nv_vit_attn_export {
   int struct_size;
diff --git a/neurovit_amd/_cabi.py b/neurovit_amd/_cabi.py
--- a/neurovit_amd/_cabi.py
+++ b/neurovit_amd/_cabi.py
@@ -134,6 +134,8 @@
                 dll.nv_gemm_set_tile(12, int(os.environ["NEUROVIT_ADAMW_WGS"]))
             if os.environ.get("NEUROVIT_HEAD_STEP"):
                 dll.nv_vit_set_head_step(int(os.environ["NEUROVIT_HEAD_STEP"]))
+            if os.environ.get("NEUROVIT_CLS_TURN"):
+                dll.nv_vit_set_cls_turn(int(os.environ["NEUROVIT_CLS_TURN"]))
             if os.environ.get("NEUROVIT_WGRAD_WGS"):
                 dll.nv_gemm_set_tile(14, int(os.environ["NEUROVIT_WGRAD_WGS"]))
             if os.environ.get("NEUROVIT_PATCH_MODE"):
diff --git a/neurovit_amd/csrc/attention.hip b/neurovit_amd/csrc/attention.hip
--- a/neurovit_amd/csrc/attention.hip
+++ b/neurovit_amd/csrc/attention.hip
@@ -848,7 +848,7 @@
 __device__ __forceinline__ void attn_bwd_dkv_res_body(char* rsmem, int by, int bx, int nblk, const r16* __restrict__ qkv, long ld,
                                                       const r16* __restrict__ out, const r16* __restrict__ dout, long ldo,
                                                       const float* __restrict__ lse, const float* __restrict__ delta, int n, int heads,
-                                                      float scale, r16* __restrict__ dqkv, long ldd, const DropCfg& drop) {
+                                                      float scale, r16* __restrict__ dqkv, long ldd, const DropCfg& drop, int live_q_tiles = 0) {
   const int tid = threadIdx.x, lane = tid & 63, r = lane & 15, g = lane >> 4;
   const int wid = __builtin_amdgcn_readfirstlane(tid >> 6);
   const int b = by / heads, h = by - b * heads, inner = heads * DH;
@@ -857,7 +857,8 @@
   const r16* V = Q + 2 * inner;
   const r16* dO = dout + (long)b * n * ldo + h * DH;
   const float* L = lse + ((long)b * heads + h) * n;
-  const int nqt = (n + TQ - 1) / TQ;
+  const int all_qt = (n + TQ - 1) / TQ;
+  const int nqt = (live_q_tiles > 0 && live_q_tiles < all_qt) ? live_q_tiles : all_qt;
   char* sQ = rsmem;
   char* sD = rsmem + nqt * IMG;
   float* sL = reinterpret_cast<float*>(rsmem + 2 * nqt * IMG);
@@ -923,10 +924,10 @@
 __global__ __launch_bounds__(RES_THREADS) void attn_bwd_dkv_res_kernel(const r16* __restrict__ qkv, long ld, const r16* __restrict__ dout,
                                                                        long ldo, const float* __restrict__ lse, const float* __restrict__ delta,
                                                                        int n, int heads, float scale, r16* __restrict__ dqkv, long ldd,
-                                                                       DropCfg drop) {
+                                                                       DropCfg drop, int live_q_tiles) {
   extern __shared__ __attribute__((aligned(16))) char rsmem[];
   const ResBlock rb = res_block(n);
-  attn_bwd_dkv_res_body<DROP, false, T>(rsmem, rb.by, rb.bx, rb.nblk, qkv, ld, nullptr, dout, ldo, lse, delta, n, heads, scale, dqkv, ldd, drop);
+  attn_bwd_dkv_res_body<DROP, false, T>(rsmem, rb.by, rb.bx, rb.nblk, qkv, ld, nullptr, dout, ldo, lse, delta, n, heads, scale, dqkv, ldd, drop, live_q_tiles);
 }
 
 template <bool DROP, typename T>
@@ -1185,9 +1186,10 @@
   }
 }
 
-extern "C" int nv_attn_bwd(const void* qkv, long ld_qkv, const void* out, const void* dout, long ld_out, const float* lse, int B, int n,
-                           int heads, int dim_head, float scale, float* delta, void* dqkv, long ld_dqkv, unsigned long drop_seed, float drop_p,
-                           void* stream) {
+extern "C" int nv_attn_bwd_live(const void* qkv, long ld_qkv, const void* out, const void* dout, long ld_out, const float* lse, int B, int n,
+                                int heads, int dim_head, float scale, float* delta, void* dqkv, long ld_dqkv, unsigned long drop_seed, float drop_p,
+                                void* stream, int live_q_tiles) {
+  NV_CHECK_ARG(live_q_tiles >= 0, "nv_attn_bwd_live: live_q_tiles = %d must be >= 0 (0 = every tile)", live_q_tiles);
   NV_CHECK_ARG(attn_generic_supported(dim_head), "nv_attn_bwd: dim_head=%d unsupported (multiples of 8 up to 128)", dim_head);
   NV_CHECK_ARG(B > 0 && n > 0 && heads > 0 && ld_qkv >= 3 * heads * dim_head && ld_dqkv >= 3 * heads * dim_head && ld_out >= heads * dim_head &&
                    (ld_qkv % 8) == 0 && (ld_out % 8) == 0 && (ld_dqkv % 4) == 0,
@@ -1220,7 +1222,7 @@
     }
     ATTN_LAUNCH(K_DQ_RES, rgrid, dim3(RES_THREADS), 2 * nt * IMG, s, q16, ld_qkv, o16, do16, ld_out, lse, n, heads, scale, delta, dq16, ld_dqkv, drop);
     NV_CHECK_LAUNCH("nv_attn_bwd/dq(resident)");
-    ATTN_LAUNCH(K_DKV_RES, rgrid, dim3(RES_THREADS), 2 * nt * IMG + 2 * nt * TQ * 4, s, q16, ld_qkv, do16, ld_out, lse, delta, n, heads, scale, dq16, ld_dqkv, drop);
+    ATTN_LAUNCH(K_DKV_RES, rgrid, dim3(RES_THREADS), 2 * nt * IMG + 2 * nt * TQ * 4, s, q16, ld_qkv, do16, ld_out, lse, delta, n, heads, scale, dq16, ld_dqkv, drop, live_q_tiles);
     nv_prof_end(slot, stream);
     NV_CHECK_LAUNCH("nv_attn_bwd/dkv(resident)");
     return NV_OK;
@@ -1237,3 +1239,8 @@
   NV_CHECK_LAUNCH("nv_attn_bwd/dkv");
   return NV_OK;
 }
+extern "C" int nv_attn_bwd(const void* qkv, long ld_qkv, const void* out, const void* dout, long ld_out, const float* lse, int B, int n,
+                           int heads, int dim_head, float scale, float* delta, void* dqkv, long ld_dqkv, unsigned long drop_seed, float drop_p,
+                           void* stream) {
+  return nv_attn_bwd_live(qkv, ld_qkv, out, dout, ld_out, lse, B, n, heads, dim_head, scale, delta, dqkv, ld_dqkv, drop_seed, drop_p, stream, 0);
+}
diff --git a/neurovit_amd/csrc/engine.hip b/neurovit_amd/csrc/engine.hip
--- a/neurovit_amd/csrc/engine.hip
+++ b/neurovit_amd/csrc/engine.hip
@@ -23,6 +23,8 @@
 extern "C" int nv_vit_set_cls_tail(int on) { g_cls_tail = on ? 1 : 0; return 0; }
 static int g_head_step = 1;
 extern "C" int nv_vit_set_head_step(int on) { g_head_step = on ? 1 : 0; return 0; }
+static int g_cls_turn = 1;
+extern "C" int nv_vit_set_cls_turn(int on) { g_cls_turn = on ? 1 : 0; return 0; }
 static bool cls_tail_wanted(const Dims& D, int training, float drop_p, int rows_form) {
   const bool want = rows_form == 1 ? false : (rows_form == 2 ? true : g_cls_tail != 0);
   (void)drop_p;
@@ -91,6 +93,7 @@
   long g, dxn, hookg, dao, delta, dt, dt16, dxp, dwpe;
   LayerScratch sc[2];
   const LayerScratch& scratch(int l) const { return sc[l & 1]; }
+  long sk, sk_bytes;
   long red_bytes, red2_bytes, total;
 };
 
@@ -132,10 +135,13 @@
     const long cs1_bytes = (long)((M + 63) / 64) * D.m * 4;
     e.cs1 = add(cs1_bytes); o.cs1 = add(cs1_bytes);
     W.f8x = add(M * d); W.f8h = add(M * (long)D.m);
+    const int widest = D.m > D.d ? (D.m > D.inner ? D.m : D.inner) : (D.d > D.inner ? D.d : D.inner);
+    W.sk_bytes = nv_skinny_nn_workspace_bytes(widest); W.sk = add(W.sk_bytes);
   } else {
     W.g = W.dxn = W.hookg = W.dao = W.delta = W.dt = W.dt16 = W.dxp = W.dwpe = -1;
     W.sc[0] = W.sc[1] = {-1, -1, -1, -1, -1, -1, -1, -1};
     W.red_bytes = W.red2_bytes = 0;
+    W.sk = -1; W.sk_bytes = 0;
   }
   W.total = cur;
 }
@@ -306,13 +312,18 @@
 }
 
 static int cls_rows_block16(const Dims& D, const LayerP& q, const LayerW& w, int l, const float* p, const r16* p16, char* ws, float eps, const float* xin,
-                            float* x1, float* x2, float* st2, void* u, unsigned long drop_seed, float drop_p, float proj_p, void* stream, const float* sd = nullptr) {
+                            float* x1, float* x2, float* st2, void* u, unsigned long drop_seed, float drop_p, float proj_p, void* stream, const float* sd = nullptr, void* nn_ws = nullptr) {
   const int B = D.B, d = D.d;
   const long rs = D.n;
   RUN(nv_skinny_nt_path(0, B, d, D.inner, ws + w.ao, D.inner * rs, p16 + q.wo, D.inner, p + q.bo, xin, d * rs, x1, d * rs, nullptr, 0, site_seed(drop_seed, 4 * l + 1), proj_p, stream,
                         path_of(sd, l, 0, B), D.n));
-  RUN(nv_ln_fwd(x1, d * rs, B, d, p + q.n2g, p + q.n2b, eps, ws + w.xn2, d * rs, st2, st2 + D.M, stream));
-  RUN(nv_skinny_nt(1, B, D.m, d, ws + w.xn2, d * rs, p16 + q.w1, d, p + q.b1, nullptr, 0, ws + w.h, D.m * rs, u, D.m * rs, site_seed(drop_seed, 4 * l + 2), drop_p, stream));
+  if (g_cls_turn && B <= 4) {
+    RUN(nv_skinny_nt_ln(B, D.m, d, x1, d * rs, p + q.n2g, p + q.n2b, eps, ws + w.xn2, d * rs, st2, st2 + D.M, p16 + q.w1, d, p + q.b1, ws + w.h, D.m * rs, u, D.m * rs,
+                        site_seed(drop_seed, 4 * l + 2), drop_p, stream, nn_ws));
+  } else {
+    RUN(nv_ln_fwd(x1, d * rs, B, d, p + q.n2g, p + q.n2b, eps, ws + w.xn2, d * rs, st2, st2 + D.M, stream));
+    RUN(nv_skinny_nt_ws(1, B, D.m, d, ws + w.xn2, d * rs, p16 + q.w1, d, p + q.b1, nullptr, 0, ws + w.h, D.m * rs, u, D.m * rs, site_seed(drop_seed, 4 * l + 2), drop_p, stream, nn_ws));
+  }
   return nv_skinny_nt_path(0, B, d, D.m, ws + w.h, D.m * rs, p16 + q.w2, D.m, p + q.b2, x1, d * rs, x2, d * rs, nullptr, 0, site_seed(drop_seed, 4 * l + 3), drop_p, stream,
                            path_of(sd, l, 1, B), D.n);
 }
@@ -445,7 +456,8 @@
     RUN(nv_attn_fwd(ws + w.qkv, 3 * D.inner, B, D.n, D.heads, D.dh, scale, ws + w.ao, D.inner, (float*)(ws + w.lse), site_seed(drop_seed, 4 * l + 0), drop_p, stream));
     RUN(export_layer(in, l, 0, ws + w.qkv, D, B, scale, stream));
     if (tail && l == D.L - 1) {
-      RUN(cls_rows_block16(D, q, w, l, p, p16, ws, eps, xin, x1, x2, st2, training ? ws + w.u : nullptr, drop_seed, drop_p, proj_drop_p(cfg, drop_p), stream, sd));
+      RUN(cls_rows_block16(D, q, w, l, p, p16, ws, eps, xin, x1, x2, st2, training ? ws + w.u : nullptr, drop_seed, drop_p, proj_drop_p(cfg, drop_p), stream, sd,
+                           training ? ws + W.sk : nullptr));
       xin = x2;
       continue;
     }
@@ -642,7 +654,7 @@
     RUN(nv_gemm_f8(0, M, 3 * D.inner, d, x8, d, p8 + q.wqkv, d, ws + w.qkv, 3 * D.inner, cs, nullptr, nullptr, 0, 1.f, stream));
     RUN(nv_attn_fwd(ws + w.qkv, 3 * D.inner, B, D.n, D.heads, D.dh, scale, ws + w.ao, D.inner, (float*)(ws + w.lse), site_seed(drop_seed, 4 * l + 0), drop_p, stream));
     if (tail && l == D.L - 1) {
-      RUN(cls_rows_block16(D, q, w, l, p, p16, ws, eps, xin, x1, x2, st2, ws + w.u, drop_seed, drop_p, proj_drop_p(cfg, drop_p), stream));
+      RUN(cls_rows_block16(D, q, w, l, p, p16, ws, eps, xin, x1, x2, st2, ws + w.u, drop_seed, drop_p, proj_drop_p(cfg, drop_p), stream, nullptr, ws + W.sk));
       xin = x2;
       continue;
     }
@@ -680,6 +692,7 @@
   hipStream_t S, A;
   float* GR(long off) const { return c.grads ? c.grads + off : nullptr; }
   void* M16(long off) const { return c.grads16 ? (void*)((r16*)c.grads16 + off) : nullptr; }
+  void* sk() const { return g_cls_turn ? ws + W.sk : nullptr; }
   float* dxn1(int l) const { return (float*)(ws + (l == D.L - 1 ? W.hookg : W.dxn)); }
 
   int bwd_head() const {
@@ -696,8 +709,8 @@
     float* dxn = (float*)(ws + W.dxn); float* st2 = (float*)(ws + w.st2);
     void* g16 = ws + sc.g16; void* du = ws + sc.du;
     if (R.tail) {
-      RUN(nv_skinny_nn(0, D.B, D.m, d, g16, d * rs, p16 + q.w2, D.m, ws + w.u, D.m * rs, du, D.m * rs, GR(q.b1), acc, site_seed(c.drop_seed, 4 * l + 2), c.drop_p, S));
-      RUN(nv_skinny_nn(1, D.B, d, D.m, du, D.m * rs, p16 + q.w1, d, nullptr, 0, dxn, d * rs, nullptr, 0, 0, 0.f, S));
+      RUN(nv_skinny_nn_ws(0, D.B, D.m, d, g16, d * rs, p16 + q.w2, D.m, ws + w.u, D.m * rs, du, D.m * rs, GR(q.b1), acc, site_seed(c.drop_seed, 4 * l + 2), c.drop_p, S, sk(), W.sk_bytes));
+      RUN(nv_skinny_nn_ws(1, D.B, d, D.m, du, D.m * rs, p16 + q.w1, d, nullptr, 0, dxn, d * rs, nullptr, 0, 0, 0.f, S, sk(), W.sk_bytes));
     } else {
       RUN(nv_gemm_bf16(1, du_tile_rows ? 6 : 5, M, D.m, d, g16, d, p16 + q.w2, D.m, du, D.m, nullptr, ws + w.u, D.m, du_tile_rows ? (float*)(ws + sc.cs1) : nullptr, D.m, 0, 1.f,
                        site_seed(c.drop_seed, 4 * l + 2), c.drop_p, S));
@@ -714,8 +727,9 @@
       RUN(nv_skinny_nn_sparse(D.B, D.inner, d, ws + sc.g16b, d * R.rs, p16 + q.wo, D.inner, ws + W.dao, M, D.n, S));
     else
       RUN(nv_gemm_bf16(1, 0, M, D.inner, d, ws + sc.g16b, d, p16 + q.wo, D.inner, ws + W.dao, D.inner, nullptr, nullptr, 0, nullptr, 0, 0, 1.f, 0, 0.f, S));
-    RUN(nv_attn_bwd(ws + w.qkv, 3 * D.inner, ws + w.ao, ws + W.dao, D.inner, (float*)(ws + w.lse), D.B, D.n, D.heads, D.dh, scale,
-                    (float*)(ws + W.delta), ws + sc.dqkv, 3 * D.inner, site_seed(c.drop_seed, 4 * l + 0), c.drop_p, S));
+    const int live_q_tiles = (R.tail && g_cls_turn && !(c.attn_grad && c.attn_grad->maps[l])) ? 1 : 0;
+    RUN(nv_attn_bwd_live(ws + w.qkv, 3 * D.inner, ws + w.ao, ws + W.dao, D.inner, (float*)(ws + w.lse), D.B, D.n, D.heads, D.dh, scale,
+                         (float*)(ws + W.delta), ws + sc.dqkv, 3 * D.inner, site_seed(c.drop_seed, 4 * l + 0), c.drop_p, S, live_q_tiles));
     if (c.attn_grad && c.attn_grad->maps[l])
       RUN(nv_attn_grad(ws + w.qkv, 3 * D.inner, ws + W.dao, D.inner, D.B, D.n, D.heads, D.dh, scale, c.attn_grad->form, c.attn_grad->maps[l], S));
     return NV_OK;
diff --git a/neurovit_amd/csrc/ln_rows.h b/neurovit_amd/csrc/ln_rows.h
--- /dev/null
+++ b/neurovit_amd/csrc/ln_rows.h
@@ -0,0 +1,44 @@
+#pragma once
+#include "common.h"
+
+template <int NV>
+__device__ __forceinline__ void row_load(const float* row, int d, int lane, f32x4 (&x)[NV]) {
+#pragma unroll
+  for (int v = 0; v < NV; ++v) {
+    const int c = (lane + 64 * v) * 4;
+    x[v] = (c < d) ? *reinterpret_cast<const f32x4*>(row + c) : f32x4{0.f, 0.f, 0.f, 0.f};
+  }
+}
+template <int NV>
+__device__ __forceinline__ void row_stats(const f32x4 (&x)[NV], int d, int lane, float eps, float& mean, float& rstd) {
+  float s = 0.f;
+#pragma unroll
+  for (int v = 0; v < NV; ++v) s += (x[v][0] + x[v][1]) + (x[v][2] + x[v][3]);
+  mean = wave_sum(s) / (float)d;
+  float q = 0.f;
+#pragma unroll
+  for (int v = 0; v < NV; ++v) {
+    const int c = (lane + 64 * v) * 4;
+    if (c < d) {
+      const f32x4 t = x[v] - mean;
+      q += (t[0] * t[0] + t[1] * t[1]) + (t[2] * t[2] + t[3] * t[3]);
+    }
+  }
+  rstd = 1.0f / sqrtf(wave_sum(q) / (float)d + eps);
+}
+template <int NV, typename Put>
+__device__ __forceinline__ void ln_fwd_row(const float* row, int d, int lane, const float* __restrict__ gamma, const float* __restrict__ beta, float eps,
+                                           float& mean, float& rstd, Put put) {
+  f32x4 xv[NV];
+  row_load<NV>(row, d, lane, xv);
+  row_stats<NV>(xv, d, lane, eps, mean, rstd);
+#pragma unroll
+  for (int v = 0; v < NV; ++v) {
+    const int c = (lane + 64 * v) * 4;
+    if (c < d) {
+      const f32x4 gm = *reinterpret_cast<const f32x4*>(gamma + c), bt = *reinterpret_cast<const f32x4*>(beta + c);
+      const f32x4 o = (xv[v] - mean) * rstd * gm + bt;
+      put(c, o);
+    }
+  }
+}
diff --git a/neurovit_amd/csrc/norm.hip b/neurovit_amd/csrc/norm.hip
--- a/neurovit_amd/csrc/norm.hip
+++ b/neurovit_amd/csrc/norm.hip
@@ -1,4 +1,5 @@
 #include "common.h"
+#include "ln_rows.h"
 
 #define WAVES_PER_BLOCK 4
 
@@ -10,31 +11,6 @@
 }
 __device__ __forceinline__ r16 cvt1_rt(float v, int fp16) { return fp16 ? cvt1<fp16_t>(v) : cvt1<bf16_t>(v); }
 
-template <int NV>
-__device__ __forceinline__ void row_load(const float* row, int d, int lane, f32x4 (&x)[NV]) {
-#pragma unroll
-  for (int v = 0; v < NV; ++v) {
-    const int c = (lane + 64 * v) * 4;
-    x[v] = (c < d) ? *reinterpret_cast<const f32x4*>(row + c) : f32x4{0.f, 0.f, 0.f, 0.f};
-  }
-}
-template <int NV>
-__device__ __forceinline__ void row_stats(const f32x4 (&x)[NV], int d, int lane, float eps, float& mean, float& rstd) {
-  float s = 0.f;
-#pragma unroll
-  for (int v = 0; v < NV; ++v) s += (x[v][0] + x[v][1]) + (x[v][2] + x[v][3]);
-  mean = wave_sum(s) / (float)d;
-  float q = 0.f;
-#pragma unroll
-  for (int v = 0; v < NV; ++v) {
-    const int c = (lane + 64 * v) * 4;
-    if (c < d) {
-      const f32x4 t = x[v] - mean;
-      q += (t[0] * t[0] + t[1] * t[1]) + (t[2] * t[2] + t[3] * t[3]);
-    }
-  }
-  rstd = 1.0f / sqrtf(wave_sum(q) / (float)d + eps);
-}
 
 template <int NV, typename OT>
 __global__ __launch_bounds__(256) void ln_fwd_kernel(const float* __restrict__ x, long ldx, int M, int d, const float* __restrict__ gamma,
@@ -42,19 +18,8 @@
                                                      float* __restrict__ mean_out, float* __restrict__ rstd_out) {
   const int lane = threadIdx.x & 63, row = blockIdx.x * WAVES_PER_BLOCK + (threadIdx.x >> 6);
   if (row >= M) return;
-  f32x4 xv[NV];
-  row_load<NV>(x + (long)row * ldx, d, lane, xv);
   float mean, rstd;
-  row_stats<NV>(xv, d, lane, eps, mean, rstd);
-#pragma unroll
-  for (int v = 0; v < NV; ++v) {
-    const int c = (lane + 64 * v) * 4;
-    if (c < d) {
-      const f32x4 gm = *reinterpret_cast<const f32x4*>(gamma + c), bt = *reinterpret_cast<const f32x4*>(beta + c);
-      const f32x4 o = (xv[v] - mean) * rstd * gm + bt;
-      store4<OT>(y + (long)row * ldy + c, o);
-    }
-  }
+  ln_fwd_row<NV>(x + (long)row * ldx, d, lane, gamma, beta, eps, mean, rstd, [&](int c, const f32x4& o) { store4<OT>(y + (long)row * ldy + c, o); });
   if (lane == 0 && mean_out) {
     mean_out[row] = mean;
     rstd_out[row] = rstd;
diff --git a/neurovit_amd/csrc/skinny.hip b/neurovit_amd/csrc/skinny.hip
--- a/neurovit_amd/csrc/skinny.hip
+++ b/neurovit_amd/csrc/skinny.hip
@@ -1,4 +1,5 @@
 #include "common.h"
+#include "ln_rows.h"
 
 namespace {
 
@@ -10,8 +11,10 @@
 template <int EPI, typename T, bool PATH>
 __global__ __launch_bounds__(256) void skinny_nt_kernel(const r16* __restrict__ A, long lda, int R, const r16* __restrict__ W, long ldw, int N, int K,
                                                         const float* __restrict__ bias, const float* __restrict__ resid, long ldr,
-                                                        void* __restrict__ out, long ldo, r16* __restrict__ u_out, long ldu, DropCfg drop, PathArg<PATH> path) {
+                                                        void* __restrict__ out, long ldo, r16* __restrict__ u_out, long ldu, DropCfg drop, PathArg<PATH> path,
+                                                        unsigned* __restrict__ tickets) {
   const int lane = threadIdx.x & 63, n = blockIdx.x * 4 + (threadIdx.x >> 6);
+  if (tickets && blockIdx.x == 0 && blockIdx.y == 0) tickets[threadIdx.x] = 0u;
   const int r0 = blockIdx.y * SK_R, rows = (R - r0 < SK_R) ? R - r0 : SK_R;
   if (n >= N) return;
   float acc[SK_R];
@@ -62,6 +65,70 @@
       if (u_out) u_out[row * ldu + n] = cvt1<T>(v);
       ((r16*)out)[row * ldo + n] = cvt1<T>(gelu_f(v) * keep);
     }
+  }
+}
+
+constexpr int SK_LN_MAXD = 2048;
+template <typename T, int NV>
+__global__ __launch_bounds__(256) void skinny_nt_ln_kernel(const float* __restrict__ x, long ldx, int R, const float* __restrict__ gamma, const float* __restrict__ beta,
+                                                           float eps, r16* __restrict__ xn, long ldxn, float* __restrict__ mean_out, float* __restrict__ rstd_out,
+                                                           const r16* __restrict__ W, long ldw, int N, int K, const float* __restrict__ bias,
+                                                           r16* __restrict__ out, long ldo, r16* __restrict__ u_out, long ldu, DropCfg drop,
+                                                           unsigned* __restrict__ tickets) {
+  __shared__ __attribute__((aligned(16))) r16 sA[SK_R][SK_LN_MAXD];
+  const int lane = threadIdx.x & 63, wid = threadIdx.x >> 6, n = blockIdx.x * 4 + wid;
+  if (tickets && blockIdx.x == 0) tickets[threadIdx.x] = 0u;
+  const bool col = n < N;
+  r16x8 wq[4];
+  if (col) {
+    const r16* w = W + (long)n * ldw;
+#pragma unroll
+    for (int q = 0; q < 4; ++q)
+      if (lane * 8 + 512 * q < K) wq[q] = *reinterpret_cast<const r16x8*>(w + lane * 8 + 512 * q);
+  }
+  if (wid < R) {
+    float mean, rstd;
+    const bool writer = blockIdx.x == 0;
+    ln_fwd_row<NV>(x + (long)wid * ldx, K, lane, gamma, beta, eps, mean, rstd, [&](int c, const f32x4& o) {
+      const r16x4 h = cvt4<T>(o[0], o[1], o[2], o[3]);
+      *reinterpret_cast<r16x4*>(&sA[wid][c]) = h;
+      if (writer) *reinterpret_cast<r16x4*>(xn + (long)wid * ldxn + c) = h;
+    });
+    if (writer && lane == 0) { mean_out[wid] = mean; rstd_out[wid] = rstd; }
+  }
+  __syncthreads();
+  if (!col) return;
+  float acc[SK_R];
+#pragma unroll
+  for (int r = 0; r < SK_R; ++r) acc[r] = 0.f;
+#pragma unroll
+  for (int q = 0; q < 4; ++q) {
+    const int kq = lane * 8 + 512 * q;
+    if (kq < K) {
+#pragma unroll
+      for (int r = 0; r < SK_R; ++r) {
+        if (r < R) {
+          const r16x8 a = *reinterpret_cast<const r16x8*>(&sA[r][kq]);
+#pragma unroll
+          for (int e = 0; e < 8; ++e) acc[r] = __builtin_fmaf(dec1<T>(a[e]), dec1<T>(wq[q][e]), acc[r]);
+        }
+      }
+    }
+  }
+  float mine = 0.f;
+#pragma unroll
+  for (int r = 0; r < SK_R; ++r) {
+    if (r < R) {
+      const float t = wave_sum(acc[r]);
+      if (lane == r) mine = t;
+    }
+  }
+  if (lane < R) {
+    const long row = lane;
+    const float v = mine + bias[n];
+    const float keep = drop.thresh ? drop_factor(drop, (unsigned long long)(row * ldo + n)) : 1.f;
+    if (u_out) u_out[row * ldu + n] = cvt1<T>(v);
+    out[row * ldo + n] = cvt1<T>(gelu_f(v) * keep);
   }
 }
 
@@ -179,10 +246,154 @@
   attr = true;
 }
 
-}
-
-extern "C" int nv_skinny_nt(int epi, int R, int N, int K, const void* A, long lda, const void* W, long ldw, const float* bias, const float* resid,
-                            long ldr, void* out, long ldo, void* u_out, long ldu, unsigned long drop_seed, float drop_p, void* stream) {
+constexpr int NS_COLS = 64, NS_WAVES = 16;
+constexpr int NS_PART_FLOATS = NN_KK * SK_R * NS_COLS;
+constexpr int NS_MIN_LDS = 84 * 1024;
+constexpr long NS_TICKET_BYTES = 1024;
+
+template <int EPI, typename T, int WPG>
+__global__ __launch_bounds__(256 * WPG) void skinny_nn_split_kernel(const r16* __restrict__ A, long lda, int R, const r16* __restrict__ W, long ldw, int N, int K,
+                                                               const r16* __restrict__ u, long ldu, void* __restrict__ out, long ldo,
+                                                               float* __restrict__ dcol, int accumulate, DropCfg drop, unsigned* tickets, unsigned* slab) {
+  constexpr int wpg = WPG;
+  extern __shared__ __attribute__((aligned(16))) float sk_lds[];
+  __shared__ unsigned s_last;
+  const int tid = threadIdx.x, lw = tid >> 8, t = tid & 255, ng = t & 7, kk = t >> 3;
+  const int cg = blockIdx.x, n0 = cg * NS_COLS, nc = n0 + ng * 8, wv = blockIdx.y * wpg + lw, parts = gridDim.y;
+  float (*part)[SK_R][NS_COLS] = reinterpret_cast<float (*)[SK_R][NS_COLS]>(sk_lds + lw * NS_PART_FLOATS);
+  float acc[SK_R][8];
+#pragma unroll
+  for (int r = 0; r < SK_R; ++r)
+#pragma unroll
+    for (int e = 0; e < 8; ++e) acc[r][e] = 0.f;
+  if (nc < N) {
+    constexpr int STEP = NS_WAVES * NN_KK, Q = WPG == 1 ? 6 : 2;
+    int rr[SK_R];
+#pragma unroll
+    for (int r = 0; r < SK_R; ++r) rr[r] = r < R ? r : R - 1;
+    for (int k = wv * NN_KK + kk; k < K; k += Q * STEP) {
+      r16x8 wq[Q];
+      r16 aq[Q][SK_R];
+#pragma unroll
+      for (int q = 0; q < Q; ++q) {
+        const int kq = (k + STEP * q < K) ? k + STEP * q : k;
+        wq[q] = *reinterpret_cast<const r16x8*>(W + (long)kq * ldw + nc);
+#pragma unroll
+        for (int r = 0; r < SK_R; ++r) aq[q][r] = A[(long)rr[r] * lda + kq];
+      }
+      __builtin_amdgcn_sched_barrier(0);
+#pragma unroll
+      for (int q = 0; q < Q; ++q) {
+        const bool in = k + STEP * q < K;
+#pragma unroll
+        for (int r = 0; r < SK_R; ++r) {
+          const float a = dec1<T>(aq[q][r]);
+#pragma unroll
+          for (int e = 0; e < 8; ++e) {
+            const float s = __builtin_fmaf(a, dec1<T>(wq[q][e]), acc[r][e]);
+            acc[r][e] = in ? s : acc[r][e];
+          }
+        }
+      }
+    }
+  }
+#pragma unroll
+  for (int r = 0; r < SK_R; ++r) {
+    *reinterpret_cast<f32x4*>(&part[kk][r][ng * 8]) = f32x4{acc[r][0], acc[r][1], acc[r][2], acc[r][3]};
+    *reinterpret_cast<f32x4*>(&part[kk][r][ng * 8 + 4]) = f32x4{acc[r][4], acc[r][5], acc[r][6], acc[r][7]};
+  }
+  __syncthreads();
+  const int r = t >> 6, c = t & 63;
+  {
+    float v = 0.f;
+#pragma unroll
+    for (int q = 0; q < NN_KK; ++q) v += part[q][r][c];
+    __hip_atomic_store(slab + (((long)cg * NS_WAVES + wv) * SK_R + r) * NS_COLS + c, __float_as_uint(v), __ATOMIC_RELAXED, __HIP_MEMORY_SCOPE_AGENT);
+  }
+  asm volatile("s_waitcnt vmcnt(0)" ::: "memory");
+  __syncthreads();
+  if (tid == 0) s_last = (__hip_atomic_fetch_add(tickets + cg, 1u, __ATOMIC_RELAXED, __HIP_MEMORY_SCOPE_AGENT) == (unsigned)parts - 1) ? 1u : 0u;
+  __syncthreads();
+  if (!s_last || lw) return;
+  if (tid == 0) __hip_atomic_store(tickets + cg, 0u, __ATOMIC_RELAXED, __HIP_MEMORY_SCOPE_AGENT);
+  float stored = 0.f;
+  const bool live = r < R && n0 + c < N;
+  {
+    float p[NS_WAVES];
+#pragma unroll
+    for (int w = 0; w < NS_WAVES; ++w)
+      p[w] = __uint_as_float(__hip_atomic_load(slab + (((long)cg * NS_WAVES + w) * SK_R + r) * NS_COLS + c, __ATOMIC_RELAXED, __HIP_MEMORY_SCOPE_AGENT));
+    float v = 0.f;
+#pragma unroll
+    for (int w = 0; w < NS_WAVES; ++w) v += p[w];
+    if (live) {
+      const long row = r;
+      const int n = n0 + c;
+      if constexpr (EPI == SK_NN_DGELU) {
+        const float keep = drop.thresh ? drop_factor(drop, (unsigned long long)(row * ldo + n)) : 1.f;
+        const r16 o = cvt1<T>(v * keep * gelu_grad_f(dec1<T>(u[row * ldu + n])));
+        ((r16*)out)[row * ldo + n] = o;
+        stored = dec1<T>(o);
+      } else if constexpr (EPI == SK_NN_F32) {
+        ((float*)out)[row * ldo + n] = v;
+      } else {
+        ((r16*)out)[row * ldo + n] = cvt1<T>(v);
+      }
+    }
+  }
+  if constexpr (EPI == SK_NN_DGELU) {
+    if (dcol) {
+      float (*cs)[NS_COLS] = reinterpret_cast<float (*)[NS_COLS]>(sk_lds);
+      __syncthreads();
+      cs[r][c] = live ? stored : 0.f;
+      __syncthreads();
+      if (r == 0 && n0 + c < N) {
+        float s = 0.f;
+#pragma unroll
+        for (int q = 0; q < SK_R; ++q) s += cs[q][c];
+        dcol[n0 + c] = (accumulate ? dcol[n0 + c] : 0.f) + s;
+      }
+    }
+  }
+}
+
+inline int ns_wpg(int N) { return ((N + NS_COLS - 1) / NS_COLS) * NS_WAVES > 256 ? 4 : 1; }
+inline long ns_ws_bytes(int N) { return NS_TICKET_BYTES + (long)((N + NS_COLS - 1) / NS_COLS) * NS_WAVES * SK_R * NS_COLS * 4; }
+
+template <int EPI, typename T>
+void ns_attrs_one() {
+  (void)hipFuncSetAttribute(reinterpret_cast<const void*>(skinny_nn_split_kernel<EPI, T, 1>), hipFuncAttributeMaxDynamicSharedMemorySize, NS_MIN_LDS);
+  (void)hipFuncSetAttribute(reinterpret_cast<const void*>(skinny_nn_split_kernel<EPI, T, 4>), hipFuncAttributeMaxDynamicSharedMemorySize, 4 * NS_PART_FLOATS * 4);
+}
+template <typename T>
+void ns_attrs_fmt() { ns_attrs_one<SK_NN_DGELU, T>(); ns_attrs_one<SK_NN_F32, T>(); ns_attrs_one<SK_NN_BF16, T>(); }
+
+bool ns_serves(int R, int N, const void* ws, long ws_bytes) {
+  return ws && R <= SK_R && (N + NS_COLS - 1) / NS_COLS <= (int)(NS_TICKET_BYTES / 4) && ws_bytes >= ns_ws_bytes(N) && nv_aligned16(ws);
+}
+
+template <int EPI>
+void ns_launch(int R, int N, int K, const void* A, long lda, const void* W, long ldw, const void* u, long ldu, void* out, long ldo, float* dcol, int accumulate,
+               DropCfg drop, void* ws, hipStream_t s) {
+  static bool attr = false;
+  if (!attr) { ns_attrs_fmt<bf16_t>(); ns_attrs_fmt<fp16_t>(); attr = true; }
+  const int wpg = ns_wpg(N), lds = wpg * NS_PART_FLOATS * 4;
+  const dim3 grid((N + NS_COLS - 1) / NS_COLS, NS_WAVES / wpg), block(256 * wpg);
+  unsigned* tickets = (unsigned*)ws;
+  unsigned* slab = (unsigned*)((char*)ws + NS_TICKET_BYTES);
+#define NS_GO(WPG) hipLaunchKernelGGL((skinny_nn_split_kernel<EPI, T, WPG>), grid, block, lds > NS_MIN_LDS ? lds : NS_MIN_LDS, s, (const r16*)A, lda, R, (const r16*)W, ldw, N, K, \
+                                     (const r16*)u, ldu, out, ldo, dcol, accumulate, drop, tickets, slab)
+  NV_DISPATCH_OPERAND(T, if (wpg == 1) NS_GO(1); else NS_GO(4));
+#undef NS_GO
+}
+
+}
+
+extern "C" long nv_skinny_nn_workspace_bytes(int N) { return N > 0 ? ns_ws_bytes(N) : -1; }
+
+extern "C" int nv_skinny_nt_ws(int epi, int R, int N, int K, const void* A, long lda, const void* W, long ldw, const float* bias, const float* resid,
+                               long ldr, void* out, long ldo, void* u_out, long ldu, unsigned long drop_seed, float drop_p, void* stream, void* nn_ws) {
+  static_assert(NS_TICKET_BYTES == 256 * 4, "skinny_nt_kernel clears one ticket word per thread");
   NV_CHECK_ARG(drop_p == 0.f || (ldo % N) == 0, "nv_skinny_nt: with dropout `out` must be a row-strided view of a dense [M, N] tensor (ldo a multiple of N)");
   const DropCfg drop = make_drop(drop_seed, drop_p);
   NV_CHECK_ARG(R > 0 && N > 0 && K > 0 && (K % 8) == 0 && (lda % 8) == 0 && (ldw % 8) == 0 && A && W && bias && out && nv_aligned16(A) && nv_aligned16(W),
@@ -192,11 +403,34 @@
   hipStream_t s = (hipStream_t)stream;
   NV_DISPATCH_OPERAND(T,
     if (epi == SK_NT_RESID)
-      hipLaunchKernelGGL((skinny_nt_kernel<SK_NT_RESID, T, false>), grid, block, 0, s, (const r16*)A, lda, R, (const r16*)W, ldw, N, K, bias, resid, ldr, out, ldo, (r16*)nullptr, 0L, drop, NoPath{});
+      hipLaunchKernelGGL((skinny_nt_kernel<SK_NT_RESID, T, false>), grid, block, 0, s, (const r16*)A, lda, R, (const r16*)W, ldw, N, K, bias, resid, ldr, out, ldo, (r16*)nullptr, 0L, drop, NoPath{}, (unsigned*)nn_ws);
     else
-      hipLaunchKernelGGL((skinny_nt_kernel<SK_NT_GELU, T, false>), grid, block, 0, s, (const r16*)A, lda, R, (const r16*)W, ldw, N, K, bias, resid, ldr, out, ldo, (r16*)u_out, ldu, drop, NoPath{}));
+      hipLaunchKernelGGL((skinny_nt_kernel<SK_NT_GELU, T, false>), grid, block, 0, s, (const r16*)A, lda, R, (const r16*)W, ldw, N, K, bias, resid, ldr, out, ldo, (r16*)u_out, ldu, drop, NoPath{}, (unsigned*)nn_ws));
   NV_CHECK_LAUNCH("nv_skinny_nt");
   return NV_OK;
+}
+extern "C" int nv_skinny_nt_ln(int R, int N, int K, const float* x, long ldx, const float* gamma, const float* beta, float eps, void* xn, long ldxn, float* mean,
+                               float* rstd, const void* W, long ldw, const float* bias, void* out, long ldo, void* u_out, long ldu, unsigned long drop_seed,
+                               float drop_p, void* stream, void* nn_ws) {
+  NV_CHECK_ARG(drop_p == 0.f || (ldo % N) == 0, "nv_skinny_nt_ln: with dropout `out` must be a row-strided view of a dense [M, N] tensor (ldo a multiple of N)");
+  NV_CHECK_ARG(R > 0 && R <= SK_R && N > 0 && K > 0 && K <= SK_LN_MAXD && (K % 8) == 0, "nv_skinny_nt_ln: R = %d must be 1..4, K = %d a multiple of 8 up to 2048", R, K);
+  NV_CHECK_ARG(x && gamma && beta && xn && mean && rstd && W && bias && out && (ldx % 4) == 0 && (ldxn % 4) == 0 && (ldw % 8) == 0 && nv_aligned16(x) && nv_aligned16(xn) &&
+                   nv_aligned16(gamma) && nv_aligned16(beta) && nv_aligned16(W),
+               "nv_skinny_nt_ln: null pointer, or ldx / ldxn no multiple of 4, ldw no multiple of 8, or an operand not 16-byte aligned");
+  const DropCfg drop = make_drop(drop_seed, drop_p);
+  const dim3 grid((N + 3) / 4), block(256);
+  hipStream_t s = (hipStream_t)stream;
+#define SK_LN(NV) hipLaunchKernelGGL((skinny_nt_ln_kernel<T, NV>), grid, block, 0, s, x, ldx, R, gamma, beta, eps, (r16*)xn, ldxn, mean, rstd, (const r16*)W, ldw, N, K, bias, \
+                                     (r16*)out, ldo, (r16*)u_out, ldu, drop, (unsigned*)nn_ws)
+  NV_DISPATCH_OPERAND(T, if (K <= 1024) SK_LN(4); else SK_LN(8));
+#undef SK_LN
+  NV_CHECK_LAUNCH("nv_skinny_nt_ln");
+  return NV_OK;
+}
+
+extern "C" int nv_skinny_nt(int epi, int R, int N, int K, const void* A, long lda, const void* W, long ldw, const float* bias, const float* resid,
+                            long ldr, void* out, long ldo, void* u_out, long ldu, unsigned long drop_seed, float drop_p, void* stream) {
+  return nv_skinny_nt_ws(epi, R, N, K, A, lda, W, ldw, bias, resid, ldr, out, ldo, u_out, ldu, drop_seed, drop_p, stream, nullptr);
 }
 
 extern "C" int nv_skinny_nt_path(int epi, int R, int N, int K, const void* A, long lda, const void* W, long ldw, const float* bias, const float* resid,
@@ -212,25 +446,36 @@
   const PathCfg pc{path, path_rows, (int)(ldo / N)};
   const dim3 grid((N + 3) / 4, (R + SK_R - 1) / SK_R), block(256);
   NV_DISPATCH_OPERAND(T, hipLaunchKernelGGL((skinny_nt_kernel<SK_NT_RESID, T, true>), grid, block, 0, (hipStream_t)stream, (const r16*)A, lda, R, (const r16*)W, ldw, N, K, bias,
-                                            resid, ldr, out, ldo, (r16*)nullptr, 0L, drop, pc));
+                                            resid, ldr, out, ldo, (r16*)nullptr, 0L, drop, pc, (unsigned*)nullptr));
   NV_CHECK_LAUNCH("nv_skinny_nt_path");
   return NV_OK;
 }
 
-extern "C" int nv_skinny_nn(int epi, int R, int N, int K, const void* A, long lda, const void* W, long ldw, const void* u, long ldu, void* out, long ldo,
-                            float* dcol, int accumulate, unsigned long drop_seed, float drop_p, void* stream) {
+extern "C" int nv_skinny_nn_ws(int epi, int R, int N, int K, const void* A, long lda, const void* W, long ldw, const void* u, long ldu, void* out, long ldo,
+                               float* dcol, int accumulate, unsigned long drop_seed, float drop_p, void* stream, void* ws, long ws_bytes) {
   NV_CHECK_ARG(drop_p == 0.f || (epi == SK_NN_DGELU && (ldo % N) == 0), "nv_skinny_nn: dropout only with epilogue 0, `out` a row-strided view of a dense [M, N] tensor");
   const DropCfg drop = make_drop(drop_seed, drop_p);
   NV_CHECK_ARG(R > 0 && N > 0 && K > 0 && (N % 8) == 0 && (ldw % 8) == 0 && A && W && out && nv_aligned16(W), "nv_skinny_nn: N, ldw must be multiples of 8, W 16-byte aligned");
   NV_CHECK_ARG(epi >= 0 && epi <= 2 && (epi != SK_NN_DGELU || u) && (!dcol || (epi == SK_NN_DGELU && R <= SK_R)), "nv_skinny_nn: epilogue 0 needs u; column sums only with epilogue 0 and R <= 4");
   const dim3 grid((N + NN_COLS - 1) / NN_COLS, (R + SK_R - 1) / SK_R), block(1024);
   hipStream_t s = (hipStream_t)stream;
+  if (ns_serves(R, N, ws, ws_bytes)) {
+#define NS_NN(E) ns_launch<E>(R, N, K, A, lda, W, ldw, u, ldu, out, ldo, dcol, accumulate, drop, ws, s)
+    if (epi == SK_NN_DGELU) NS_NN(SK_NN_DGELU); else if (epi == SK_NN_F32) NS_NN(SK_NN_F32); else NS_NN(SK_NN_BF16);
+#undef NS_NN
+    NV_CHECK_LAUNCH("nv_skinny_nn(split)");
+    return NV_OK;
+  }
   nn_attrs();
 #define SK_NN(E) hipLaunchKernelGGL((skinny_nn_kernel<E, T>), grid, block, NN_LDS, s, (const r16*)A, lda, R, (const r16*)W, ldw, N, K, (const r16*)u, ldu, out, ldo, dcol, accumulate, 0L, 0, drop)
   NV_DISPATCH_OPERAND(T, if (epi == SK_NN_DGELU) SK_NN(SK_NN_DGELU); else if (epi == SK_NN_F32) SK_NN(SK_NN_F32); else SK_NN(SK_NN_BF16));
 #undef SK_NN
   NV_CHECK_LAUNCH("nv_skinny_nn");
   return NV_OK;
+}
+extern "C" int nv_skinny_nn(int epi, int R, int N, int K, const void* A, long lda, const void* W, long ldw, const void* u, long ldu, void* out, long ldo,
+                            float* dcol, int accumulate, unsigned long drop_seed, float drop_p, void* stream) {
+  return nv_skinny_nn_ws(epi, R, N, K, A, lda, W, ldw, u, ldu, out, ldo, dcol, accumulate, drop_seed, drop_p, stream, nullptr, 0);
 }
 
 extern "C" int nv_skinny_nn_sparse(int R, int N, int K, const void* A, long lda, const void* W, long ldw, void* out, long total_rows, int keep_every,
diff --git a/neurovit_amd/ops.py b/neurovit_amd/ops.py
--- a/neurovit_amd/ops.py
+++ b/neurovit_amd/ops.py
@@ -67,13 +67,33 @@
     return out
 
 
+def skinny_nt_ln(x: torch.Tensor, gamma, beta, W: torch.Tensor, bias: torch.Tensor, xn: torch.Tensor, mean: torch.Tensor, rstd: torch.Tensor,
+                 out: torch.Tensor, u_out: Optional[torch.Tensor] = None, eps: float = 1e-5, drop_seed: int = 0, drop_p: float = 0.0) -> torch.Tensor:
+    _need_cuda(x, W)
+    R, K = x.shape
+    N = W.shape[0]
+    check(lib.nv_skinny_nt_ln(R, N, K, _p(x), x.stride(0), _p(gamma), _p(beta), float(eps), _p(xn), xn.stride(0), _p(mean), _p(rstd), _p(W), W.stride(0),
+                              _p(bias), _p(out), out.stride(0), _p(u_out), 0 if u_out is None else u_out.stride(0), int(drop_seed), float(drop_p),
+                              _stream(), None), "nv_skinny_nt_ln")
+    return out
+
+
+def skinny_nn_workspace(N: int, device="cuda") -> torch.Tensor:
+    return torch.zeros(lib.nv_skinny_nn_workspace_bytes(int(N)), dtype=torch.uint8, device=device)
+
+
 def skinny_nn(epi: int, A: torch.Tensor, W: torch.Tensor, out: torch.Tensor, u: Optional[torch.Tensor] = None,
-              dcol: Optional[torch.Tensor] = None, accumulate: bool = False, drop_seed: int = 0, drop_p: float = 0.0) -> torch.Tensor:
+              dcol: Optional[torch.Tensor] = None, accumulate: bool = False, drop_seed: int = 0, drop_p: float = 0.0,
+              ws: Optional[torch.Tensor] = None) -> torch.Tensor:
     _need_cuda(A, W)
     R, K = A.shape
     N = W.shape[1]
-    check(lib.nv_skinny_nn(epi, R, N, K, _p(A), A.stride(0), _p(W), W.stride(0), _p(u), 0 if u is None else u.stride(0), _p(out), out.stride(0),
-                           _p(dcol), int(accumulate), int(drop_seed), float(drop_p), _stream()), "nv_skinny_nn")
+    args = (epi, R, N, K, _p(A), A.stride(0), _p(W), W.stride(0), _p(u), 0 if u is None else u.stride(0), _p(out), out.stride(0),
+            _p(dcol), int(accumulate), int(drop_seed), float(drop_p), _stream())
+    if ws is None:
+        check(lib.nv_skinny_nn(*args), "nv_skinny_nn")
+    else:
+        check(lib.nv_skinny_nn_ws(*args, _p(ws), ws.numel()), "nv_skinny_nn_ws")
     return out
 
 
@@ -346,12 +366,16 @@
     return out
 
 
-def attn_bwd(qkv, out, dout, lse, B, n, heads, dim_head=64, drop_seed=0, drop_p=0.0):
+def attn_bwd(qkv, out, dout, lse, B, n, heads, dim_head=64, drop_seed=0, drop_p=0.0, live_q_tiles=None):
     inner = heads * dim_head
     dqkv = torch.empty((B * n, 3 * inner), dtype=op16(), device=qkv.device)
     delta = torch.empty((B, heads, n), dtype=torch.float32, device=qkv.device)
-    check(lib.nv_attn_bwd(_p(qkv), qkv.stride(0), _p(out), _p(dout), inner, _p(lse), B, n, heads, dim_head, dim_head ** -0.5, _p(delta),
-                          _p(dqkv), 3 * inner, drop_seed, drop_p, _stream()), "nv_attn_bwd")
+    args = (_p(qkv), qkv.stride(0), _p(out), _p(dout), inner, _p(lse), B, n, heads, dim_head, dim_head ** -0.5, _p(delta),
+            _p(dqkv), 3 * inner, drop_seed, drop_p, _stream())
+    if live_q_tiles is None:
+        check(lib.nv_attn_bwd(*args), "nv_attn_bwd")
+    else:
+        check(lib.nv_attn_bwd_live(*args, int(live_q_tiles)), "nv_attn_bwd_live")
     return dqkv, delta
 
 
```

Result: no change. 1169 volumes/s, median of 6 (+0.3%).
